# elun15/Graph-Convolutional-Network-for-Multi-Camera-Vehicle-Tracking

Hardware: NVIDIA B200
Metric: mpn_inference_directed_edges_per_sec (higher is better)
Workload: dtype f32

## Files before the change

graph-convolutional-network-for-multi-camera-vehicle-tracking_b200/_lib.py:

```python
import ctypes as C
import os

_HERE = os.path.dirname(os.path.abspath(__file__))
LIB_PATH = os.path.join(_HERE, "libmpn_b200.so")

MPN_OK, MPN_ERR_INVALID, MPN_ERR_CUDA, MPN_ERR_UNSORTED, MPN_ERR_WORKSPACE, MPN_ERR_NO_DEVICE = range(6)
MPN_DE, MPN_DH, MPN_MAX_NODE_LAYERS = 4, 32, 8
MPN_SUMS_DOUBLES = 96
ABI_VERSION = 6
STAGE_ENC0, STAGE_ENC1, STAGE_EDGE, STAGE_NODE, STAGE_APPLY = range(5)
POST_CUT, POST_PRUNE, POST_SPLIT = 1, 2, 4

W_ENC1_W, W_ENC1_B, W_ENC1_G, W_ENC1_BETA = 0, 8, 12, 16
W_ENC2_W, W_ENC2_B, W_ENC2_G, W_ENC2_BETA = 20, 36, 40, 44
W_EDGE_W, W_EDGE_B, W_EDGE_G, W_EDGE_BETA = 48, 320, 324, 328
W_NODE_W, W_NODE_B, W_NODE_G, W_NODE_BETA = 332, 1484, 1516, 1548
W_CLS_W, W_CLS_B = 1580, 1588
W_EDGE_W0, W_NODE_W0, W_SMALL_FLOATS = 1592, 1864, 2888


class MpnGraph(C.Structure):
    _fields_ = [("n_nodes", C.c_int32), ("n_cols", C.c_int32), ("row_offset", C.c_int32), ("chunk", C.c_int32),
                ("n_edges", C.c_int64), ("max_tasks", C.c_int32), ("layout_hint", C.c_int32),
                ("rowptr", C.c_void_p), ("col", C.c_void_p), ("taskptr", C.c_void_p), ("task_row", C.c_void_p),
                ("n_tasks", C.c_void_p), ("n_graphs", C.c_int32), ("max_graph_nodes", C.c_int32),
                ("node_gid", C.c_void_p), ("graph_nptr", C.c_void_p)]


class MpnWeights(C.Structure):
    _fields_ = [("n_node_layers", C.c_int32), ("node_dims", C.c_int32 * (MPN_MAX_NODE_LAYERS + 1)),
                ("node_w", C.c_void_p * MPN_MAX_NODE_LAYERS), ("node_b", C.c_void_p * MPN_MAX_NODE_LAYERS),
                ("node_gamma", C.c_void_p * MPN_MAX_NODE_LAYERS), ("node_beta", C.c_void_p * MPN_MAX_NODE_LAYERS),
                ("small", C.c_void_p),
                ("node_w_hi", C.c_void_p * MPN_MAX_NODE_LAYERS), ("node_w_lo", C.c_void_p * MPN_MAX_NODE_LAYERS),
                ("node_w_hi16", C.c_void_p * MPN_MAX_NODE_LAYERS), ("node_w_lo16", C.c_void_p * MPN_MAX_NODE_LAYERS),
                ("node_w_scale16", C.c_float * MPN_MAX_NODE_LAYERS), ("node_bn_gmax", C.c_float * MPN_MAX_NODE_LAYERS),
                ("node_bn_bmax", C.c_float * MPN_MAX_NODE_LAYERS),
                ("node_agg", C.c_int32), ("reattach_nodes", C.c_int32), ("reattach_edges", C.c_int32), ("reserved", C.c_int32)]


AGG_SUM, AGG_MEAN, AGG_MAX = 0, 1, 2


MPN_MAX_PEERS = 16


class MpnPeerCtx(C.Structure):
    _fields_ = [("rank", C.c_int32), ("world", C.c_int32), ("sums", C.c_void_p * MPN_MAX_PEERS),
                ("flags", C.c_void_p * MPN_MAX_PEERS), ("h", C.c_void_p * MPN_MAX_PEERS),
                ("cstats", C.c_void_p * MPN_MAX_PEERS),
                ("seq_moments", C.c_uint64), ("seq_h", C.c_uint64), ("seq_c", C.c_uint64),
                ("shard_node_encoder", C.c_int32), ("reserved", C.c_int32),
                ("edge_attr", C.c_void_p * MPN_MAX_PEERS), ("node_tables", C.c_void_p * MPN_MAX_PEERS),
                ("block_start", C.c_int32 * (MPN_MAX_PEERS + 1)), ("reserved2", C.c_int32), ("seq_t", C.c_uint64)]
MPN_PEER_CSTAT_COLS = 1024


class MpnError(RuntimeError):
    def __init__(self, code, message):
        super().__init__("libmpn_b200 error %d: %s" % (code, message))
        self.code = code


class UnsortedEdgeIndex(MpnError):
    pass


_lib = None

_PROTOS = {
    "mpn_abi_version": (C.c_int, []),
    "mpn_last_error": (C.c_char_p, []),
    "mpn_kernel_launches": (C.c_uint64, []),
    "mpn_check_device": (C.c_int, [C.c_int]),
    "mpn_set_pdl": (C.c_int, [C.c_int]),
    "mpn_graph_build": (C.c_int, [C.POINTER(MpnGraph), C.c_void_p, C.c_void_p]),
    "mpn_graph_build_i32": (C.c_int, [C.POINTER(MpnGraph), C.c_void_p, C.c_void_p, C.c_void_p]),
    "mpn_graph_build_deferred": (C.c_int, [C.POINTER(MpnGraph), C.c_void_p, C.c_void_p, C.c_void_p, C.c_void_p]),
    "mpn_cross_camera_edges": (C.c_int64, [C.c_void_p, C.c_int32]),
    "mpn_cross_camera_block_edges": (C.c_int64, [C.c_void_p, C.c_int32, C.c_int32, C.c_int32]),
    "mpn_graph_build_cross_camera": (C.c_int, [C.POINTER(MpnGraph), C.c_void_p, C.c_int32, C.c_void_p, C.c_void_p]),
    "mpn_cross_camera_batched_layout": (C.c_int64, [C.c_void_p, C.c_int32, C.c_void_p, C.c_int32, C.c_void_p]),
    "mpn_graph_build_cross_camera_batched": (C.c_int, [C.POINTER(MpnGraph), C.c_void_p, C.c_int32, C.c_void_p, C.c_void_p,
                                                       C.c_void_p, C.c_void_p]),
    "mpn_profile_gram": (C.c_int, [C.c_int]),
    "mpn_profile_gram_ms": (C.c_float, []),
    "mpn_shared_gram_mode": (C.c_int, [C.c_void_p, C.c_int32, C.c_void_p, C.c_size_t, C.c_void_p]),
    "mpn_shared_gram_row_range": (C.c_int, [C.c_int32, C.c_int32, C.c_void_p, C.c_int32, C.c_void_p]),
    "mpn_pack_decisions": (C.c_int, [C.c_void_p, C.c_int64, C.c_void_p, C.c_void_p]),
    "mpn_profile_timeline": (C.c_int, [C.c_int]),
    "mpn_profile_timeline_read": (C.c_int, [C.c_void_p, C.c_char_p, C.c_int]),
    "mpn_edge_features_workspace_bytes": (C.c_size_t, [C.POINTER(MpnGraph), C.c_int32]),
    "mpn_edge_features": (C.c_int, [C.POINTER(MpnGraph), C.c_void_p, C.c_int32, C.c_void_p, C.c_int, C.c_void_p, C.c_size_t, C.c_void_p]),
    "mpn_forward_workspace_bytes": (C.c_size_t, [C.POINTER(MpnGraph), C.POINTER(MpnWeights), C.c_int32]),
    "mpn_forward": (C.c_int, [C.POINTER(MpnGraph), C.POINTER(MpnWeights), C.c_void_p, C.c_void_p, C.c_int32, C.c_int32,
                              C.c_void_p, C.c_void_p, C.c_void_p, C.c_void_p, C.c_int, C.c_void_p, C.c_size_t, C.c_void_p]),
    "mpn_forward_with_edge_features": (C.c_int, [C.POINTER(MpnGraph), C.POINTER(MpnWeights), C.c_void_p, C.c_void_p, C.c_int32, C.c_int32,
                                                 C.c_void_p, C.c_void_p, C.c_void_p, C.c_void_p, C.c_int, C.c_void_p, C.c_size_t,
                                                 C.c_void_p, C.c_size_t, C.c_void_p]),
    "mpn_plan_create": (C.c_int, [C.POINTER(C.c_void_p), C.POINTER(MpnGraph), C.POINTER(MpnWeights), C.c_int32, C.c_int32,
                                  C.c_int64, C.c_int, C.c_void_p, C.c_size_t]),
    "mpn_plan_destroy": (None, [C.c_void_p]),
    "mpn_plan_node_encoder": (C.c_int, [C.c_void_p, C.c_void_p, C.c_void_p]),
    "mpn_plan_node_tables": (C.c_int, [C.c_void_p, C.c_int32, C.c_void_p]),
    "mpn_plan_sweep": (C.c_int, [C.c_void_p, C.c_int32, C.c_int32, C.c_void_p, C.c_void_p, C.c_void_p, C.c_void_p, C.c_void_p]),
    "mpn_plan_sums": (C.c_void_p, [C.c_void_p]),
    "mpn_plan_reduce": (C.c_int, [C.c_void_p, C.c_int32, C.c_int, C.c_void_p]),
    "mpn_plan_finalize": (C.c_int, [C.c_void_p, C.c_int32, C.c_int32, C.c_void_p]),
    "mpn_plan_node_finalize": (C.c_int, [C.c_void_p, C.c_int32, C.c_void_p]),
    "mpn_plan_h_full": (C.c_void_p, [C.c_void_p]),
    "mpn_split_tf32": (C.c_int, [C.c_void_p, C.c_int64, C.c_void_p, C.c_void_p, C.c_void_p]),
    "mpn_split_f16": (C.c_int, [C.c_void_p, C.c_int64, C.c_float, C.c_void_p, C.c_void_p, C.POINTER(C.c_float), C.c_void_p]),
    "mpn_forward_sharded": (C.c_int, [C.POINTER(MpnGraph), C.POINTER(MpnWeights), C.c_void_p, C.c_void_p, C.c_int32, C.c_int32,
                                      C.c_int64, C.c_void_p, C.c_void_p, C.c_void_p, C.c_void_p, C.c_int, C.POINTER(MpnPeerCtx),
                                      C.c_void_p, C.c_size_t, C.c_void_p]),
    "mpn_forward_sharded_with_edge_features": (C.c_int, [C.POINTER(MpnGraph), C.POINTER(MpnWeights), C.c_void_p, C.c_void_p, C.c_int32,
                                                         C.c_int32, C.c_int64, C.c_void_p, C.c_void_p, C.c_void_p, C.c_void_p, C.c_int,
                                                         C.POINTER(MpnPeerCtx), C.c_void_p, C.c_size_t, C.c_void_p, C.c_size_t, C.c_void_p]),
    "mpn_decide": (C.c_int, [C.c_void_p, C.c_int64, C.c_void_p, C.c_void_p, C.c_void_p]),
    "mpn_post_workspace_bytes": (C.c_size_t, [C.POINTER(MpnGraph)]),
    "mpn_cut": (C.c_int, [C.POINTER(MpnGraph), C.c_void_p, C.c_void_p, C.c_size_t, C.c_void_p]),
    "mpn_prune": (C.c_int, [C.POINTER(MpnGraph), C.c_void_p, C.c_void_p, C.c_int32, C.c_int32, C.POINTER(C.c_int32),
                            C.POINTER(C.c_int32), C.c_void_p, C.c_size_t, C.c_void_p]),
    "mpn_split": (C.c_int, [C.POINTER(MpnGraph), C.c_void_p, C.c_void_p, C.c_int32, C.c_int32, C.POINTER(C.c_int32),
                            C.c_void_p, C.c_size_t, C.c_void_p]),
    "mpn_split_last_stats": (None, [C.c_void_p]),
    "mpn_scc_labels": (C.c_int, [C.POINTER(MpnGraph), C.c_void_p, C.c_void_p, C.POINTER(C.c_int32), C.c_void_p, C.c_size_t, C.c_void_p]),
    "mpn_post_processing": (C.c_int, [C.POINTER(MpnGraph), C.c_void_p, C.c_void_p, C.c_int32, C.c_int32, C.c_int32, C.c_void_p,
                                      C.POINTER(C.c_int32), C.POINTER(C.c_int32), C.c_void_p, C.c_size_t, C.c_void_p]),
    "mpn_post_processing_batched": (C.c_int, [C.POINTER(MpnGraph), C.c_void_p, C.c_void_p, C.c_int32, C.c_void_p, C.c_int32,
                                              C.c_void_p, C.c_void_p, C.c_void_p, C.c_size_t, C.c_void_p]),
    "mpn_active_edges": (C.c_int, [C.POINTER(MpnGraph), C.c_void_p, C.c_void_p, C.c_void_p, C.c_int64, C.POINTER(C.c_int64),
                                   C.c_void_p, C.c_size_t, C.c_void_p]),
    "mpn_compact_workspace_bytes": (C.c_size_t, [C.POINTER(MpnGraph)]),
    "mpn_count_active": (C.c_int, [C.POINTER(MpnGraph), C.c_void_p, C.POINTER(C.c_int64), C.c_void_p, C.c_size_t, C.c_void_p]),
    "mpn_compact_active": (C.c_int, [C.POINTER(MpnGraph), C.c_void_p, C.c_void_p, C.c_int32, C.c_void_p, C.c_void_p, C.c_void_p,
                                     C.c_void_p, C.c_void_p, C.c_size_t, C.c_void_p]),
    "mpn_clear_inactive": (C.c_int, [C.c_void_p, C.c_void_p, C.c_void_p, C.c_int64, C.c_void_p]),
    "mpn_labels_reference": (C.c_int, [C.POINTER(MpnGraph), C.c_void_p, C.c_void_p, C.POINTER(C.c_int32), C.c_void_p, C.c_size_t,
                                      C.c_void_p]),
    "mpn_labels_reference_batched": (C.c_int, [C.POINTER(MpnGraph), C.c_void_p, C.c_void_p, C.c_void_p, C.c_void_p, C.c_size_t,
                                              C.c_void_p]),
    "mpn_labels_reference_host": (C.c_int, [C.c_void_p, C.c_void_p, C.c_int64, C.c_int32, C.c_void_p, C.POINTER(C.c_int32)]),
    "mpn_split_exact_host": (C.c_int, [C.c_void_p, C.c_void_p, C.c_void_p, C.c_int64, C.c_int32, C.c_int32, C.c_void_p,
                                      C.c_void_p]),
    "mpn_edge_confusion": (C.c_int, [C.c_void_p, C.c_int, C.c_void_p, C.c_int, C.c_int64, C.c_void_p, C.c_void_p]),
    "mpn_contingency_workspace_bytes": (C.c_size_t, [C.c_int64]),
    "mpn_contingency": (C.c_int, [C.c_void_p, C.c_void_p, C.c_int64, C.c_int64, C.c_int64, C.c_void_p, C.c_void_p, C.c_void_p,
                                  C.POINTER(C.c_int64), C.c_void_p, C.c_void_p, C.c_void_p, C.c_size_t, C.c_void_p]),
    "mpn_expected_mutual_information_host": (C.c_double, [C.c_void_p, C.c_int64, C.c_void_p, C.c_int64, C.c_int64]),
    "mpn_relabel_workspace_bytes": (C.c_size_t, [C.c_int64]),
    "mpn_relabel_detections": (C.c_int, [C.c_void_p, C.c_void_p, C.c_int64, C.c_void_p, C.c_void_p, C.c_void_p, C.c_int64,
                                         C.c_void_p, C.c_void_p, C.c_size_t, C.c_void_p]),
    "mpn_write_mtmc_txt_host": (C.c_int, [C.c_char_p, C.c_void_p, C.c_int64, C.c_int32]),
    "mpn_edge_labels": (C.c_int, [C.POINTER(MpnGraph), C.c_void_p, C.c_void_p, C.c_void_p]),
    "mpn_normalize_columns_workspace_bytes": (C.c_size_t, [C.c_int32]),
    "mpn_normalize_columns": (C.c_int, [C.c_void_p, C.c_int32, C.c_int32, C.c_void_p, C.c_void_p, C.c_size_t, C.c_void_p]),
    "mpn_normalize_columns_batched": (C.c_int, [C.c_void_p, C.c_int32, C.c_int32, C.c_void_p, C.c_int32, C.c_void_p, C.c_void_p,
                                                C.c_size_t, C.c_void_p]),
    "mpn_gemm_nt_workspace_bytes": (C.c_size_t, [C.c_int32, C.c_int32, C.c_int32, C.c_int]),
    "mpn_gram_nt": (C.c_int, [C.c_void_p, C.c_int32, C.c_void_p, C.c_int32, C.c_int32, C.c_int32, C.c_void_p, C.c_void_p, C.c_size_t,
                              C.c_void_p]),
    "mpn_gemm_nt": (C.c_int, [C.c_void_p, C.c_void_p, C.c_void_p, C.c_void_p, C.c_int32, C.c_int32, C.c_int32, C.c_int,
                              C.c_void_p, C.c_size_t, C.c_void_p]),
}

EXPORTED_SYMBOLS = tuple(_PROTOS.keys())


def lib():
    global _lib
    if _lib is None:
        if not os.path.isfile(LIB_PATH):
            raise ImportError("libmpn_b200.so not built: run %s (or __graft_entry__.build()); "
                              "the MPN hot path has no CPU fallback" % os.path.join(_HERE, "csrc", "build.sh"))
        l = C.CDLL(LIB_PATH)
        for name, (res, args) in _PROTOS.items():
            fn = getattr(l, name)
            fn.restype, fn.argtypes = res, args
        if l.mpn_abi_version() != ABI_VERSION:
            raise ImportError("libmpn_b200.so ABI version mismatch")
        _lib = l
    return _lib


def check(code):
    if code != MPN_OK:
        msg = lib().mpn_last_error().decode("utf-8", "replace")
        if code == MPN_ERR_UNSORTED:
            raise UnsortedEdgeIndex(code, msg)
        raise MpnError(code, msg)


_DEVICE_OK = set()


def require_device(index: int):
    index = int(index)
    if index not in _DEVICE_OK:
        check(lib().mpn_check_device(index))
        _DEVICE_OK.add(index)
```

graph-convolutional-network-for-multi-camera-vehicle-tracking_b200/csrc/gemm_tc.cu:

```cuda
#include <cuda.h>
#include <cuda_fp16.h>
#include <stdlib.h>

#include <cmath>

#include "common.cuh"
#include "kernels.h"
#include "tcgen05.cuh"

namespace mpn {

constexpr int TC_BM = 128;
constexpr int TC_BK = 32;
constexpr int TC_UMMA_K = 8;
constexpr int TC_THREADS = 192;
constexpr int TC_BK_F16 = 64;

__device__ __forceinline__ uint64_t make_smem_desc(uint32_t saddr) {
  uint64_t d = 0;
  d |= (uint64_t)((saddr & 0x3FFFF) >> 4);
  d |= (uint64_t)1 << 16;
  d |= (uint64_t)(1024 >> 4) << 32;
  d |= (uint64_t)1 << 46;
  d |= (uint64_t)2 << 61;
  return d;
}

template <int BN>
struct TcCfg {
  static constexpr int STAGES = (BN == 256) ? 2 : 3;
  static constexpr int A_BYTES = TC_BM * TC_BK * 4;
  static constexpr int B_BYTES = BN * TC_BK * 4;
  static constexpr int STAGE_BYTES = 2 * A_BYTES + 2 * B_BYTES;
  static constexpr int SMEM_BYTES = STAGES * STAGE_BYTES + 1024  + 256 ;
  static constexpr int N_MAIN = (BN == 256) ? 1 : 2;
  static constexpr int TMEM_COLS = 512;
  static constexpr int CORR_COL = N_MAIN * BN;
  static constexpr uint32_t IDESC = (1u << 4) | (2u << 7) | (2u << 10) | ((uint32_t)(BN >> 3) << 17) | ((uint32_t)(TC_BM >> 4) << 24);
  static constexpr uint32_t IDESC_F16 = (1u << 4) | ((uint32_t)(BN >> 3) << 17) | ((uint32_t)(TC_BM >> 4) << 24);
};

template <int BN, bool SYM, bool F16>
__global__ void __launch_bounds__(TC_THREADS, 1)
gemm_nt_3xtf32_kernel(const __grid_constant__ CUtensorMap map_a_hi, const __grid_constant__ CUtensorMap map_a_lo,
                      const __grid_constant__ CUtensorMap map_b_hi, const __grid_constant__ CUtensorMap map_b_lo,
                      const float* __restrict__ bias, float* __restrict__ C, int M, int N, int K,
                      const int* __restrict__ graph_nptr, const long long* __restrict__ g_off,
                      const float* __restrict__ out_scale, const int* __restrict__ run_flag) {
  pdl_wait();
  if (run_flag != nullptr && *run_flag == 0) return;
  constexpr int BK = F16 ? TC_BK_F16 : TC_BK;
  using Cfg = TcCfg<BN>;
  extern __shared__ uint8_t smem_raw[];
  uint8_t* smem = (uint8_t*)(((uintptr_t)smem_raw + 1023) & ~(uintptr_t)1023);
  uint64_t* full_bar = (uint64_t*)(smem + Cfg::STAGES * Cfg::STAGE_BYTES);
  uint64_t* empty_bar = full_bar + Cfg::STAGES;
  uint64_t* tmem_full_bar = empty_bar + Cfg::STAGES;
  uint32_t* tmem_slot = (uint32_t*)(tmem_full_bar + 1);

  const int warp = threadIdx.x >> 5, lane = threadIdx.x & 31;
  int m0 = blockIdx.y * TC_BM, n0 = blockIdx.x * BN;
  int tm0 = m0, tn0 = n0;
  const int num_kb = (K + BK - 1) / BK;
  if (SYM && n0 + BN <= m0) return;
  if (graph_nptr != nullptr) {
    const int base = graph_nptr[blockIdx.z];
    const int ng = graph_nptr[blockIdx.z + 1] - base;
    if (m0 >= ng || n0 >= ng) return;
    tm0 = base + m0;
    tn0 = base + n0;
    M = N = ng;
    C += g_off[blockIdx.z];
  }
  if (threadIdx.x == 0) {
    for (int s = 0; s < Cfg::STAGES; ++s) { mbar_init(&full_bar[s], 1); mbar_init(&empty_bar[s], 1); }
    mbar_init(tmem_full_bar, 1);
    asm volatile("fence.mbarrier_init.release.cluster;" ::: "memory");
  }
  if (warp == 1) {
    asm volatile("tcgen05.alloc.cta_group::1.sync.aligned.shared::cta.b32 [%0], %1;" ::"r"(smem_u32(tmem_slot)), "n"(Cfg::TMEM_COLS));
    asm volatile("tcgen05.relinquish_alloc_permit.cta_group::1.sync.aligned;");
  }
  asm volatile("tcgen05.fence::before_thread_sync;" ::: "memory");
  __syncthreads();
  asm volatile("tcgen05.fence::after_thread_sync;" ::: "memory");
  const uint32_t tmem_base = *tmem_slot;

  if (warp == 0) {
    if (lane == 0) {
      asm volatile("prefetch.tensormap [%0];" ::"l"(&map_a_hi));
      asm volatile("prefetch.tensormap [%0];" ::"l"(&map_a_lo));
      asm volatile("prefetch.tensormap [%0];" ::"l"(&map_b_hi));
      asm volatile("prefetch.tensormap [%0];" ::"l"(&map_b_lo));
      int stage = 0;
      uint32_t phase = 0;
      for (int kb = 0; kb < num_kb; ++kb) {
        mbar_wait(&empty_bar[stage], phase ^ 1);
        uint8_t* st = smem + stage * Cfg::STAGE_BYTES;
        mbar_expect_tx(&full_bar[stage], Cfg::STAGE_BYTES);
        const int k0 = kb * BK;
        tma_load_2d(&map_a_hi, &full_bar[stage], st, k0, tm0);
        tma_load_2d(&map_a_lo, &full_bar[stage], st + Cfg::A_BYTES, k0, tm0);
        tma_load_2d(&map_b_hi, &full_bar[stage], st + 2 * Cfg::A_BYTES, k0, tn0);
        tma_load_2d(&map_b_lo, &full_bar[stage], st + 2 * Cfg::A_BYTES + Cfg::B_BYTES, k0, tn0);
        if (++stage == Cfg::STAGES) { stage = 0; phase ^= 1; }
      }
    }
  } else if (warp == 1) {
    if (lane == 0) {
      int stage = 0;
      uint32_t phase = 0;
      for (int kb = 0; kb < num_kb; ++kb) {
        mbar_wait(&full_bar[stage], phase);
        asm volatile("tcgen05.fence::after_thread_sync;" ::: "memory");
        const uint32_t sbase = smem_u32(smem + stage * Cfg::STAGE_BYTES);
        const uint64_t a_hi = make_smem_desc(sbase), a_lo = make_smem_desc(sbase + Cfg::A_BYTES);
        const uint64_t b_hi = make_smem_desc(sbase + 2 * Cfg::A_BYTES), b_lo = make_smem_desc(sbase + 2 * Cfg::A_BYTES + Cfg::B_BYTES);
#pragma unroll
        for (int kk = 0; kk < TC_BK / TC_UMMA_K; ++kk) {
          const uint64_t adv = (uint64_t)((kk * TC_UMMA_K * 4) >> 4);
          const int slice = kb * (TC_BK / TC_UMMA_K) + kk;
          const int which = (Cfg::N_MAIN == 2) ? (slice & 1) : 0;
          if (F16) {
            umma_f16(tmem_base + which * BN, a_hi + adv, b_hi + adv, Cfg::IDESC_F16, slice >= Cfg::N_MAIN);
            umma_f16(tmem_base + Cfg::CORR_COL, a_lo + adv, b_hi + adv, Cfg::IDESC_F16, slice != 0);
            umma_f16(tmem_base + Cfg::CORR_COL, a_hi + adv, b_lo + adv, Cfg::IDESC_F16, 1);
          } else {
            umma_tf32(tmem_base + which * BN, a_hi + adv, b_hi + adv, Cfg::IDESC, slice >= Cfg::N_MAIN);
            umma_tf32(tmem_base + Cfg::CORR_COL, a_lo + adv, b_hi + adv, Cfg::IDESC, slice != 0);
            umma_tf32(tmem_base + Cfg::CORR_COL, a_hi + adv, b_lo + adv, Cfg::IDESC, 1);
          }
        }
        umma_commit(&empty_bar[stage]);
        if (++stage == Cfg::STAGES) { stage = 0; phase ^= 1; }
      }
      umma_commit(tmem_full_bar);
    }
  } else {
    mbar_wait(tmem_full_bar, 0);
    asm volatile("tcgen05.fence::after_thread_sync;" ::: "memory");
    const int q = warp & 3;
    const int row = m0 + q * 32 + lane;
    const bool vec_ok = ((N & 3) == 0) && ((((uintptr_t)C) & 15) == 0);
    const float oscale = (F16 && out_scale) ? *out_scale : 1.f;
#pragma unroll 1
    for (int c0 = 0; c0 < BN; c0 += 32) {
      if (n0 + c0 >= N) break;
      float v[32], w[32];
      const uint32_t tq = tmem_base + ((uint32_t)(q * 32) << 16) + (uint32_t)c0;
      tmem_ld32(tq, v);
      if (Cfg::N_MAIN == 2) {
        tmem_ld32(tq + BN, w);
#pragma unroll
        for (int j = 0; j < 32; ++j) v[j] += w[j];
      }
      tmem_ld32(tq + Cfg::CORR_COL, w);
#pragma unroll
      for (int j = 0; j < 32; ++j) v[j] = F16 ? (v[j] + w[j]) * oscale : v[j] + w[j];
      if (row < M) {
        float* out = C + (size_t)row * N + n0 + c0;
        if (vec_ok && n0 + c0 + 32 <= N) {
#pragma unroll
          for (int j = 0; j < 32; j += 4) {
            float4 o = make_float4(v[j], v[j + 1], v[j + 2], v[j + 3]);
            if (bias) {
              const float4 b = *reinterpret_cast<const float4*>(bias + n0 + c0 + j);
              o.x += b.x; o.y += b.y; o.z += b.z; o.w += b.w;
            }
            *reinterpret_cast<float4*>(out + j) = o;
          }
        } else {
#pragma unroll
          for (int j = 0; j < 32; ++j)
            if (n0 + c0 + j < N) out[j] = v[j] + (bias ? bias[n0 + c0 + j] : 0.f);
        }
      }
      if (SYM && row < M) {
#pragma unroll
        for (int j = 0; j < 32; ++j) {
          const int col = n0 + c0 + j;
          if (col < N && col >= m0 + TC_BM) C[(size_t)col * N + row] = v[j];
        }
      }
    }
    asm volatile("tcgen05.fence::before_thread_sync;" ::: "memory");
  }
  __syncthreads();
  if (warp == 1) {
    asm volatile("tcgen05.fence::after_thread_sync;" ::: "memory");
    asm volatile("tcgen05.dealloc.cta_group::1.sync.aligned.b32 %0, %1;" ::"r"(tmem_base), "n"(Cfg::TMEM_COLS));
  }
}

__global__ void __launch_bounds__(256) split_tf32_kernel(const float4* __restrict__ x, long long n4, int K, const float* __restrict__ scale,
                                                         const float* __restrict__ shift, const int* __restrict__ row_gid,
                                                         float4* __restrict__ hi, float4* __restrict__ lo) {
  pdl_wait();
  const long long stride = (long long)gridDim.x * blockDim.x;
  for (long long i = (long long)blockIdx.x * blockDim.x + threadIdx.x; i < n4; i += stride) {
    const float4 v = x[i];
    float in[4] = {v.x, v.y, v.z, v.w};
    if (scale != nullptr) {
      const int k = (int)((i * 4) % K);
      const size_t o = (row_gid ? (size_t)row_gid[(i * 4) / K] * K : 0) + k;
      const float4 sc = *reinterpret_cast<const float4*>(scale + o), sh = *reinterpret_cast<const float4*>(shift + o);
      in[0] = fmaxf(fmaf(in[0], sc.x, sh.x), 0.f);
      in[1] = fmaxf(fmaf(in[1], sc.y, sh.y), 0.f);
      in[2] = fmaxf(fmaf(in[2], sc.z, sh.z), 0.f);
      in[3] = fmaxf(fmaf(in[3], sc.w, sh.w), 0.f);
    }
    float h[4], l[4];
#pragma unroll
    for (int j = 0; j < 4; ++j) {
      uint32_t hb, lb;
      asm("cvt.rna.tf32.f32 %0, %1;" : "=r"(hb) : "f"(in[j]));
      h[j] = __uint_as_float(hb);
      const float r = in[j] - h[j];
      asm("cvt.rna.tf32.f32 %0, %1;" : "=r"(lb) : "f"(r));
      l[j] = __uint_as_float(lb);
    }
    hi[i] = make_float4(h[0], h[1], h[2], h[3]);
    lo[i] = make_float4(l[0], l[1], l[2], l[3]);
  }
}

__device__ __forceinline__ float f16_scale_of(float amax) {
  if (!(amax > 0.f) || !isfinite(amax)) return 1.f;
  int e;
  frexpf(amax, &e);
  return ldexpf(1.f, 14 - e);
}
__global__ void __launch_bounds__(256) split_f16_kernel(const float4* __restrict__ x, long long n4, const float* __restrict__ amax,
                                                        uint2* __restrict__ hi, uint2* __restrict__ lo, float* __restrict__ out_scale,
                                                        const int* __restrict__ run_flag) {
  pdl_wait();
  if (run_flag != nullptr && *run_flag == 0) return;
  const float s = f16_scale_of(*amax);
  if (out_scale && blockIdx.x == 0 && threadIdx.x == 0) *out_scale = (1.f / s) * (1.f / s);
  const long long stride = (long long)gridDim.x * blockDim.x;
  for (long long i = (long long)blockIdx.x * blockDim.x + threadIdx.x; i < n4; i += stride) {
    const float4 v = x[i];
    const float in[4] = {v.x * s, v.y * s, v.z * s, v.w * s};
    __half h[4], l[4];
#pragma unroll
    for (int j = 0; j < 4; ++j) {
      h[j] = __float2half_rn(in[j]);
      l[j] = __float2half_rn(in[j] - __half2float(h[j]));
    }
    uint2 ph, pl;
    ph.x = (uint32_t)__half_as_ushort(h[0]) | ((uint32_t)__half_as_ushort(h[1]) << 16);
    ph.y = (uint32_t)__half_as_ushort(h[2]) | ((uint32_t)__half_as_ushort(h[3]) << 16);
    pl.x = (uint32_t)__half_as_ushort(l[0]) | ((uint32_t)__half_as_ushort(l[1]) << 16);
    pl.y = (uint32_t)__half_as_ushort(l[2]) | ((uint32_t)__half_as_ushort(l[3]) << 16);
    hi[i] = ph;
    lo[i] = pl;
  }
}

typedef CUresult (*EncodeTiledFn)(CUtensorMap*, CUtensorMapDataType, cuuint32_t, void*, const cuuint64_t*, const cuuint64_t*,
                                  const cuuint32_t*, const cuuint32_t*, CUtensorMapInterleave, CUtensorMapSwizzle,
                                  CUtensorMapL2promotion, CUtensorMapFloatOOBfill);

static EncodeTiledFn get_encode_fn() {
  static EncodeTiledFn fn = nullptr;
  if (!fn) {
    void* p = nullptr;
    cudaDriverEntryPointQueryResult q;
    if (cudaGetDriverEntryPoint("cuTensorMapEncodeTiled", &p, cudaEnableDefault, &q) == cudaSuccess && q == cudaDriverEntryPointSuccess)
      fn = (EncodeTiledFn)p;
  }
  return fn;
}

int make_tma_map_2d(CUtensorMap* map, const void* base, int rows, int K, int box_rows, bool f16) {
  EncodeTiledFn enc = get_encode_fn();
  MPN_REQUIRE(enc != nullptr, "cuTensorMapEncodeTiled is not available from the driver");
  cuuint64_t dims[2] = {(cuuint64_t)K, (cuuint64_t)rows};
  cuuint64_t strides[1] = {(cuuint64_t)K * (f16 ? sizeof(__half) : sizeof(float))};
  cuuint32_t box[2] = {(cuuint32_t)(f16 ? TC_BK_F16 : TC_BK), (cuuint32_t)box_rows};
  cuuint32_t estr[2] = {1, 1};
  CUresult r = enc(map, f16 ? CU_TENSOR_MAP_DATA_TYPE_FLOAT16 : CU_TENSOR_MAP_DATA_TYPE_FLOAT32, 2, (void*)base, dims, strides, box, estr, CU_TENSOR_MAP_INTERLEAVE_NONE,
                   CU_TENSOR_MAP_SWIZZLE_128B, CU_TENSOR_MAP_L2_PROMOTION_L2_256B, CU_TENSOR_MAP_FLOAT_OOB_FILL_NONE);
  MPN_REQUIRE(r == CUDA_SUCCESS, "cuTensorMapEncodeTiled failed with CUresult %d (rows=%d K=%d)", (int)r, rows, K);
  return MPN_OK;
}

int split_tf32(const float* x, long long n, float* hi, float* lo, cudaStream_t st) {
  MPN_REQUIRE(x && hi && lo && n > 0 && (n % 4) == 0, "split_tf32: bad arguments (n must be a positive multiple of 4)");
  MPN_REQUIRE((((uintptr_t)x | (uintptr_t)hi | (uintptr_t)lo) & 15) == 0, "split_tf32: pointers must be 16-byte aligned");
  mpn::launch(split_tf32_kernel, (int)min((long long)kNumSMs * 8, (n / 4 + 255) / 256), 256, 0, st, (const float4*)x, n / 4, 4, nullptr, nullptr, nullptr, (float4*)hi, (float4*)lo);
  MPN_LAUNCH_OK();
  return MPN_OK;
}

bool gemm_tc_supported(int M, int N, int K) { return M >= 1 && N >= 64 && K >= 64 && (K % 4) == 0; }

size_t gemm_tc_workspace_bytes(int M, int N, int K) {
  if (!gemm_tc_supported(M, N, K)) return 0;
  const size_t plane_a = (((size_t)M * K * sizeof(float)) + 255) & ~(size_t)255;
  const size_t plane_b = (((size_t)N * K * sizeof(float)) + 255) & ~(size_t)255;
  return 2 * plane_a + 2 * plane_b + 1024;
}

template <int BN, bool SYM, bool F16 = false>
static int launch_tc(const CUtensorMap& ah, const CUtensorMap& al, const CUtensorMap& bh, const CUtensorMap& bl, const float* bias,
                     float* C, int M, int N, int K, cudaStream_t st, const int* graph_nptr = nullptr, const long long* g_off = nullptr,
                     int n_graphs = 1, int max_ng = 0, const float* out_scale = nullptr, const int* run_flag = nullptr) {
  static bool configured = false;
  if (!configured) {
    MPN_CUDA_OK(cudaFuncSetAttribute(gemm_nt_3xtf32_kernel<BN, SYM, F16>, cudaFuncAttributeMaxDynamicSharedMemorySize, TcCfg<BN>::SMEM_BYTES));
    configured = true;
  }
  dim3 grid(div_up(N, BN), div_up(M, TC_BM));
  if (graph_nptr) grid = dim3(div_up(max_ng, BN), div_up(max_ng, TC_BM), n_graphs);
  mpn::launch(gemm_nt_3xtf32_kernel<BN, SYM, F16>, grid, TC_THREADS, TcCfg<BN>::SMEM_BYTES, st, ah, al, bh, bl, bias, C, M, N, K, graph_nptr, g_off, out_scale, run_flag);
  MPN_LAUNCH_OK();
  return MPN_OK;
}

int gemm_nt_tc(const float* A, const float* B, const float* bias, float* C, int M, int N, int K, void* ws, size_t ws_bytes,
               cudaStream_t st, const float* a_scale, const float* a_shift, const float* b_hi_cached, const float* b_lo_cached,
               const int* row_gid) {
  MPN_REQUIRE(gemm_tc_supported(M, N, K), "tcgen05 GEMM: unsupported shape %d x %d x %d", M, N, K);
  MPN_REQUIRE(ws && ws_bytes >= gemm_tc_workspace_bytes(M, N, K), "tcgen05 GEMM: workspace too small");
  MPN_REQUIRE((((uintptr_t)A | (uintptr_t)B) & 15) == 0, "tcgen05 GEMM: operands must be 16-byte aligned");
  char* w = (char*)(((uintptr_t)ws + 255) & ~(uintptr_t)255);
  const size_t plane_b = (((size_t)N * K * sizeof(float)) + 255) & ~(size_t)255;
  const size_t plane_a = (((size_t)M * K * sizeof(float)) + 255) & ~(size_t)255;
  float* b_hi = (float*)w;
  float* b_lo = (float*)(w + plane_b);
  float *a_hi, *a_lo;
  const int split_grid = kNumSMs * 8;
  if (b_hi_cached && b_lo_cached) {
    b_hi = (float*)b_hi_cached;
    b_lo = (float*)b_lo_cached;
  } else {
    mpn::launch(split_tf32_kernel, split_grid, 256, 0, st, (const float4*)B, (long long)N * K / 4, K, nullptr, nullptr, nullptr, (float4*)b_hi, (float4*)b_lo);
    MPN_LAUNCH_OK();
  }
  if (a_scale == nullptr && A >= B && A + (size_t)M * K <= B + (size_t)N * K) {
    a_hi = b_hi + (A - B);
    a_lo = b_lo + (A - B);
  } else {
    a_hi = (float*)(w + 2 * plane_b);
    a_lo = (float*)(w + 2 * plane_b + plane_a);
    mpn::launch(split_tf32_kernel, split_grid, 256, 0, st, (const float4*)A, (long long)M * K / 4, K, a_scale, a_shift, row_gid, (float4*)a_hi, (float4*)a_lo);
    MPN_LAUNCH_OK();
  }
  CUtensorMap ah, al, bh, bl;
  static int forced_bn = -1;
  if (forced_bn < 0) {
    const char* e = getenv("MPN_TC_BN");
    forced_bn = e ? atoi(e) : 0;
  }
  const int BN = (forced_bn == 128 || forced_bn == 256) ? forced_bn : 128;
  MPN_TRY(make_tma_map_2d(&ah, a_hi, M, K, TC_BM, false));
  MPN_TRY(make_tma_map_2d(&al, a_lo, M, K, TC_BM, false));
  MPN_TRY(make_tma_map_2d(&bh, b_hi, N, K, BN, false));
  MPN_TRY(make_tma_map_2d(&bl, b_lo, N, K, BN, false));
  const bool sym = (A == B) && (M == N) && bias == nullptr;
  if (BN == 256) return launch_tc<256, false>(ah, al, bh, bl, bias, C, M, N, K, st);
  if (sym) return launch_tc<128, true>(ah, al, bh, bl, bias, C, M, N, K, st);
  return launch_tc<128, false>(ah, al, bh, bl, bias, C, M, N, K, st);
}

__global__ void __launch_bounds__(256) split_f16_bn_kernel(const float4* __restrict__ x, long long n4, int K, const float* __restrict__ scale,
                                                           const float* __restrict__ shift, const int* __restrict__ row_gid,
                                                           const float* __restrict__ amax_dev, float amax_host, float b_scale,
                                                           uint2* __restrict__ hi, uint2* __restrict__ lo, float* __restrict__ out_scale) {
  pdl_wait();
  const float s = f16_scale_of(amax_dev ? *amax_dev : amax_host);
  if (out_scale && blockIdx.x == 0 && threadIdx.x == 0) *out_scale = (1.f / s) * (1.f / b_scale);
  const long long stride = (long long)gridDim.x * blockDim.x;
  for (long long i = (long long)blockIdx.x * blockDim.x + threadIdx.x; i < n4; i += stride) {
    const float4 v = x[i];
    float in[4] = {v.x, v.y, v.z, v.w};
    if (scale != nullptr) {
      const int k = (int)((i * 4) % K);
      const size_t o = (row_gid ? (size_t)row_gid[(i * 4) / K] * K : 0) + k;
      const float4 sc = *reinterpret_cast<const float4*>(scale + o), sh = *reinterpret_cast<const float4*>(shift + o);
      in[0] = fmaxf(fmaf(in[0], sc.x, sh.x), 0.f);
      in[1] = fmaxf(fmaf(in[1], sc.y, sh.y), 0.f);
      in[2] = fmaxf(fmaf(in[2], sc.z, sh.z), 0.f);
      in[3] = fmaxf(fmaf(in[3], sc.w, sh.w), 0.f);
    }
    __half h[4], l[4];
#pragma unroll
    for (int j = 0; j < 4; ++j) {
      const float t = fminf(in[j] * s, 65000.f);
      h[j] = __float2half_rn(t);
      l[j] = __float2half_rn(t - __half2float(h[j]));
    }
    uint2 ph, pl;
    ph.x = (uint32_t)__half_as_ushort(h[0]) | ((uint32_t)__half_as_ushort(h[1]) << 16);
    ph.y = (uint32_t)__half_as_ushort(h[2]) | ((uint32_t)__half_as_ushort(h[3]) << 16);
    pl.x = (uint32_t)__half_as_ushort(l[0]) | ((uint32_t)__half_as_ushort(l[1]) << 16);
    pl.y = (uint32_t)__half_as_ushort(l[2]) | ((uint32_t)__half_as_ushort(l[3]) << 16);
    hi[i] = ph;
    lo[i] = pl;
  }
}
__global__ void __launch_bounds__(256) absmax_kernel(const float4* __restrict__ x, long long n4, unsigned int* __restrict__ amax_bits) {
  pdl_wait();
  float m = 0.f;
  const long long stride = (long long)gridDim.x * blockDim.x;
  for (long long i = (long long)blockIdx.x * blockDim.x + threadIdx.x; i < n4; i += stride) {
    const float4 v = x[i];
    m = fmaxf(m, fmaxf(fmaxf(fabsf(v.x), fabsf(v.y)), fmaxf(fabsf(v.z), fabsf(v.w))));
  }
#pragma unroll
  for (int o = 16; o > 0; o >>= 1) m = fmaxf(m, __shfl_xor_sync(0xffffffffu, m, o));
  if ((threadIdx.x & 31) == 0) atomicMax(amax_bits, __float_as_uint(m));
}

float f16_plane_scale_host(float amax) {
  if (!(amax > 0.f) || !std::isfinite(amax)) return 1.f;
  int e;
  frexpf(amax, &e);
  return ldexpf(1.f, 14 - e);
}

int split_f16_host_scale(const float* x, long long n, float amax, void* hi, void* lo, float* scale_out, cudaStream_t st) {
  MPN_REQUIRE(x && hi && lo && n > 0 && (n % 4) == 0, "split_f16: bad arguments (n must be a positive multiple of 4)");
  MPN_REQUIRE((((uintptr_t)x | (uintptr_t)hi | (uintptr_t)lo) & 15) == 0, "split_f16: pointers must be 16-byte aligned");
  mpn::launch(split_f16_bn_kernel, (int)min((long long)kNumSMs * 8, (n / 4 + 255) / 256), 256, 0, st, (const float4*)x, n / 4, 4, nullptr, nullptr, nullptr,
                                                                                           nullptr, amax, 1.f, (uint2*)hi, (uint2*)lo, nullptr);
  MPN_LAUNCH_OK();
  if (scale_out) *scale_out = f16_plane_scale_host(amax);
  return MPN_OK;
}

int gemm_nt_tc_f16(const float* A, const float* bias, float* C, int M, int N, int K, void* ws, size_t ws_bytes, cudaStream_t st,
                   const float* a_scale, const float* a_shift, const int* row_gid, float a_amax_host, const void* b_hi16,
                   const void* b_lo16, float b_scale) {
  MPN_REQUIRE(gemm_tc_supported(M, N, K) && (K % 8) == 0, "tcgen05 fp16-plane GEMM: unsupported shape %d x %d x %d", M, N, K);
  MPN_REQUIRE(ws && ws_bytes >= gemm_tc_workspace_bytes(M, N, K), "tcgen05 GEMM: workspace too small");
  MPN_REQUIRE(b_hi16 && b_lo16 && b_scale > 0.f, "tcgen05 fp16-plane GEMM: missing weight planes");
  char* w = (char*)(((uintptr_t)ws + 255) & ~(uintptr_t)255);
  const size_t plane = (((size_t)M * K * sizeof(__half)) + 255) & ~(size_t)255;
  __half* a_hi = (__half*)w;
  __half* a_lo = (__half*)(w + plane);
  float* out_scale = (float*)(w + 2 * plane);
  unsigned int* amax_bits = (unsigned int*)(w + 2 * plane + 256);
  const float* amax_dev = nullptr;
  if (!(a_amax_host > 0.f)) {
    MPN_CUDA_OK(cudaMemsetAsync(amax_bits, 0, sizeof(unsigned int), st));
    mpn::launch(absmax_kernel, kNumSMs * 8, 256, 0, st, (const float4*)A, (long long)M * K / 4, amax_bits);
    MPN_LAUNCH_OK();
    amax_dev = (const float*)amax_bits;
  }
  mpn::launch(split_f16_bn_kernel, kNumSMs * 8, 256, 0, st, (const float4*)A, (long long)M * K / 4, K, a_scale, a_shift, row_gid, amax_dev, a_amax_host,
                                                   b_scale, (uint2*)a_hi, (uint2*)a_lo, out_scale);
  MPN_LAUNCH_OK();
  CUtensorMap ah, al, bh, bl;
  MPN_TRY(make_tma_map_2d(&ah, a_hi, M, K, TC_BM, true));
  MPN_TRY(make_tma_map_2d(&al, a_lo, M, K, TC_BM, true));
  MPN_TRY(make_tma_map_2d(&bh, b_hi16, N, K, 128, true));
  MPN_TRY(make_tma_map_2d(&bl, b_lo16, N, K, 128, true));
  return launch_tc<128, false, true>(ah, al, bh, bl, bias, C, M, N, K, st, nullptr, nullptr, 1, 0, out_scale);
}

static bool gram_f16_enabled() {
  static int opt = -1;
  if (opt < 0) { const char* e = getenv("MPN_GRAM_F16"); opt = e ? atoi(e) : 1; }
  return opt != 0;
}

int gram_nt_tc(const float* X, int a_row0, float* C, int M, int N, int K, const float* amax_dev, void* ws, size_t ws_bytes, cudaStream_t st,
               const int* run_flag) {
  const float* A = X + (size_t)a_row0 * K;
  if (!gram_f16_enabled() || amax_dev == nullptr || (K % 8) != 0) {
    MPN_REQUIRE(run_flag == nullptr, "tcgen05 Gram: the TF32 planes have no conditional launch");
    return gemm_nt_tc(A, X, nullptr, C, M, N, K, ws, ws_bytes, st);
  }
  MPN_REQUIRE(gemm_tc_supported(M, N, K), "tcgen05 Gram: unsupported shape %d x %d x %d", M, N, K);
  MPN_REQUIRE(ws && ws_bytes >= gemm_tc_workspace_bytes(M, N, K), "tcgen05 Gram: workspace too small");
  char* w = (char*)(((uintptr_t)ws + 255) & ~(uintptr_t)255);
  const size_t plane = (((size_t)N * K * sizeof(__half)) + 255) & ~(size_t)255;
  __half* hi = (__half*)w;
  __half* lo = (__half*)(w + plane);
  float* out_scale = (float*)(w + 2 * plane);
  mpn::launch(split_f16_kernel, kNumSMs * 8, 256, 0, st, (const float4*)X, (long long)N * K / 4, amax_dev, (uint2*)hi, (uint2*)lo, out_scale, run_flag);
  MPN_LAUNCH_OK();
  CUtensorMap ah, al, bh, bl;
  MPN_TRY(make_tma_map_2d(&ah, hi + (size_t)a_row0 * K, M, K, TC_BM, true));
  MPN_TRY(make_tma_map_2d(&al, lo + (size_t)a_row0 * K, M, K, TC_BM, true));
  MPN_TRY(make_tma_map_2d(&bh, hi, N, K, 128, true));
  MPN_TRY(make_tma_map_2d(&bl, lo, N, K, 128, true));
  if (a_row0 == 0 && M == N) return launch_tc<128, true, true>(ah, al, bh, bl, nullptr, C, M, N, K, st, nullptr, nullptr, 1, 0, out_scale, run_flag);
  return launch_tc<128, false, true>(ah, al, bh, bl, nullptr, C, M, N, K, st, nullptr, nullptr, 1, 0, out_scale, run_flag);
}

int gram_blockdiag_tc(const float* X, int N, int K, const int* graph_nptr, const long long* g_off, int n_graphs, int max_ng,
                      float* Gbuf, void* ws, size_t ws_bytes, cudaStream_t st, const float* amax_dev) {
  MPN_REQUIRE(gemm_tc_supported(N, 64, K), "block-diagonal tcgen05 Gram: unsupported K=%d", K);
  MPN_REQUIRE(n_graphs >= 1 && n_graphs <= 65535, "block-diagonal Gram: at most 65535 graphs per launch");
  const size_t plane = (((size_t)N * K * sizeof(float)) + 255) & ~(size_t)255;
  MPN_REQUIRE(ws && ws_bytes >= 2 * plane + 256, "block-diagonal Gram: workspace too small");
  char* w = (char*)(((uintptr_t)ws + 255) & ~(uintptr_t)255);
  if (gram_f16_enabled() && amax_dev != nullptr && (K % 8) == 0) {
    const size_t plane16 = (((size_t)N * K * sizeof(__half)) + 255) & ~(size_t)255;
    __half *hi16 = (__half*)w, *lo16 = (__half*)(w + plane16);
    float* out_scale = (float*)(w + 2 * plane16);
    mpn::launch(split_f16_kernel, kNumSMs * 8, 256, 0, st, (const float4*)X, (long long)N * K / 4, amax_dev, (uint2*)hi16, (uint2*)lo16, out_scale, (const int*)nullptr);
    MPN_LAUNCH_OK();
    CUtensorMap mh16, ml16;
    MPN_TRY(make_tma_map_2d(&mh16, hi16, N, K, TC_BM, true));
    MPN_TRY(make_tma_map_2d(&ml16, lo16, N, K, TC_BM, true));
    return launch_tc<128, true, true>(mh16, ml16, mh16, ml16, nullptr, Gbuf, N, N, K, st, graph_nptr, g_off, n_graphs, max_ng, out_scale);
  }
  float *hi = (float*)w, *lo = (float*)(w + plane);
  mpn::launch(split_tf32_kernel, kNumSMs * 8, 256, 0, st, (const float4*)X, (long long)N * K / 4, K, nullptr, nullptr, nullptr, (float4*)hi, (float4*)lo);
  MPN_LAUNCH_OK();
  CUtensorMap mh, ml;
  MPN_TRY(make_tma_map_2d(&mh, hi, N, K, TC_BM, false));
  MPN_TRY(make_tma_map_2d(&ml, lo, N, K, TC_BM, false));
  return launch_tc<128, true>(mh, ml, mh, ml, nullptr, Gbuf, N, N, K, st, graph_nptr, g_off, n_graphs, max_ng);
}

}
```

graph-convolutional-network-for-multi-camera-vehicle-tracking_b200/csrc/gram_ef.cu:

```cuda
#include <cuda.h>
#include <cuda_fp16.h>

#include <stdlib.h>
#include <string.h>

#include "common.cuh"
#include "kernels.h"
#include "tcgen05.cuh"

namespace mpn {

constexpr int GE_BM = 128, GE_BN = 128, GE_BK = 64;
constexpr int GE_STAGES = 3;
constexpr int GE_PLANE_BYTES = GE_BM * GE_BK * 2;
constexpr int GE_STAGE_BYTES = 4 * GE_PLANE_BYTES;
constexpr int GE_EPI_WARPS = 8;
constexpr int GE_THREADS = 64 + 32 * GE_EPI_WARPS;
constexpr int GE_TMEM_COLS = 512;
constexpr int GE_SUB = 8;
constexpr int GE_TPITCH = GE_SUB + 1;
constexpr uint32_t GE_IDESC_N256 = (1u << 4) | ((uint32_t)(256 >> 3) << 17) | ((uint32_t)(GE_BM >> 4) << 24);
constexpr uint32_t GE_IDESC_N128 = (1u << 4) | ((uint32_t)(128 >> 3) << 17) | ((uint32_t)(GE_BM >> 4) << 24);

struct GeSmem {
// ... 524 lines not shown
            tb[lane][jj] = make_float2(cross ? dd : -1.f, cosv);
          }
          __syncwarp();
          {
            const int cj = lane & (GE_SUB - 1), rsel = lane >> 3;
            const int col = cbase + sub * GE_SUB + cj;
#pragma unroll
            for (int k = 0; k < 32; k += 4) {
              const int rr = k + rsel;
              const float2 o = tb[rr][cj];
              const int4 ri = S.rowinfo[q * 32 + rr];
              if (o.x >= 0.f) A.edge_attr[col + (col >= ri.z ? ri.y : ri.x)] = o;
            }
          }
          __syncwarp();
        }
        if (__any_sync(0xffffffffu, flagged != 0u)) {
          while (flagged) {
            const int j = __ffs(flagged) - 1;
            flagged &= flagged - 1;
            const int col = cbase + j;
            const int4 cb = S.cs_b[c0 + j];
            const bool mir = !SHARED && mirror && cb.y >= 0;
            const int slot = atomicAdd(A.refine_count, mir ? 2 : 1);
            A.refine_list[slot] = col + (col >= gap1 ? rp_row - (gap1 - gap0) : rp_row);
            if (mir) A.refine_list[slot + 1] = grow + (grow >= cb.w ? cb.z : cb.y);
          }
        }
        acc[0] += (double)s_a; acc[1] += (double)s_b; acc[2] += (double)s_aa; acc[3] += (double)s_ab; acc[4] += (double)s_bb;
      }
      tc_fence_before();
      mbar_arrive(&S.tmem_empty_bar[as]);
      asm volatile("bar.sync 1, 256;" ::: "memory");
    }
    if (A.partials != nullptr) {
      double* red = reinterpret_cast<double*>(&S.tbuf[0][0][0]);
#pragma unroll
      for (int k = 0; k < 5; ++k) {
        const double s = warp_sum(acc[k]);
        if (lane == 0) red[ew * 5 + k] = s;
      }
      asm volatile("bar.sync 1, 256;" ::: "memory");
      if (et < 5) {
        double s = 0.0;
        for (int wv = 0; wv < GE_EPI_WARPS; ++wv) s += red[wv * 5 + et];
        A.partials[(size_t)blockIdx.x * MPN_SUMS_DOUBLES + et] = s;
      }
    }
  }
  tc_fence_before();
  __syncthreads();
  if (warp == 1) {
    tc_fence_after();
    tmem_dealloc(tmem_base, GE_TMEM_COLS);
  }
}

int ge_workspace_layout(int n_cols, int M, int D, GeWorkspace* L, void* ws, size_t ws_bytes) {
  Arena a(ws, ws_bytes);
  const size_t plane = (size_t)n_cols * D;
  L->hi = a.take<uint16_t>(plane);
  L->lo = a.take<uint16_t>(plane);
  L->rec = a.take<float4>((size_t)n_cols);
  L->scale_inv = a.take<float>((size_t)n_cols);
  const int tm = (M + GE_BM - 1) / GE_BM, tn = (n_cols + GE_BN - 1) / GE_BN;
  L->tiles = a.take<int>((size_t)tm * tn);
  L->n_tiles = a.take<int>(1);
  L->total = a.off;
  return a.ok() ? MPN_OK : MPN_ERR_WORKSPACE;
}

int ge_col_mean_splits() { return GE_CM_SPLITS; }
bool gram_ef_shape_ok(int M, int N, int D) { return M >= 1 && N >= 2 && D >= GE_BK && (D % GE_BK) == 0 && N < 65536 * GE_BN && M < 65536 * GE_BM; }

static int g_profile_gram = 0;
static cudaEvent_t g_prof_ev[2] = {nullptr, nullptr};

int ge_col_mean(const float* x, int n, int D, double* part, unsigned int* ticket, float* mu, cudaStream_t st) {
  MPN_REQUIRE((D % 4) == 0 && (((uintptr_t)x) & 15) == 0, "column means: D must be a multiple of 4 and x 16-byte aligned");
  const int splits = min(GE_CM_SPLITS, max(1, n / 8));
  mpn::launch(ge_col_mean_kernel, dim3(div_up(D, 128), splits), 256, 0, st, x, n, D, div_up(n, splits), part, ticket, mu);
  MPN_LAUNCH_OK();
  return MPN_OK;
}

int gram_ef_run(const float* x, const float* mu, const mpn_graph* g, int D, int2* gap, int* not_one_gap, float2* edge_attr,
                int* refine_list, int* refine_count, double* partials, int* n_partial_rows, const GeWorkspace& L, cudaStream_t st,
                const GeShare* share) {
  const int N = g->n_cols, M = g->n_nodes;
  MPN_REQUIRE(gram_ef_shape_ok(M, N, D), "fused edge features: unsupported shape M=%d N=%d D=%d", M, N, D);
  const int cs_grid = min(kNumSMs * 16, div_up((long long)N, GE_CS_WARPS));
  const size_t cs_smem = (size_t)GE_CS_WARPS * D * sizeof(float);
  if (cs_smem <= 48 * 1024) {
    mpn::launch(ge_center_split_kernel<true>, cs_grid, 32 * GE_CS_WARPS, cs_smem, st, x, mu, N, D, (uint2*)L.hi, (uint2*)L.lo, L.rec, L.scale_inv, *g,
                gap, not_one_gap);
  } else {
    mpn::launch(ge_center_split_kernel<false>, cs_grid, 32 * GE_CS_WARPS, 0, st, x, mu, N, D, (uint2*)L.hi, (uint2*)L.lo, L.rec, L.scale_inv, *g,
                gap, not_one_gap);
  }
  MPN_LAUNCH_OK();
  GeShare sh;
  memset(&sh, 0, sizeof(sh));
  if (share != nullptr) {
    sh = *share;
    MPN_REQUIRE(sh.world >= 2 && sh.world <= MPN_MAX_PEERS && sh.rank >= 0 && sh.rank < sh.world && sh.mode != nullptr, "shared Gram: bad rank/world");
    MPN_REQUIRE(sh.blk[sh.rank] == g->row_offset && sh.blk[sh.rank + 1] == g->row_offset + M && sh.blk[0] == 0 && sh.blk[sh.world] == N,
                "shared Gram: the row blocks do not match the graph (block [%d,%d), graph rows [%d,%d) of %d)", sh.blk[sh.rank],
                sh.blk[sh.rank + 1], g->row_offset, g->row_offset + M, N);
    MPN_REQUIRE((float2*)sh.ea[sh.rank] == edge_attr, "shared Gram: edge_attr must be this rank's peer-visible buffer");
    mpn::launch(ge_share_exchange_kernel, 1, 1024, 0, st, sh, g->rowptr, (const int2*)gap, M, (const int*)not_one_gap);
    MPN_LAUNCH_OK();
  }
  const int sym = (g->row_offset == 0 && M == N) ? 1 : 0;
  mpn::launch(ge_tile_list_kernel, 1, 1024, 0, st, gap, M, N, g->row_offset, sym, L.tiles, L.n_tiles, not_one_gap, sh);
  MPN_LAUNCH_OK();
  CUtensorMap ah, al, bh, bl;
  MPN_TRY(make_tma_map_2d(&ah, L.hi + (size_t)g->row_offset * D, M, D, GE_BM, true));
  MPN_TRY(make_tma_map_2d(&al, L.lo + (size_t)g->row_offset * D, M, D, GE_BM, true));
  MPN_TRY(make_tma_map_2d(&bh, L.hi, N, D, GE_BN, true));
  MPN_TRY(make_tma_map_2d(&bl, L.lo, N, D, GE_BN, true));
  static bool configured = false;
  if (!configured) {
    MPN_CUDA_OK(cudaFuncSetAttribute(gram_ef_kernel<false>, cudaFuncAttributeMaxDynamicSharedMemorySize, GE_SMEM_BYTES));
    MPN_CUDA_OK(cudaFuncSetAttribute(gram_ef_kernel<true>, cudaFuncAttributeMaxDynamicSharedMemorySize, GE_SMEM_BYTES));
    configured = true;
  }
  GeArgs A;
  A.rec = L.rec; A.scale_inv = L.scale_inv; A.rowptr = g->rowptr; A.gap = gap; A.tiles = L.tiles; A.n_tiles = L.n_tiles;
  A.not_one_gap = not_one_gap; A.edge_attr = edge_attr; A.refine_list = refine_list; A.refine_count = refine_count;
  A.partials = partials; A.M = M; A.N = N; A.K = D; A.row_global0 = g->row_offset; A.sym = sym;
  A.d_eps2 = (float)((double)D * (double)PAIRWISE_EPS * (double)PAIRWISE_EPS);
  A.sh = sh;
  A.node_tab = share ? sh.tab[sh.rank] : nullptr;
  static int balance = -1;
  if (balance < 0) { const char* e = getenv("MPN_GRAM_BALANCE"); balance = e ? atoi(e) : 1; }
  A.balance = balance;
  const int tm = (M + GE_BM - 1) / GE_BM, tn = (N + GE_BN - 1) / GE_BN;
  const int grid = (int)min((long long)kNumSMs, (long long)tm * tn);
  if (n_partial_rows) *n_partial_rows = grid;
  if (g_profile_gram) {
    if (!g_prof_ev[0]) { MPN_CUDA_OK(cudaEventCreate(&g_prof_ev[0])); MPN_CUDA_OK(cudaEventCreate(&g_prof_ev[1])); }
    MPN_CUDA_OK(cudaEventRecord(g_prof_ev[0], st));
  }
  mpn::launch(gram_ef_kernel<false>, grid, GE_THREADS, GE_SMEM_BYTES, st, ah, al, bh, bl, A);
  MPN_LAUNCH_OK();
  if (share != nullptr) {
    mpn::launch(gram_ef_kernel<true>, grid, GE_THREADS, GE_SMEM_BYTES, st, ah, al, bh, bl, A);
    MPN_LAUNCH_OK();
  }
  if (g_profile_gram) MPN_CUDA_OK(cudaEventRecord(g_prof_ev[1], st));
  return MPN_OK;
}

}

extern "C" int mpn_shared_gram_row_range(int32_t rank, int32_t world, const int32_t* block_start, int32_t c, int32_t* out) {
  if (world < 1 || world > MPN_MAX_PEERS || rank < 0 || rank >= world || block_start == nullptr || out == nullptr) return -1;
  mpn::GeShare sh;
  memset(&sh, 0, sizeof(sh));
  sh.rank = rank; sh.world = world;
  for (int r = 0; r <= world; ++r) sh.blk[r] = block_start[r];
  if (c < sh.blk[0] || c >= sh.blk[world]) return -1;
  const int owner = mpn::ge_owner(sh, c);
  const int2 range = mpn::ge_row_range(sh, owner, c);
  out[0] = range.x; out[1] = range.y;
  return owner;
}

extern "C" int mpn_profile_gram(int enable) {
  mpn::g_profile_gram = enable != 0;
  return mpn::g_profile_gram;
}
extern "C" float mpn_profile_gram_ms(void) {
  float ms = -1.f;
  if (mpn::g_prof_ev[0] && cudaEventSynchronize(mpn::g_prof_ev[1]) == cudaSuccess) cudaEventElapsedTime(&ms, mpn::g_prof_ev[0], mpn::g_prof_ev[1]);
  return ms;
}
```

graph-convolutional-network-for-multi-camera-vehicle-tracking_b200/csrc/kernels.h:

```cpp
#pragma once
#include <cuda.h>
#include <cuda_runtime.h>
#include <stddef.h>
#include <stdint.h>

namespace mpn {

constexpr float PAIRWISE_EPS = 1e-6f;
constexpr float COSINE_EPS = 1e-8f;
constexpr float REFINE_FRACTION = 0.25f;

int make_tma_map_2d(CUtensorMap* map, const void* base, int rows, int K, int box_rows, bool f16);

struct GeWorkspace {
  uint16_t *hi, *lo;
  float4* rec;
  float* scale_inv;
  int *tiles, *n_tiles;
  size_t total;
};
struct GeShare {
  int rank, world;
  int blk[MPN_MAX_PEERS + 1];
  float2* ea[MPN_MAX_PEERS];
  int4* tab[MPN_MAX_PEERS];
  unsigned long long* flags[MPN_MAX_PEERS];
  unsigned long long seq;
  int* mode;
};
int ge_workspace_layout(int n_cols, int M, int D, GeWorkspace* L, void* ws, size_t ws_bytes);
bool gram_ef_shape_ok(int M, int N, int D);
int ge_col_mean_splits();
int ge_col_mean(const float* x, int n, int D, double* part, unsigned int* ticket, float* mu, cudaStream_t st);
int gram_ef_run(const float* x, const float* mu, const mpn_graph* g, int D, int2* gap, int* not_one_gap, float2* edge_attr,
                int* refine_list, int* refine_count, double* partials, int* n_partial_rows, const GeWorkspace& L, cudaStream_t st,
                const GeShare* share = nullptr);

struct EfMoments {
  double* partials;
  unsigned long long* fixed_sums;
  const int* handled_flag;
  int known_fused;
};
int edge_features_impl(const mpn_graph* g, const float* x, int32_t D, float* edge_attr, int use_tc, void* ws, size_t ws_bytes,
                       cudaStream_t st, EfMoments* moments, const GeShare* share = nullptr);

int gemm_nt_simt(const float* A, const float* B, const float* bias, const float* a_scale, const float* a_shift,
                 float* C, int M, int N, int K, cudaStream_t st, const int* row_gid = nullptr);

size_t gemm_tc_workspace_bytes(int M, int N, int K);
int gemm_nt_tc(const float* A, const float* B, const float* bias, float* C, int M, int N, int K,
               void* workspace, size_t workspace_bytes, cudaStream_t st, const float* a_scale = nullptr,
               const float* a_shift = nullptr, const float* b_hi_cached = nullptr, const float* b_lo_cached = nullptr,
               const int* row_gid = nullptr);
int split_tf32(const float* x, long long n, float* hi, float* lo, cudaStream_t st);
int gram_nt_tc(const float* X, int a_row0, float* C, int M, int N, int K, const float* amax_dev, void* workspace, size_t workspace_bytes,
               cudaStream_t st, const int* run_flag = nullptr);
bool gemm_tc_supported(int M, int N, int K);
int gemm_nt_tc_f16(const float* A, const float* bias, float* C, int M, int N, int K, void* workspace, size_t workspace_bytes,
                   cudaStream_t st, const float* a_scale, const float* a_shift, const int* row_gid, float a_amax_host,
                   const void* b_hi16, const void* b_lo16, float b_scale);
int split_f16_host_scale(const float* x, long long n, float amax, void* hi, void* lo, float* scale_out, cudaStream_t st);
int gram_blockdiag_tc(const float* X, int N, int K, const int* graph_nptr, const long long* g_off, int n_graphs, int max_ng,
                      float* Gbuf, void* ws, size_t ws_bytes, cudaStream_t st, const float* amax_dev = nullptr);

}
```

graph-convolutional-network-for-multi-camera-vehicle-tracking_b200/csrc/mpn_forward.cu:

```cuda
#include <mutex>
#include <new>
#include <stdlib.h>
#include <string.h>

#include "common.cuh"
#include "kernels.h"
#include "tcgen05.cuh"

namespace mpn {

enum {
  FC_ENC1_W = 0,
  FC_ENC1_C = 8,
  FC_ENC2_W = 12,
  FC_ENC2_C = 28,
  FC_EDGE_WE = 32,
  FC_BN3_S = 48,
  FC_BN3_T = 52,
  FC_NODE_WE = 64,
  FC_BN4_S = 192,
  FC_BN4_T = 224,
  FC_CLS_W = 256,
  FC_CLS_B = 264,
  FC_EDGE_WE0 = 272,
  FC_TOTAL = 288
};

constexpr int SUMS = MPN_SUMS_DOUBLES;
constexpr int SWEEP_THREADS = 256;
constexpr int SWEEP_BLOCKS_PER_SM = 4;
constexpr int SWEEP_GRID = kNumSMs * SWEEP_BLOCKS_PER_SM;
constexpr int SWEEP_RESIDENT_BLOCKS = 3;
constexpr int SWEEP_RESIDENT_GRID = kNumSMs * SWEEP_RESIDENT_BLOCKS;
constexpr float BN_EPS = 1e-5f;

struct EdgeConsts {
  float v[FC_TOTAL];
};

__device__ __forceinline__ void load_consts(EdgeConsts& sc, const float* __restrict__ consts) {
  for (int i = threadIdx.x; i < FC_TOTAL; i += blockDim.x) sc.v[i] = consts[i];
  __syncthreads();
}

constexpr int TASK_PART = 16;
__device__ __forceinline__ void warp_load_consts(EdgeConsts& sc, const float* __restrict__ consts_g, int lane) {
  __syncwarp();
  for (int i = lane; i < FC_TOTAL; i += 32) sc.v[i] = consts_g[i];
  __syncwarp();
}

__device__ __forceinline__ void enc_layer1(const EdgeConsts& sc, float2 ea, float (&a1)[4]) {
#pragma unroll
  for (int j = 0; j < 4; ++j)
    a1[j] = fmaxf(fmaf(sc.v[FC_ENC1_W + 2 * j], ea.x, fmaf(sc.v[FC_ENC1_W + 2 * j + 1], ea.y, sc.v[FC_ENC1_C + j])), 0.f);
}
__device__ __forceinline__ void enc_layer2_pre(const float* __restrict__ w2 , const float* __restrict__ c2,
                                               const float (&a1)[4], float (&u)[4]) {
#pragma unroll
  for (int j = 0; j < 4; ++j) {
    float s = c2[j];
#pragma unroll
    for (int k = 0; k < 4; ++k) s = fmaf(w2[4 * j + k], a1[k], s);
    u[j] = s;
  }
}
__device__ __forceinline__ void enc_full(const EdgeConsts& sc, float2 ea, float (&e0)[4]) {
  float a1[4];
  enc_layer1(sc, ea, a1);
  enc_layer2_pre(&sc.v[FC_ENC2_W], &sc.v[FC_ENC2_C], a1, e0);
#pragma unroll
  for (int j = 0; j < 4; ++j) e0[j] = fmaxf(e0[j], 0.f);
}
__device__ __forceinline__ void edge_pre(const EdgeConsts& sc, const float4 ps, const float4 pd, const float (&ein)[4], float (&y)[4]) {
  const float p[4] = {ps.x + pd.x, ps.y + pd.y, ps.z + pd.z, ps.w + pd.w};
#pragma unroll
  for (int j = 0; j < 4; ++j) {
    float s = p[j];
#pragma unroll
    for (int k = 0; k < 4; ++k) s = fmaf(sc.v[FC_EDGE_WE + 4 * j + k], ein[k], s);
    y[j] = s;
  }
}
__device__ __forceinline__ void bn3_relu(const EdgeConsts& sc, const float (&y)[4], float (&e)[4]) {
#pragma unroll
  for (int j = 0; j < 4; ++j) e[j] = fmaxf(fmaf(sc.v[FC_BN3_S + j], y[j], sc.v[FC_BN3_T + j]), 0.f);
}

struct TaskRange {
  int row, beg, end;
};
__device__ __forceinline__ TaskRange task_range(const mpn_graph& g, int t) {
  TaskRange r;
  r.row = g.task_row[t];
  const int rb = g.rowptr[r.row];
  r.beg = rb + (t - g.taskptr[r.row]) * g.chunk;
  r.end = min(r.beg + g.chunk, g.rowptr[r.row + 1]);
  return r;
}

__device__ __forceinline__ bool task_in(int t, int n_tasks) { return (unsigned)t < (unsigned)n_tasks; }
struct TaskPrefetch {
  TaskRange cur, nxt;
  int row_n;
  __device__ __forceinline__ void start(const mpn_graph& g, int t, int stride, int n_tasks) {
    if (task_in(t, n_tasks)) cur = task_range(g, t);
    row_n = task_in(t + stride, n_tasks) ? g.task_row[t + stride] : 0;
  }
  __device__ __forceinline__ int issue(const mpn_graph& g, int t, int stride, int n_tasks) {
    if (task_in(t + stride, n_tasks)) {
      const int tn = t + stride;
      nxt.row = row_n;
      const int rb = g.rowptr[row_n];
      nxt.beg = rb + (tn - g.taskptr[row_n]) * g.chunk;
      nxt.end = min(nxt.beg + g.chunk, g.rowptr[row_n + 1]);
    }
    return task_in(t + 2 * stride, n_tasks) ? g.task_row[t + 2 * stride] : 0;
  }
  __device__ __forceinline__ void rotate(int row_nn) { cur = nxt; row_n = row_nn; }
};

struct PeerArgs;
struct FinArgs {
  int stage;
  const double* partials;
  int n_partials;
  int row_stride;
  const double* partials2;
  int n_partials2;
  double* sums;
  float* consts;
  const float* small;
  double n_total;
  unsigned int* counter;
  double* n_total_dev;
  double local_edges;
  const unsigned long long* fixed;
  const struct PeerArgs* peers;
  unsigned long long seq;
  int re_e;
};

__device__ __forceinline__ int fin_ncols(int stage) { return (stage == MPN_STAGE_NODE) ? 74 : 8; }

__device__ __forceinline__ double fold_rows(const double* rows, int n_rows, int row_stride, int ncols) {
  __shared__ double red[2048];
  const int k = threadIdx.x;
  const size_t rs = (size_t)row_stride * SUMS;
  const int pairs = ncols >> 1;
  int groups = (int)blockDim.x / pairs;
  if (groups * ncols > 2048) groups = 2048 / ncols;
  if (k < groups * pairs) {
    const int cp = k % pairs, gi = k / pairs;
    const double* base = rows + 2 * cp;
    double2 a0 = make_double2(0.0, 0.0), a1 = a0, a2 = a0, a3 = a0;
    int p = gi;
    for (; p + 3 * groups < n_rows; p += 4 * groups) {
      const double2 v0 = __ldcg(reinterpret_cast<const double2*>(base + (size_t)p * rs));
      const double2 v1 = __ldcg(reinterpret_cast<const double2*>(base + (size_t)(p + groups) * rs));
      const double2 v2 = __ldcg(reinterpret_cast<const double2*>(base + (size_t)(p + 2 * groups) * rs));
// ... 980 lines not shown
      } else {
        float a1[4], u[4];
        enc_layer1(sc, ea, a1);
        enc_layer2_pre(w2raw, w2raw + 16, a1, u);
#pragma unroll
        for (int k = 0; k < 4; ++k) { const double d = u[k]; acc[k] += d; acc[4 + k] += d * d; }
      }
    }
#pragma unroll
    for (int k = 0; k < 8; ++k) {
      const double v = warp_sum(acc[k]);
      if (lane == 0) task_part[(size_t)t * TASK_PART + k] = v;
    }
  }
}

__global__ void __launch_bounds__(128) graph_finalize_kernel(int stage, const mpn_graph g, const double* __restrict__ task_part,
                                                             const float* __restrict__ A, const float4* __restrict__ s1_task,
                                                             const float* __restrict__ small, double* __restrict__ sums_all,
                                                             float* __restrict__ consts_all, int re_e) {
  pdl_wait();
  __shared__ double red[4][64];
  const int gi = blockIdx.x;
  const int n0 = g.graph_nptr[gi], n1 = g.graph_nptr[gi + 1];
  const int t0 = g.taskptr[n0], t1 = g.taskptr[n1];
  const int lane = threadIdx.x & 31, warp = threadIdx.x >> 5;
  double* sums = sums_all + (size_t)gi * SUMS;
  const int ncols = (stage == MPN_STAGE_NODE) ? 10 : 8;
  const int cbase = (stage == MPN_STAGE_NODE) ? 64 : 0;
  for (int col = warp; col < ncols; col += 4) {
    double v = 0.0;
    for (int t = t0 + lane; t < t1; t += 32) v += task_part[(size_t)t * TASK_PART + col];
    v = warp_sum(v);
    if (lane == 0) sums[cbase + col] = v;
  }
  if (stage == MPN_STAGE_NODE) {
    float w[4];
#pragma unroll
    for (int k = 0; k < 4; ++k) w[k] = small[MPN_W_NODE_W + lane * 36 + 32 + k];
    double m1 = 0.0, m2 = 0.0;
    for (int n = n0 + warp; n < n1; n += 4) {
      const int deg = g.rowptr[n + 1] - g.rowptr[n];
      if (deg == 0) continue;
      double sv[4] = {0, 0, 0, 0};
      for (int t = g.taskptr[n]; t < g.taskptr[n + 1]; ++t) {
        const float4 v = s1_task[t];
        sv[0] += v.x; sv[1] += v.y; sv[2] += v.z; sv[3] += v.w;
      }
      const double a = A[(size_t)n * MPN_DH + lane];
      const double qd = w[0] * sv[0] + w[1] * sv[1] + w[2] * sv[2] + w[3] * sv[3];
      m1 += deg * a + qd;
      m2 += deg * a * a + 2.0 * a * qd;
    }
    red[warp][lane] = m1;
    red[warp][32 + lane] = m2;
    __syncthreads();
    if (threadIdx.x < 64) sums[threadIdx.x] = red[0][threadIdx.x] + red[1][threadIdx.x] + red[2][threadIdx.x] + red[3][threadIdx.x];
  }
  __syncthreads();
  FinArgs f;
  f.stage = stage;
  f.partials = nullptr; f.n_partials = 0; f.row_stride = 1; f.partials2 = nullptr; f.n_partials2 = 0;
  f.sums = sums;
  f.consts = consts_all + (size_t)gi * FC_TOTAL;
  f.small = small;
  f.n_total = (double)(g.rowptr[n1] - g.rowptr[n0]);
  f.counter = nullptr;
  f.n_total_dev = nullptr;
  f.local_edges = 0.0;
  f.fixed = nullptr;
  f.peers = nullptr;
  f.seq = 0;
  f.re_e = re_e;
  finalize_body(f, 0, 1);
}

__global__ void __launch_bounds__(256) colstats_graph_kernel(const float* __restrict__ Y, int Nc, const int* __restrict__ graph_nptr,
                                                             const float* __restrict__ gamma, const float* __restrict__ beta,
                                                             float* __restrict__ scale, float* __restrict__ shift) {
  pdl_wait();
  __shared__ double ssum[8][33], ssq[8][33];
  const int cx = threadIdx.x & 31, ry = threadIdx.x >> 5;
  const int col = blockIdx.x * 32 + cx;
  const int gi = blockIdx.y;
  const int r0 = graph_nptr[gi], r1 = graph_nptr[gi + 1];
  double s = 0.0, q = 0.0;
  if (col < Nc)
    for (int r = r0 + ry; r < r1; r += 8) {
      const double v = Y[(size_t)r * Nc + col];
      s += v;
      q += v * v;
    }
  ssum[ry][cx] = s;
  ssq[ry][cx] = q;
  __syncthreads();
  if (ry == 0 && col < Nc) {
    for (int i = 1; i < 8; ++i) { s += ssum[i][cx]; q += ssq[i][cx]; }
    const int M = r1 - r0;
    const double mean = s / M;
    double var = q / M - mean * mean;
    if (var < 0.0) var = 0.0;
    const double sc = (double)gamma[col] / sqrt(var + (double)BN_EPS);
    scale[(size_t)gi * Nc + col] = (float)sc;
    shift[(size_t)gi * Nc + col] = (float)((double)beta[col] - sc * mean);
  }
}

__global__ void __launch_bounds__(SWEEP_THREADS) classify_encoded_kernel(const float2* __restrict__ edge_attr, long long E,
                                                                         const float* __restrict__ consts,
                                                                         float2* __restrict__ logits, uint8_t* __restrict__ pred,
                                                                         float* __restrict__ prob1) {
  pdl_wait();
  __shared__ EdgeConsts sc;
  load_consts(sc, consts);
  const long long stride = (long long)gridDim.x * blockDim.x;
  for (long long e = (long long)blockIdx.x * blockDim.x + threadIdx.x; e < E; e += stride) {
    float ep[4];
    enc_full(sc, ldg_stream2(edge_attr + e), ep);
    float l0 = sc.v[FC_CLS_B + 0], l1 = sc.v[FC_CLS_B + 1];
#pragma unroll
    for (int k = 0; k < 4; ++k) {
      l0 = fmaf(sc.v[FC_CLS_W + k], ep[k], l0);
      l1 = fmaf(sc.v[FC_CLS_W + 4 + k], ep[k], l1);
    }
    logits[e] = make_float2(l0, l1);
    if (pred) pred[e] = (l1 > l0) ? 1 : 0;
    if (prob1) prob1[e] = softmax1(l0, l1);
  }
}

__global__ void __launch_bounds__(256) pack_decisions_kernel(const uint8_t* __restrict__ pred, long long E, uint32_t* __restrict__ words) {
  pdl_wait();
  const long long n_words = (E + 31) >> 5;
  const int lane = threadIdx.x & 31;
  const long long warp0 = ((long long)blockIdx.x * blockDim.x + threadIdx.x) >> 5, nwarps = ((long long)gridDim.x * blockDim.x) >> 5;
  for (long long w = warp0; w < n_words; w += nwarps) {
    const long long e = (w << 5) + lane;
    const unsigned int bits = __ballot_sync(0xffffffffu, e < E && pred[e] != 0);
    if (lane == 0) words[w] = bits;
  }
}

__global__ void decide_kernel(const float2* __restrict__ logits, long long E, uint8_t* __restrict__ pred, float* __restrict__ prob1) {
  pdl_wait();
  const long long stride = (long long)gridDim.x * blockDim.x;
  for (long long e = (long long)blockIdx.x * blockDim.x + threadIdx.x; e < E; e += stride) {
    const float2 l = logits[e];
    if (pred) pred[e] = (l.y > l.x) ? 1 : 0;
    if (prob1) prob1[e] = softmax1(l.x, l.y);
  }
}

constexpr int CS_ROWSPLIT_MAX = 64;
__global__ void __launch_bounds__(256) colstats_kernel(const float* __restrict__ Y, int M, int Nc, int rows_per_split,
                                                       double* __restrict__ part , unsigned int* __restrict__ tile_counter,
                                                       const float* __restrict__ gamma, const float* __restrict__ beta,
                                                       float* __restrict__ scale, float* __restrict__ shift) {
  pdl_wait();
  __shared__ double ssum[8][33], ssq[8][33];
  __shared__ unsigned int s_ticket;
  const int cx = threadIdx.x & 31, ry = threadIdx.x >> 5;
  const int col = blockIdx.x * 32 + cx;
  const int r0 = blockIdx.y * rows_per_split, r1 = min(r0 + rows_per_split, M);
  double s = 0.0, q = 0.0;
  if (col < Nc)
    for (int r = r0 + ry; r < r1; r += 8) {
      const double v = Y[(size_t)r * Nc + col];
      s += v;
      q += v * v;
    }
  ssum[ry][cx] = s;
  ssq[ry][cx] = q;
  __syncthreads();
  if (ry == 0 && col < Nc) {
    for (int i = 1; i < 8; ++i) { s += ssum[i][cx]; q += ssq[i][cx]; }
    part[((size_t)blockIdx.y * Nc + col) * 2 + 0] = s;
    part[((size_t)blockIdx.y * Nc + col) * 2 + 1] = q;
  }
  if (tile_counter == nullptr) return;
  __threadfence();
  __syncthreads();
  if (threadIdx.x == 0) s_ticket = atomicAdd(&tile_counter[blockIdx.x], 1u);
  __syncthreads();
  if (s_ticket != gridDim.y - 1) return;
  __threadfence();
  if (ry == 0 && col < Nc) {
    double ts = 0.0, tq = 0.0;
    for (int i = 0; i < (int)gridDim.y; ++i) {
      ts += __ldcg(&part[((size_t)i * Nc + col) * 2 + 0]);
      tq += __ldcg(&part[((size_t)i * Nc + col) * 2 + 1]);
    }
    const double mean = ts / M;
    double var = tq / M - mean * mean;
    if (var < 0.0) var = 0.0;
    const double sc = (double)gamma[col] / sqrt(var + (double)BN_EPS);
    scale[col] = (float)sc;
    shift[col] = (float)((double)beta[col] - sc * mean);
  }
  if (threadIdx.x == 0) tile_counter[blockIdx.x] = 0u;
}

__global__ void __launch_bounds__(1024) colstats_peer_kernel(const double* __restrict__ part, int splits, int Nc, int M_total,
                                                             const float* __restrict__ gamma, const float* __restrict__ beta,
                                                             float* __restrict__ scale, float* __restrict__ shift,
                                                             const PeerArgs P, unsigned long long seq) {
  pdl_wait();
  const int col = threadIdx.x;
  const int slot = (int)(seq & 1ull);
  double* mine = P.cstats[P.rank] + (size_t)slot * MPN_PEER_CSTAT_COLS * 2;
  if (col < Nc) {
    double s = 0.0, q = 0.0;
    for (int i = 0; i < splits; ++i) {
      s += part[((size_t)i * Nc + col) * 2 + 0];
      q += part[((size_t)i * Nc + col) * 2 + 1];
    }
    mine[2 * col] = s;
    mine[2 * col + 1] = q;
  }
  __threadfence_system();
  __syncthreads();
  if (col == 0) st_release_sys(P.flags[P.rank] + 2 * KPEERS, seq);
  if (col < P.world) wait_flag(P.flags[col] + 2 * KPEERS, seq);
  __syncthreads();
  if (col < Nc) {
    double s = 0.0, q = 0.0;
    for (int r = 0; r < P.world; ++r) {
      const double* src = P.cstats[r] + (size_t)slot * MPN_PEER_CSTAT_COLS * 2 + 2 * col;
      double a, b;
      asm volatile("ld.volatile.global.f64 %0, [%1];" : "=d"(a) : "l"(src));
      asm volatile("ld.volatile.global.f64 %0, [%1];" : "=d"(b) : "l"(src + 1));
      s += a;
      q += b;
    }
    const double mean = s / M_total;
    double var = q / M_total - mean * mean;
    if (var < 0.0) var = 0.0;
    const double sc = (double)gamma[col] / sqrt(var + (double)BN_EPS);
    scale[col] = (float)sc;
    shift[col] = (float)((double)beta[col] - sc * mean);
  }
}

__global__ void bn_relu_apply_peer_kernel(const float* __restrict__ Y, int rows, int row_offset, const float* __restrict__ scale,
                                          const float* __restrict__ shift, const PeerArgs P) {
  pdl_wait();
  const long long total = (long long)rows * MPN_DH;
  const long long stride = (long long)gridDim.x * blockDim.x;
  for (long long i = (long long)blockIdx.x * blockDim.x + threadIdx.x; i < total; i += stride) {
    const int c = (int)(i % MPN_DH);
    const float v = fmaxf(fmaf(Y[i], scale[c], shift[c]), 0.f);
    const size_t o = (size_t)row_offset * MPN_DH + (size_t)i;
    for (int r = 0; r < P.world; ++r) P.h[r][o] = v;
  }
}

__global__ void bn_relu_apply_kernel(const float* __restrict__ Y, long long total, int Nc, const float* __restrict__ scale,
                                     const float* __restrict__ shift, const int* __restrict__ row_gid, float* __restrict__ out) {
  pdl_wait();
  const long long stride = (long long)gridDim.x * blockDim.x;
  for (long long i = (long long)blockIdx.x * blockDim.x + threadIdx.x; i < total; i += stride) {
    const int c = (int)(i % Nc);
    const size_t o = row_gid ? (size_t)row_gid[i / Nc] * Nc + c : (size_t)c;
    out[i] = fmaxf(fmaf(Y[i], scale[o], shift[o]), 0.f);
  }
}

constexpr int NT_NODES = 64, NT_THREADS = 256, NT_OUT = 40;
template <bool RE_N>
__global__ void __launch_bounds__(NT_THREADS) node_tables_kernel(const float* __restrict__ h_full, float* __restrict__ h0_full,
                                                                 int first_step, int n_cols, int row_offset,
                                                                 int n_rows, const float* __restrict__ small,
                                                                 float* __restrict__ Ps, float* __restrict__ Pd,
                                                                 float* __restrict__ A) {
  pdl_wait();
  __shared__ float hs[NT_NODES][33];
  __shared__ float ws[NT_OUT][33];
  __shared__ float hs0[RE_N ? NT_NODES : 1][33];
  __shared__ float ws0[RE_N ? NT_OUT : 1][33];
  __shared__ float bs[NT_OUT];
  const int n0 = blockIdx.x * NT_NODES;
  for (int i = threadIdx.x; i < NT_NODES * 32; i += NT_THREADS) {
    const int n = n0 + (i >> 5);
    const float v = (n < n_cols) ? h_full[(size_t)n * 32 + (i & 31)] : 0.f;
    hs[i >> 5][i & 31] = v;
    if (RE_N) {
      float v0 = v;
      if (n < n_cols) {
        if (first_step) h0_full[(size_t)n * 32 + (i & 31)] = v;
        else v0 = h0_full[(size_t)n * 32 + (i & 31)];
      }
      hs0[i >> 5][i & 31] = v0;
    }
  }
  for (int i = threadIdx.x; i < NT_OUT * 32; i += NT_THREADS) {
    const int o = i >> 5, c = i & 31;
    float v, v0 = 0.f;
    if (o < 4) v = small[MPN_W_EDGE_W + o * 68 + c];
    else if (o < 8) v = small[MPN_W_EDGE_W + (o - 4) * 68 + 32 + c];
    else v = small[MPN_W_NODE_W + (o - 8) * 36 + c];
    ws[o][c] = v;
    if (RE_N) {
      if (o < 4) v0 = small[MPN_W_EDGE_W0 + o * 68 + c];
      else if (o < 8) v0 = small[MPN_W_EDGE_W0 + (o - 4) * 68 + 32 + c];
      else v0 = small[MPN_W_NODE_W0 + (o - 8) * 32 + c];
      ws0[o][c] = v0;
    }
  }
  if (threadIdx.x < NT_OUT) {
    const int o = threadIdx.x;
    bs[o] = (o < 4) ? small[MPN_W_EDGE_B + o] : (o < 8 ? 0.f : small[MPN_W_NODE_B + o - 8]);
  }
  __syncthreads();
  for (int i = threadIdx.x; i < NT_NODES * NT_OUT; i += NT_THREADS) {
    const int ln = i / NT_OUT, o = i % NT_OUT;
    const int n = n0 + ln;
    if (n >= n_cols) continue;
    float s = bs[o];
    if (RE_N) {
#pragma unroll
      for (int c = 0; c < 32; ++c) s = fmaf(ws0[o][c], hs0[ln][c], s);
    }
#pragma unroll
    for (int c = 0; c < 32; ++c) s = fmaf(ws[o][c], hs[ln][c], s);
    const int lr = n - row_offset;
    if (o >= 4 && o < 8) Pd[(size_t)n * 4 + (o - 4)] = s;
    else if (lr >= 0 && lr < n_rows) {
      if (o < 4) Ps[(size_t)lr * 4 + o] = s;
      else A[(size_t)lr * 32 + (o - 8)] = s;
    }
  }
}

struct AbsFix {
  int on;
  int agg;
  const float* A;
  const float4* s1_task;
  const float* consts;
};
template <bool PEERS>
__global__ void __launch_bounds__(256) node_finalize_kernel(const mpn_graph g, const float* __restrict__ msg_task,
                                                            float* __restrict__ h_full, const PeerArgs P, const AbsFix fix) {
  pdl_wait();
  const int lane = threadIdx.x & 31;
  const int gwarp = (blockIdx.x * blockDim.x + threadIdx.x) >> 5;
  const int nwarps = (gridDim.x * blockDim.x) >> 5;
  for (int n = gwarp; n < g.n_nodes; n += nwarps) {
    float s = 0.f;
    const int tb = g.taskptr[n], te = g.taskptr[n + 1];
    if (fix.agg == MPN_AGG_MAX) {
      for (int t = tb; t < te; ++t) s = fmaxf(s, msg_task[(size_t)t * MPN_DH + lane]);
    } else {
      for (int t = tb; t < te; ++t) s += msg_task[(size_t)t * MPN_DH + lane];
    }
    if (fix.on && te > tb) {
      float4 s1 = make_float4(0.f, 0.f, 0.f, 0.f);
      for (int t = tb; t < te; ++t) {
        const float4 v = fix.s1_task[t];
        s1.x += v.x; s1.y += v.y; s1.z += v.z; s1.w += v.w;
      }
      const float deg = (float)(g.rowptr[n + 1] - g.rowptr[n]);
      const float ap = fmaf(fix.consts[FC_BN4_S + lane], fix.A[(size_t)n * MPN_DH + lane], fix.consts[FC_BN4_T + lane]);
      const float* w = fix.consts + FC_NODE_WE + 4 * lane;
      const float lin = fmaf(deg, ap, fmaf(w[0], s1.x, fmaf(w[1], s1.y, fmaf(w[2], s1.z, w[3] * s1.w))));
      s = 0.5f * (s + lin);
    }
    if (fix.agg == MPN_AGG_MEAN) s /= fmaxf((float)(g.rowptr[n + 1] - g.rowptr[n]), 1.f);
    const size_t o = (size_t)(g.row_offset + n) * MPN_DH + lane;
    h_full[o] = s;
    if (PEERS)
      for (int r = 0; r < P.world; ++r)
        if (r != P.rank) P.h[r][o] = s;
  }
}

}

using namespace mpn;

struct mpn_fwd_plan {
  mpn_graph g;
  mpn_weights w;
  int L, n_cls, use_tc, max_dim;
  int msg_abs;
  long long total_edges;
  float *act0, *act1, *colscale, *colshift;
  double* colpart;
  float *h_full, *h0_full, *Ps, *Pd, *A, *consts, *s1_task, *msg_task, *ybuf;
  double *partials, *partials2, *sums;
  unsigned int* fin_counter;
  unsigned long long* fix_sums;
  int seq_m_active;
  PeerArgs* peers_dev;
  unsigned long long seq_m;
  unsigned int* col_counter;
  int fuse_fin;
  int n_graphs;
  double* n_total_dev;
  int n_total_on_device;
  double* task_part;
  void* gemm_ws;
  size_t gemm_ws_bytes;
};

static bool stores_y(const mpn_fwd_plan& p) {
  static int opt = -1;
  if (opt < 0) { const char* e = getenv("MPN_STORE_Y"); opt = e ? atoi(e) : 1; }
  return p.L > 1 || (p.L == 1 && opt != 0 && p.n_graphs <= 1);
}

static mpn::AbsFix abs_fix(const mpn_fwd_plan* p) {
  mpn::AbsFix f;
  f.on = p->msg_abs;
  f.agg = p->w.node_agg;
  f.A = p->A;
  f.s1_task = (const float4*)p->s1_task;
  f.consts = p->consts;
  return f;
}

static int plan_layout(mpn_fwd_plan& p, void* ws, size_t ws_bytes, size_t* need) {
  Arena a(ws, ws_bytes);
  const mpn_graph& g = p.g;
  int max_dim = 0;
  for (int i = 1; i <= p.w.n_node_layers; ++i) max_dim = p.w.node_dims[i] > max_dim ? p.w.node_dims[i] : max_dim;
  p.max_dim = max_dim;
  p.act0 = a.take<float>((size_t)g.n_cols * max_dim);
  p.act1 = a.take<float>((size_t)g.n_cols * max_dim);
  const size_t G = (g.n_graphs > 1 && g.node_gid && g.graph_nptr) ? (size_t)g.n_graphs : 1;
  p.n_graphs = (int)G;
  p.colscale = a.take<float>(G * (max_dim > 0 ? max_dim : 1));
  p.colshift = a.take<float>(G * (max_dim > 0 ? max_dim : 1));
  p.colpart = a.take<double>((size_t)CS_ROWSPLIT_MAX * (max_dim > 0 ? max_dim : 1) * 2);
  p.h_full = a.take<float>((size_t)g.n_cols * MPN_DH);
  p.h0_full = p.w.reattach_nodes ? a.take<float>((size_t)g.n_cols * MPN_DH) : nullptr;
  p.Ps = a.take<float>((size_t)g.n_nodes * 4);
  p.Pd = a.take<float>((size_t)g.n_cols * 4);
  p.A = a.take<float>((size_t)g.n_nodes * MPN_DH);
  p.consts = a.take<float>(G * FC_TOTAL);
  p.task_part = (G > 1) ? a.take<double>((size_t)g.max_tasks * TASK_PART) : nullptr;
  p.s1_task = a.take<float>((size_t)g.max_tasks * 4);
  p.msg_task = a.take<float>((size_t)g.max_tasks * MPN_DH);
  p.sums = a.take<double>(G * SUMS);
  p.partials = a.take<double>((size_t)SWEEP_GRID * SUMS);
  p.partials2 = nullptr;
  p.fin_counter = a.take<unsigned int>(FIN_COUNTERS);
  p.fix_sums = a.take<unsigned long long>(8);
  p.peers_dev = a.take<PeerArgs>(1);
  p.n_total_dev = a.take<double>(1);
  p.col_counter = a.take<unsigned int>((size_t)(max_dim > 0 ? max_dim : 1) / 32 + 1);
  p.ybuf = stores_y(p) ? a.take<float>((size_t)g.n_edges * 4) : nullptr;
  size_t gw = 0;
  if (p.use_tc) {
    int prev = p.w.node_dims[0];
    for (int i = 0; i < p.w.n_node_layers; ++i) {
      size_t b = gemm_tc_workspace_bytes(g.n_cols, p.w.node_dims[i + 1], prev);
      gw = b > gw ? b : gw;
      prev = p.w.node_dims[i + 1];
    }
  }
  p.gemm_ws_bytes = gw;
  p.gemm_ws = gw ? (void*)a.take<char>(gw) : nullptr;
  if (need) *need = a.off;
  if (!a.ok()) {
    set_error("forward workspace too small: need %zu bytes, have %zu", a.off, ws_bytes);
    return MPN_ERR_WORKSPACE;
  }
  return MPN_OK;
}

static int check_weights(const mpn_weights* w) {
  MPN_REQUIRE(w != nullptr, "weights is NULL");
  MPN_REQUIRE(w->n_node_layers >= 1 && w->n_node_layers <= MPN_MAX_NODE_LAYERS, "n_node_layers must be in [1,%d]", MPN_MAX_NODE_LAYERS);
  MPN_REQUIRE(w->node_dims[w->n_node_layers] == MPN_DH, "node_out_dim must be %d (got %d)", MPN_DH, w->node_dims[w->n_node_layers]);
  for (int i = 0; i < w->n_node_layers; ++i)
    MPN_REQUIRE(w->node_w[i] && w->node_b[i] && w->node_gamma[i] && w->node_beta[i] && w->node_dims[i] > 0, "node layer %d has NULL tensors", i);
  MPN_REQUIRE(w->small != nullptr, "small weight block is NULL");
  MPN_REQUIRE(w->node_agg >= MPN_AGG_SUM && w->node_agg <= MPN_AGG_MAX, "node_agg must be MPN_AGG_SUM, _MEAN or _MAX (got %d)", w->node_agg);
  return MPN_OK;
}

extern "C" {

size_t mpn_forward_workspace_bytes(const mpn_graph* g, const mpn_weights* w, int32_t num_enc_steps) {
  if (!g || !w) return 0;
  mpn_fwd_plan p;
  memset(&p, 0, sizeof(p));
  p.g = *g; p.w = *w; p.L = num_enc_steps; p.use_tc = 1;
  size_t need = 0;
  plan_layout(p, nullptr, 0, &need);
  return need + 256;
}

int mpn_plan_create(mpn_fwd_plan** plan_out, const mpn_graph* g, const mpn_weights* w, int32_t L, int32_t n_cls,
                    int64_t total_edges, int use_tc, void* ws, size_t ws_bytes) {
  MPN_REQUIRE(plan_out && g && ws, "plan_create: NULL argument");
  MPN_TRY(check_weights(w));
  MPN_REQUIRE(L >= 0 && n_cls >= 0 && n_cls <= (L > 0 ? L : 1), "need 0 <= num_class_steps <= max(num_enc_steps,1)");
  MPN_REQUIRE(total_edges >= g->n_edges, "total_edges smaller than this shard's edges");
  MPN_REQUIRE(total_edges > 1, "BatchNorm over edges needs more than 1 edge (reference raises ValueError)");
  MPN_REQUIRE(g->n_cols > 1, "BatchNorm over nodes needs more than 1 node (reference raises ValueError)");
  MPN_REQUIRE(((uintptr_t)ws & 255) == 0, "workspace must be 256-byte aligned");
  mpn_fwd_plan* p = new (std::nothrow) mpn_fwd_plan;
  MPN_REQUIRE(p != nullptr, "out of host memory");
  memset(p, 0, sizeof(*p));
  p->g = *g; p->w = *w; p->L = L; p->n_cls = n_cls; p->use_tc = use_tc; p->total_edges = total_edges;
  int rc = plan_layout(*p, ws, ws_bytes, nullptr);
  if (rc != MPN_OK) { delete p; return rc; }
  *plan_out = p;
  return MPN_OK;
}

void mpn_plan_destroy(mpn_fwd_plan* plan) { delete plan; }
double* mpn_plan_sums(mpn_fwd_plan* plan) { return plan ? plan->sums : nullptr; }
float* mpn_plan_h_full(mpn_fwd_plan* plan) { return plan ? plan->h_full : nullptr; }

static cudaError_t clear_moment_state(const mpn_fwd_plan* p, cudaStream_t st) {
  return cudaMemsetAsync(p->partials, 0, (size_t)((const char*)(p->fix_sums + 8) - (const char*)p->partials), st);
}

static FinArgs make_fin(const mpn_fwd_plan* p, int stage, bool fused) {
  FinArgs f;
  f.stage = stage;
  f.partials = p->partials;
  f.n_partials = SWEEP_GRID;
  f.row_stride = 1;
  f.partials2 = p->partials;
  f.n_partials2 = SWEEP_GRID;
  f.sums = p->sums;
  f.consts = p->consts;
  f.small = p->w.small;
  f.n_total = (double)p->total_edges;
  f.counter = fused ? p->fin_counter : nullptr;
  f.n_total_dev = p->n_total_on_device ? p->n_total_dev : nullptr;
  f.local_edges = (double)p->g.n_edges;
  f.fixed = nullptr;
  f.peers = nullptr;
  f.seq = 0;
  if (fused && p->seq_m_active) { f.peers = p->peers_dev; f.seq = ++const_cast<mpn_fwd_plan*>(p)->seq_m; }
  f.re_e = p->w.reattach_edges ? (stores_y(*p) ? 2 : 1) : 0;
  return f;
}

static int sweep_fin(const mpn_fwd_plan* p, int stage, bool fused, int grid, cudaStream_t st, FinArgs& f) {
  f = make_fin(p, stage, fused);
  f.n_partials = f.n_partials2 = grid;
  if (!fused && grid < SWEEP_GRID)
    MPN_CUDA_OK(cudaMemsetAsync(p->partials + (size_t)grid * SUMS, 0, sizeof(double) * (size_t)(SWEEP_GRID - grid) * SUMS, st));
  return MPN_OK;
}

static bool encoder_f16(const mpn_fwd_plan* p, int l, int K) {
  static int opt = -1;
  if (opt < 0) { const char* e = getenv("MPN_ENC_F16"); opt = e ? atoi(e) : 1; }
  return opt != 0 && (K % 8) == 0 && p->w.node_w_hi16[l] && p->w.node_w_lo16[l] && p->w.node_w_scale16[l] > 0.f;
}
static float encoder_input_bound(const mpn_fwd_plan* p, int l, int M_total) {
  if (l == 0) return -1.f;
  const float b = p->w.node_bn_bmax[l - 1] + p->w.node_bn_gmax[l - 1] * sqrtf((float)(M_total > 1 ? M_total - 1 : 1));
  return b > 0.f ? b * 1.0001f : 1.f;
}

static int node_encoder_layers(mpn_fwd_plan* p, const float* x, int l_begin, int l_end, cudaStream_t st) {
  MPN_REQUIRE(p && x, "node_encoder: NULL argument");
  const int M = p->g.n_cols;
  const bool batched = p->n_graphs > 1;
  if (l_begin == 0) MPN_CUDA_OK(cudaMemsetAsync(p->col_counter, 0, sizeof(unsigned int) * ((size_t)p->max_dim / 32 + 1), st));
  float* bufs[2] = {p->act0, p->act1};
  const float* in = l_begin == 0 ? x : bufs[(l_begin - 1) & 1];
  const float *sc = l_begin == 0 ? nullptr : p->colscale, *sh = l_begin == 0 ? nullptr : p->colshift;
  for (int l = l_begin; l < l_end; ++l) {
    const int K = p->w.node_dims[l], Nc = p->w.node_dims[l + 1];
    float* out = bufs[l & 1];
    bool done = false;
    const int* gid = batched ? p->g.node_gid : nullptr;
    if (p->use_tc && gemm_tc_supported(M, Nc, K)) {
      if (encoder_f16(p, l, K))
        MPN_TRY(gemm_nt_tc_f16(in, p->w.node_b[l], out, M, Nc, K, p->gemm_ws, p->gemm_ws_bytes, st, sc, sh, gid,
                               encoder_input_bound(p, l, M), p->w.node_w_hi16[l], p->w.node_w_lo16[l], p->w.node_w_scale16[l]));
      else
        MPN_TRY(gemm_nt_tc(in, p->w.node_w[l], p->w.node_b[l], out, M, Nc, K, p->gemm_ws, p->gemm_ws_bytes, st, sc, sh,
                           p->w.node_w_hi[l], p->w.node_w_lo[l], gid));
      done = true;
    }
    if (!done) MPN_TRY(gemm_nt_simt(in, p->w.node_w[l], p->w.node_b[l], sc, sh, out, M, Nc, K, st, gid));
    if (batched) {
      mpn::launch(colstats_graph_kernel, dim3(div_up(Nc, 32), p->n_graphs), 256, 0, st, out, Nc, p->g.graph_nptr, p->w.node_gamma[l],
                                                                              p->w.node_beta[l], p->colscale, p->colshift);
    } else {
      int splits = div_up(M, 256);
      splits = splits > CS_ROWSPLIT_MAX ? CS_ROWSPLIT_MAX : splits;
      const int rps = div_up(M, splits);
      mpn::launch(colstats_kernel, dim3(div_up(Nc, 32), splits), 256, 0, st, out, M, Nc, rps, p->colpart, p->col_counter, p->w.node_gamma[l],
                                                                    p->w.node_beta[l], p->colscale, p->colshift);
    }
    MPN_LAUNCH_OK();
    in = out;
    sc = p->colscale;
    sh = p->colshift;
  }
  if (l_end < p->w.n_node_layers) return MPN_OK;
  mpn::launch(bn_relu_apply_kernel, min(kNumSMs * 4, div_up((long long)M * MPN_DH, 256)), 256, 0, st, in, (long long)M * MPN_DH, MPN_DH, sc, sh, batched ? p->g.node_gid : nullptr, p->h_full);
  MPN_LAUNCH_OK();
  return MPN_OK;
}

int mpn_plan_node_encoder(mpn_fwd_plan* p, const float* x, void* stream) {
  MPN_REQUIRE(p && x, "node_encoder: NULL argument");
  return node_encoder_layers(p, x, 0, p->w.n_node_layers, (cudaStream_t)stream);
}

static int node_encoder_sharded(mpn_fwd_plan* p, const float* x, const PeerArgs& P, unsigned long long& seq_c, cudaStream_t st,
                                int l_begin, int l_end) {
  const int M = p->g.n_nodes, off = p->g.row_offset;
  float* bufs[2] = {p->act0, p->act1};
  const float* in = l_begin == 0 ? x + (size_t)off * p->w.node_dims[0] : bufs[(l_begin - 1) & 1];
  const float *sc = l_begin == 0 ? nullptr : p->colscale, *sh = l_begin == 0 ? nullptr : p->colshift;
  for (int l = l_begin; l < l_end; ++l) {
    const int K = p->w.node_dims[l], Nc = p->w.node_dims[l + 1];
    MPN_REQUIRE(Nc <= MPN_PEER_CSTAT_COLS, "sharded node encoder: layer width %d > %d", Nc, MPN_PEER_CSTAT_COLS);
    float* out = bufs[l & 1];
    if (p->use_tc && gemm_tc_supported(M, Nc, K) && encoder_f16(p, l, K))
      MPN_TRY(gemm_nt_tc_f16(in, p->w.node_b[l], out, M, Nc, K, p->gemm_ws, p->gemm_ws_bytes, st, sc, sh, nullptr,
                             encoder_input_bound(p, l, p->g.n_cols), p->w.node_w_hi16[l], p->w.node_w_lo16[l], p->w.node_w_scale16[l]));
    else if (p->use_tc && gemm_tc_supported(M, Nc, K))
      MPN_TRY(gemm_nt_tc(in, p->w.node_w[l], p->w.node_b[l], out, M, Nc, K, p->gemm_ws, p->gemm_ws_bytes, st, sc, sh,
                         p->w.node_w_hi[l], p->w.node_w_lo[l], nullptr));
    else
      MPN_TRY(gemm_nt_simt(in, p->w.node_w[l], p->w.node_b[l], sc, sh, out, M, Nc, K, st, nullptr));
    int splits = div_up(M, 256);
    splits = splits > CS_ROWSPLIT_MAX ? CS_ROWSPLIT_MAX : splits;
    const int rps = div_up(M, splits);
    mpn::launch(colstats_kernel, dim3(div_up(Nc, 32), splits), 256, 0, st, out, M, Nc, rps, p->colpart, nullptr, p->w.node_gamma[l],
                                                                  p->w.node_beta[l], p->colscale, p->colshift);
    MPN_LAUNCH_OK();
    mpn::launch(colstats_peer_kernel, 1, 1024, 0, st, p->colpart, splits, Nc, p->g.n_cols, p->w.node_gamma[l], p->w.node_beta[l], p->colscale,
                                            p->colshift, P, ++seq_c);
    MPN_LAUNCH_OK();
    in = out;
    sc = p->colscale;
    sh = p->colshift;
  }
  if (l_end < p->w.n_node_layers) return MPN_OK;
  mpn::launch(bn_relu_apply_peer_kernel, min(kNumSMs * 4, div_up((long long)M * MPN_DH, 256)), 256, 0, st, in, M, off, sc, sh, P);
  MPN_LAUNCH_OK();
  return MPN_OK;
}

int mpn_plan_node_tables(mpn_fwd_plan* p, int32_t step, void* stream) {
  MPN_REQUIRE(p, "node_tables: NULL plan");
  if (p->w.reattach_nodes)
    mpn::launch(node_tables_kernel<true>, div_up(p->g.n_cols, NT_NODES), NT_THREADS, 0, (cudaStream_t)stream, 
        p->h_full, p->h0_full, step <= 1, p->g.n_cols, p->g.row_offset, p->g.n_nodes, p->w.small, p->Ps, p->Pd, p->A);
  else
    mpn::launch(node_tables_kernel<false>, div_up(p->g.n_cols, NT_NODES), NT_THREADS, 0, (cudaStream_t)stream, 
        p->h_full, nullptr, step <= 1, p->g.n_cols, p->g.row_offset, p->g.n_nodes, p->w.small, p->Ps, p->Pd, p->A);
  MPN_LAUNCH_OK();
  return MPN_OK;
}

int mpn_plan_sweep(mpn_fwd_plan* p, int32_t step, int32_t stage, const float* edge_attr, float* logits_out,
                   uint8_t* pred_out, float* prob1_out, void* stream) {
  MPN_REQUIRE(p && edge_attr, "sweep: NULL argument");
  cudaStream_t st = (cudaStream_t)stream;
  const mpn_graph& g = p->g;
  const float2* ea = (const float2*)edge_attr;
  const bool stored = stores_y(*p);
  const bool fused = p->fuse_fin != 0;
  const int flat_grid = (int)min((long long)SWEEP_GRID, (long long)div_up(g.n_edges > 0 ? g.n_edges : 1, SWEEP_THREADS));
  const bool batched = p->n_graphs > 1;
  const float4 *Ps4 = (const float4*)p->Ps, *Pd4 = (const float4*)p->Pd;
  float4* yb = (float4*)p->ybuf;
  if (batched) {
    double* tp = p->task_part;
    switch (stage) {
      case MPN_STAGE_ENC0:
        mpn::launch(enc_moments_task_kernel<0>, SWEEP_GRID, SWEEP_THREADS, 0, st, g, ea, p->consts, p->w.small, tp);
        break;
      case MPN_STAGE_ENC1:
        mpn::launch(enc_moments_task_kernel<1>, SWEEP_GRID, SWEEP_THREADS, 0, st, g, ea, p->consts, p->w.small, tp);
        break;
      case MPN_STAGE_EDGE:
        if (step == 1) {
          if (stored) mpn::launch(edge_moments_kernel<0, true, true>, SWEEP_GRID, SWEEP_THREADS, 0, st, g, ea, Ps4, Pd4, yb, p->consts, tp, make_fin(p, stage, false));
          else mpn::launch(edge_moments_kernel<0, false, true>, SWEEP_GRID, SWEEP_THREADS, 0, st, g, ea, Ps4, Pd4, nullptr, p->consts, tp, make_fin(p, stage, false));
        } else {
          if (p->w.reattach_edges) mpn::launch(edge_moments_kernel<1, true, true, true>, SWEEP_GRID, SWEEP_THREADS, 0, st, g, ea, Ps4, Pd4, yb, p->consts, tp, make_fin(p, stage, false));
          else mpn::launch(edge_moments_kernel<1, true, true>, SWEEP_GRID, SWEEP_THREADS, 0, st, g, ea, Ps4, Pd4, yb, p->consts, tp, make_fin(p, stage, false));
        }
        break;
      case MPN_STAGE_NODE:
        if (stored) mpn::launch(node_moments_sweep_kernel<1, true>, SWEEP_RESIDENT_GRID, SWEEP_THREADS, 0, st, g, ea, Ps4, Pd4, yb, p->consts, (float4*)p->s1_task, tp, p->A, p->w.small, make_fin(p, stage, false));
        else mpn::launch(node_moments_sweep_kernel<0, true>, SWEEP_GRID, SWEEP_THREADS, 0, st, g, ea, Ps4, Pd4, nullptr, p->consts, (float4*)p->s1_task, tp, p->A, p->w.small, make_fin(p, stage, false));
        break;
      case MPN_STAGE_APPLY: {
        const bool classify = logits_out != nullptr;
        float2* lg = (float2*)logits_out;
        MPN_REQUIRE(p->L > 0, "batched graphs need num_enc_steps >= 1");
#define MPN_APPLY_B2(YS, CL, MX) mpn::launch(apply_kernel<YS, CL, true, MX>, SWEEP_GRID, SWEEP_THREADS, 0, st, g, ea, Ps4, Pd4, yb, p->A, p->consts, p->msg_task, lg, pred_out, prob1_out)
#define MPN_APPLY_B(YS, CL) do { if (p->w.node_agg == MPN_AGG_MAX) MPN_APPLY_B2(YS, CL, true); else MPN_APPLY_B2(YS, CL, false); } while (0)
        if (stored) { if (classify) MPN_APPLY_B(1, true); else MPN_APPLY_B(1, false); }
        else        { if (classify) MPN_APPLY_B(0, true); else MPN_APPLY_B(0, false); }
#undef MPN_APPLY_B
#undef MPN_APPLY_B2
        break;
      }
      default:
        MPN_REQUIRE(false, "unknown stage %d", stage);
    }
    MPN_LAUNCH_OK();
    if (stage != MPN_STAGE_APPLY) {
      mpn::launch(graph_finalize_kernel, p->n_graphs, 128, 0, st, stage, g, tp, p->A, (const float4*)p->s1_task, p->w.small, p->sums, p->consts,
                                                         p->w.reattach_edges ? (stored ? 2 : 1) : 0);
      MPN_LAUNCH_OK();
    }
    return MPN_OK;
  }
  switch (stage) {
    case MPN_STAGE_ENC0:
      MPN_CUDA_OK(clear_moment_state(p, st));
      mpn::launch(enc_moments_kernel<0>, flat_grid, SWEEP_THREADS, 0, st, ea, g.n_edges, p->consts, p->w.small, p->partials, make_fin(p, stage, fused),
                  (const int*)nullptr);
      break;
    case MPN_STAGE_ENC1:
      if ((((uintptr_t)ea) & 15) == 0 && g.n_edges >= 2) {
        const long long n_pairs = g.n_edges >> 1;
        const int pgrid = (int)min((long long)kNumSMs * 2, (long long)div_up(n_pairs, SWEEP_THREADS));
        FinArgs pf;
        MPN_TRY(sweep_fin(p, stage, fused, pgrid, st, pf));
        mpn::launch(enc_moments1_packed_kernel, pgrid, SWEEP_THREADS, 0, st, (const float4*)ea, n_pairs, ea, g.n_edges, p->consts, p->w.small,
                    p->partials, pf);
      } else {
        mpn::launch(enc_moments_kernel<1>, flat_grid, SWEEP_THREADS, 0, st, ea, g.n_edges, p->consts, p->w.small, p->partials, make_fin(p, stage, fused),
                    (const int*)nullptr);
      }
      break;
    case MPN_STAGE_EDGE:
      if (step == 1) {
        if (stored) mpn::launch(edge_moments_kernel<0, true, false>, SWEEP_GRID, SWEEP_THREADS, 0, st, g, ea, Ps4, Pd4, yb, p->consts, p->partials, make_fin(p, stage, fused));
        else mpn::launch(edge_moments_kernel<0, false, false>, SWEEP_GRID, SWEEP_THREADS, 0, st, g, ea, Ps4, Pd4, nullptr, p->consts, p->partials, make_fin(p, stage, fused));
      } else {
        if (p->w.reattach_edges) mpn::launch(edge_moments_kernel<1, true, false, true>, SWEEP_GRID, SWEEP_THREADS, 0, st, g, ea, Ps4, Pd4, yb, p->consts, p->partials, make_fin(p, stage, fused));
        else mpn::launch(edge_moments_kernel<1, true, false>, SWEEP_GRID, SWEEP_THREADS, 0, st, g, ea, Ps4, Pd4, yb, p->consts, p->partials, make_fin(p, stage, fused));
      }
      break;
    case MPN_STAGE_NODE: {
      FinArgs nf;
      MPN_TRY(sweep_fin(p, stage, fused, stored ? SWEEP_RESIDENT_GRID : SWEEP_GRID, st, nf));
      if (stored) mpn::launch(node_moments_sweep_kernel<1, false>, SWEEP_RESIDENT_GRID, SWEEP_THREADS, 0, st, g, ea, Ps4, Pd4, yb, p->consts, (float4*)p->s1_task, p->partials, p->A, p->w.small, nf);
      else mpn::launch(node_moments_sweep_kernel<0, false>, SWEEP_GRID, SWEEP_THREADS, 0, st, g, ea, Ps4, Pd4, nullptr, p->consts, (float4*)p->s1_task, p->partials, p->A, p->w.small, nf);
      break;
    }
    case MPN_STAGE_APPLY: {
      const bool classify = logits_out != nullptr;
      float2* lg = (float2*)logits_out;
      if (p->L == 0) {
        MPN_REQUIRE(classify, "L == 0 needs a logits buffer");
        mpn::launch(classify_encoded_kernel, flat_grid, SWEEP_THREADS, 0, st, ea, g.n_edges, p->consts, lg, pred_out, prob1_out);
        break;
      }
      static int apply_tc = -1;
      if (apply_tc < 0) { const char* e = getenv("MPN_APPLY_TC"); apply_tc = e ? atoi(e) : 1; }
      p->msg_abs = 0;
      if (p->use_tc && apply_tc && stored && g.chunk >= ATC_THREADS && (!classify || (pred_out != nullptr) == (prob1_out != nullptr))) {
        const bool agg_max = p->w.node_agg == MPN_AGG_MAX;
        p->msg_abs = agg_max ? 0 : 1;
#define MPN_ATC3(CL, DE, MX, NC) mpn::launch(apply_tc_kernel<CL, DE, MX, NC>, kNumSMs * NC, ATC_THREADS, 0, st, g, yb, p->A, p->consts, p->msg_task, lg, pred_out, prob1_out)
#define MPN_ATC2(CL, DE, MX) MPN_ATC3(CL, DE, MX, ATC_CTAS_PER_SM)
#define MPN_ATC(CL, DE) do { if (agg_max) MPN_ATC2(CL, DE, true); else MPN_ATC2(CL, DE, false); } while (0)
        if (!classify) MPN_ATC(false, false);
        else if (pred_out && prob1_out) MPN_ATC(true, true);
        else MPN_ATC(true, false);
#undef MPN_ATC
#undef MPN_ATC2
#undef MPN_ATC3
        break;
      }
#define MPN_APPLY2(YS, CL, MX) mpn::launch(apply_kernel<YS, CL, false, MX>, SWEEP_GRID, SWEEP_THREADS, 0, st, g, ea, Ps4, Pd4, yb, p->A, p->consts, p->msg_task, lg, pred_out, prob1_out)
#define MPN_APPLY(YS, CL) do { if (p->w.node_agg == MPN_AGG_MAX) MPN_APPLY2(YS, CL, true); else MPN_APPLY2(YS, CL, false); } while (0)
      if (stored) { if (classify) MPN_APPLY(1, true); else MPN_APPLY(1, false); }
      else        { if (classify) MPN_APPLY(0, true); else MPN_APPLY(0, false); }
#undef MPN_APPLY
#undef MPN_APPLY2
      break;
    }
    default:
      MPN_REQUIRE(false, "unknown stage %d", stage);
  }
  MPN_LAUNCH_OK();
  return MPN_OK;
}

int mpn_plan_finalize(mpn_fwd_plan* p, int32_t step, int32_t stage, void* stream) {
  MPN_REQUIRE(p, "finalize: NULL plan");
  (void)step;
  if (p->n_graphs > 1) return MPN_OK;
  mpn::launch(finalize_kernel, 1, FIN_THREADS, 0, (cudaStream_t)stream, make_fin(p, stage, false), 0, 1);
  MPN_LAUNCH_OK();
  return MPN_OK;
}

int mpn_plan_reduce(mpn_fwd_plan* p, int32_t stage, int with_consts, void* stream) {
  MPN_REQUIRE(p, "reduce: NULL plan");
  if (p->n_graphs > 1) return MPN_OK;
  mpn::launch(finalize_kernel, 1, FIN_THREADS, 0, (cudaStream_t)stream, make_fin(p, stage, false), 1, with_consts);
  MPN_LAUNCH_OK();
  return MPN_OK;
}

int mpn_plan_node_finalize(mpn_fwd_plan* p, int32_t step, void* stream) {
  MPN_REQUIRE(p, "node_finalize: NULL plan");
  (void)step;
  mpn::launch(node_finalize_kernel<false>, min(kNumSMs * 8, div_up((long long)p->g.n_nodes * 32, 256)), 256, 0, (cudaStream_t)stream, p->g, p->msg_task, p->h_full, PeerArgs(), abs_fix(p));
  MPN_LAUNCH_OK();
  return MPN_OK;
}

struct SideStream {
  cudaStream_t stream;
  cudaEvent_t fork, join;
};
static SideStream* side_stream() {
  static SideStream table[64];
  static int state[64];
  static std::mutex init_lock;
  int dev = 0;
  if (cudaGetDevice(&dev) != cudaSuccess || dev < 0 || dev >= 64) return nullptr;
  std::lock_guard<std::mutex> hold(init_lock);
  if (state[dev] == 0) {
    SideStream& s = table[dev];
    const bool ok = cudaStreamCreateWithFlags(&s.stream, cudaStreamNonBlocking) == cudaSuccess &&
                    cudaEventCreateWithFlags(&s.fork, cudaEventDisableTiming) == cudaSuccess &&
                    cudaEventCreateWithFlags(&s.join, cudaEventDisableTiming) == cudaSuccess;
    state[dev] = ok ? 1 : -1;
  }
  return state[dev] == 1 ? &table[dev] : nullptr;
}

constexpr int TL_MAX = 24;
static bool g_tl_on = false;
static cudaEvent_t g_tl_ev[TL_MAX];
static const char* g_tl_name[TL_MAX];
static int g_tl_n = 0;
static void tl_mark(const char* name, cudaStream_t st, bool first = false) {
  if (!g_tl_on) return;
  if (first) g_tl_n = 0;
  if (g_tl_n >= TL_MAX) return;
  if (!g_tl_ev[g_tl_n] && cudaEventCreate(&g_tl_ev[g_tl_n]) != cudaSuccess) return;
  if (cudaEventRecord(g_tl_ev[g_tl_n], st) != cudaSuccess) return;
  g_tl_name[g_tl_n++] = name;
}

static int forward_impl(const mpn_graph* g, const mpn_weights* w, const float* x, float* edge_attr_rw, int32_t L, int32_t n_cls,
                        float* logits_out, float* h_out, uint8_t* pred_out, float* prob1_out, int use_tc, void* ws, size_t ws_bytes,
                        void* ef_ws, size_t ef_ws_bytes, void* stream) {
  const float* edge_attr = edge_attr_rw;
  MPN_REQUIRE(g && x && edge_attr && logits_out, "forward: NULL argument");
  MPN_REQUIRE(g->row_offset == 0 && g->n_cols == g->n_nodes, "mpn_forward runs an unsharded graph; use the plan API for row blocks");
  cudaStream_t st = (cudaStream_t)stream;
  mpn_fwd_plan* p = nullptr;
  MPN_TRY(mpn_plan_create(&p, g, w, L, n_cls, g->n_edges, use_tc, ws, ws_bytes));
  int rc = MPN_OK;
  const size_t lstride = (size_t)g->n_edges * 2;
#define STEP_TRY(expr) do { rc = (expr); if (rc != MPN_OK) goto done; } while (0)
  p->fuse_fin = (p->n_graphs > 1) ? 0 : 1;
  {
    SideStream* ss = side_stream();
    tl_mark("start", st, true);
    const bool fork = ss != nullptr && cudaEventRecord(ss->fork, st) == cudaSuccess && cudaStreamWaitEvent(ss->stream, ss->fork, 0) == cudaSuccess;
    bool encoder_enqueued = false;
    int enc_done_layers = 0;
#define ENQUEUE_ENCODER() do { if (!encoder_enqueued) { encoder_enqueued = true; \
      STEP_TRY(node_encoder_layers(p, x, enc_done_layers, p->w.n_node_layers, fork ? ss->stream : st)); \
      tl_mark("node_encoder_end(side stream)", fork ? ss->stream : st); \
      if (fork && cudaEventRecord(ss->join, ss->stream) != cudaSuccess) { set_error("event record failed"); rc = MPN_ERR_CUDA; goto done; } } } while (0)
    if (!fork || ef_ws == nullptr) ENQUEUE_ENCODER();
    else if (p->w.n_node_layers > 1) {
      STEP_TRY(node_encoder_layers(p, x, 0, 1, ss->stream));
      enc_done_layers = 1;
    }
    bool enc0_done = false;
    if (ef_ws != nullptr && p->n_graphs <= 1) {
      if (clear_moment_state(p, st) != cudaSuccess) { set_error("memset failed"); rc = MPN_ERR_CUDA; goto done; }
      EfMoments mom;
      mom.partials = p->partials; mom.fixed_sums = p->fix_sums; mom.handled_flag = nullptr; mom.known_fused = 0;
      STEP_TRY(edge_features_impl(g, x, w->node_dims[0], edge_attr_rw, use_tc, ef_ws, ef_ws_bytes, st, &mom));
      ENQUEUE_ENCODER();
      if (mom.handled_flag != nullptr) {
        if (!mom.known_fused) {
          const int flat_grid = (int)min((long long)SWEEP_GRID, (long long)div_up(g->n_edges > 0 ? g->n_edges : 1, SWEEP_THREADS));
          mpn::launch(enc_moments_kernel<0>, flat_grid, SWEEP_THREADS, 0, st, (const float2*)edge_attr, g->n_edges, p->consts, p->w.small,
                      p->partials, make_fin(p, MPN_STAGE_ENC0, false), mom.handled_flag);
          ++mpn::g_kernel_launches;
        }
        FinArgs f = make_fin(p, MPN_STAGE_ENC0, false);
        f.fixed = p->fix_sums;
        mpn::launch(finalize_kernel, 1, FIN_THREADS, 0, st, f, 1, 1);
        ++mpn::g_kernel_launches;
        if (cudaGetLastError() != cudaSuccess) { set_error("ENC0 finalize launch failed"); rc = MPN_ERR_CUDA; goto done; }
        if ((long long)kNumSMs > (long long)div_up(g->n_edges > 0 ? g->n_edges : 1, SWEEP_THREADS) &&
            cudaMemsetAsync(p->partials, 0, sizeof(double) * SWEEP_GRID * SUMS, st) != cudaSuccess) { set_error("memset failed"); rc = MPN_ERR_CUDA; goto done; }
        enc0_done = true;
      }
    } else if (ef_ws != nullptr) {
      STEP_TRY(mpn_edge_features(g, x, w->node_dims[0], edge_attr_rw, use_tc, ef_ws, ef_ws_bytes, st));
    }
    ENQUEUE_ENCODER();
#undef ENQUEUE_ENCODER
    if (!enc0_done) STEP_TRY(mpn_plan_sweep(p, 0, MPN_STAGE_ENC0, edge_attr, nullptr, nullptr, nullptr, st));
    tl_mark("edge_features+enc0_end", st);
    STEP_TRY(mpn_plan_sweep(p, 0, MPN_STAGE_ENC1, edge_attr, nullptr, nullptr, nullptr, st));
    tl_mark("enc1_end", st);
    if (fork && cudaStreamWaitEvent(st, ss->join, 0) != cudaSuccess) { set_error("stream wait failed"); rc = MPN_ERR_CUDA; goto done; }
    tl_mark("joined", st);
  }
  if (L == 0) {
    STEP_TRY(mpn_plan_sweep(p, 0, MPN_STAGE_APPLY, edge_attr, logits_out, pred_out, prob1_out, st));
  }
  {
    const int first_class_step = L - n_cls + 1;
    int k = 0;
    for (int step = 1; step <= L; ++step) {
      STEP_TRY(mpn_plan_node_tables(p, step, st));
      tl_mark("node_tables_end", st);
      STEP_TRY(mpn_plan_sweep(p, step, MPN_STAGE_EDGE, edge_attr, nullptr, nullptr, nullptr, st));
      tl_mark("edge_update_end", st);
      STEP_TRY(mpn_plan_sweep(p, step, MPN_STAGE_NODE, edge_attr, nullptr, nullptr, nullptr, st));
      tl_mark("node_moments_end", st);
      const bool cls = step >= first_class_step;
      const bool last = step == L;
      STEP_TRY(mpn_plan_sweep(p, step, MPN_STAGE_APPLY, edge_attr, cls ? logits_out + lstride * k : nullptr,
                              (cls && last) ? pred_out : nullptr, (cls && last) ? prob1_out : nullptr, st));
      if (cls) ++k;
      tl_mark("node_apply_end", st);
      STEP_TRY(mpn_plan_node_finalize(p, step, st));
      tl_mark("node_finalize_end", st);
    }
  }
  if (h_out) {
    cudaError_t e = cudaMemcpyAsync(h_out, p->h_full, sizeof(float) * (size_t)g->n_nodes * MPN_DH, cudaMemcpyDeviceToDevice, st);
    if (e != cudaSuccess) { set_error("h copy failed: %s", cudaGetErrorString(e)); rc = MPN_ERR_CUDA; }
  }
#undef STEP_TRY
done:
  mpn_plan_destroy(p);
  return rc;
}

int mpn_forward(const mpn_graph* g, const mpn_weights* w, const float* x, const float* edge_attr, int32_t L, int32_t n_cls,
                float* logits_out, float* h_out, uint8_t* pred_out, float* prob1_out, int use_tc, void* ws, size_t ws_bytes,
                void* stream) {
  return forward_impl(g, w, x, const_cast<float*>(edge_attr), L, n_cls, logits_out, h_out, pred_out, prob1_out, use_tc, ws, ws_bytes,
                      nullptr, 0, stream);
}

int mpn_forward_with_edge_features(const mpn_graph* g, const mpn_weights* w, const float* x, float* edge_attr_out, int32_t L,
                                   int32_t n_cls, float* logits_out, float* h_out, uint8_t* pred_out, float* prob1_out, int use_tc,
                                   void* ws, size_t ws_bytes, void* ef_ws, size_t ef_ws_bytes, void* stream) {
  MPN_REQUIRE(ef_ws != nullptr && edge_attr_out != nullptr, "forward_with_edge_features: NULL edge-feature buffer / workspace");
  return forward_impl(g, w, x, edge_attr_out, L, n_cls, logits_out, h_out, pred_out, prob1_out, use_tc, ws, ws_bytes, ef_ws,
                      ef_ws_bytes, stream);
}

static int forward_sharded_impl(const mpn_graph* g, const mpn_weights* w, const float* x, float* edge_attr_rw, int32_t L, int32_t n_cls,
                                int64_t total_edges, float* logits_out, float* h_out, uint8_t* pred_out, float* prob1_out, int use_tc,
                                const mpn_peer_ctx* peers, void* ws, size_t ws_bytes, void* ef_ws, size_t ef_ws_bytes, void* stream) {
  const float* edge_attr = edge_attr_rw;
  MPN_REQUIRE(g && x && edge_attr && logits_out && peers, "forward_sharded: NULL argument");
  MPN_REQUIRE(peers->world >= 1 && peers->world <= MPN_MAX_PEERS && peers->rank >= 0 && peers->rank < peers->world, "forward_sharded: bad rank/world");
  MPN_REQUIRE(g->n_graphs <= 1, "forward_sharded: batched graphs cannot be row-sharded");
  MPN_REQUIRE(L >= 1, "forward_sharded needs num_enc_steps >= 1");
  PeerArgs P;
  P.rank = peers->rank;
  P.world = peers->world;
  for (int r = 0; r < peers->world; ++r) {
    MPN_REQUIRE(peers->sums[r] && peers->flags[r] && (L <= 1 || peers->h[r]), "forward_sharded: NULL peer buffer for rank %d", r);
    MPN_REQUIRE(!peers->shard_node_encoder || (peers->h[r] && peers->cstats[r]), "forward_sharded: sharded encoder needs h and cstats buffers");
    P.sums[r] = peers->sums[r];
    P.flags[r] = (unsigned long long*)peers->flags[r];
    P.h[r] = peers->h[r];
    P.cstats[r] = peers->cstats[r];
  }
  const bool shard_enc = peers->shard_node_encoder != 0;
  cudaStream_t st = (cudaStream_t)stream;
  mpn_fwd_plan* p = nullptr;
  MPN_TRY(mpn_plan_create(&p, g, w, L, n_cls, total_edges > 0 ? total_edges : (int64_t)1 << 40, use_tc, ws, ws_bytes));
  p->n_total_on_device = total_edges > 0 ? 0 : 1;
  if (L > 1 || shard_enc) p->h_full = peers->h[peers->rank];
  p->fuse_fin = 1;
  p->seq_m_active = 1;
  p->seq_m = peers->seq_moments;
  int rc = MPN_OK;
  unsigned long long& seq_m = p->seq_m;
  unsigned long long seq_h = peers->seq_h, seq_c = peers->seq_c;
  if (cudaMemcpyAsync(p->peers_dev, &P, sizeof(PeerArgs), cudaMemcpyHostToDevice, st) != cudaSuccess ||
      cudaMemsetAsync(p->fin_counter, 0, sizeof(unsigned int) * FIN_COUNTERS, st) != cudaSuccess) {
    set_error("peer table upload failed");
    mpn_plan_destroy(p);
    return MPN_ERR_CUDA;
  }
  bool h_pending = false;
  const size_t lstride = (size_t)g->n_edges * 2;
  GeShare share;
  const GeShare* share_ptr = nullptr;
  if (ef_ws != nullptr && peers->world >= 2 && peers->edge_attr[0] != nullptr) {
    memset(&share, 0, sizeof(share));
    share.rank = peers->rank; share.world = peers->world; share.seq = peers->seq_t + 1;
    for (int r = 0; r < peers->world; ++r) {
      if (!(peers->edge_attr[r] && peers->node_tables[r])) { set_error("forward_sharded: NULL shared-Gram buffer for rank %d", r); mpn_plan_destroy(p); return MPN_ERR_INVALID; }
      share.ea[r] = (float2*)peers->edge_attr[r];
      share.tab[r] = (int4*)peers->node_tables[r];
      share.flags[r] = (unsigned long long*)peers->flags[r];
      share.blk[r] = peers->block_start[r];
    }
    share.blk[peers->world] = peers->block_start[peers->world];
    share_ptr = &share;
  }
#define STEP_TRY(expr) do { rc = (expr); if (rc != MPN_OK) goto done; } while (0)
#define PEER_FINALIZE(stage) do { mpn::launch(finalize_peer_kernel, 1, FIN_THREADS, 0, st, make_fin(p, stage, false), P, ++seq_m); \
    ++mpn::g_kernel_launches; if (cudaGetLastError() != cudaSuccess) { set_error("finalize_peer launch failed"); rc = MPN_ERR_CUDA; goto done; } } while (0)
#define ENC0_STAGE() do { \
    bool enc0_done_ = false; \
    if (ef_ws != nullptr) { \
      if (clear_moment_state(p, st) != cudaSuccess) { set_error("memset failed"); rc = MPN_ERR_CUDA; goto done; } \
      EfMoments mom_; \
      mom_.partials = p->partials; mom_.fixed_sums = p->fix_sums; mom_.handled_flag = nullptr; mom_.known_fused = 0; \
      STEP_TRY(edge_features_impl(g, x, w->node_dims[0], edge_attr_rw, use_tc, ef_ws, ef_ws_bytes, st, &mom_, share_ptr)); \
      if (mom_.handled_flag != nullptr) { \
// ... 164 lines not shown
```

include/mpn_b200.h:

```cpp
#ifndef MPN_B200_H
#define MPN_B200_H

#include <stddef.h>
#include <stdint.h>

#ifdef __cplusplus
extern "C" {
#endif

#define MPN_B200_ABI_VERSION 6

enum {
  MPN_OK = 0,
  MPN_ERR_INVALID = 1,
  MPN_ERR_CUDA = 2,
  MPN_ERR_UNSORTED = 3,
  MPN_ERR_WORKSPACE = 4,
  MPN_ERR_NO_DEVICE = 5
};

#define MPN_DE 4
#define MPN_DH 32
#define MPN_MAX_NODE_LAYERS 8

int mpn_abi_version(void);
const char* mpn_last_error(void);
uint64_t mpn_kernel_launches(void);
int mpn_set_pdl(int enable);
int mpn_check_device(int dev);

typedef struct mpn_graph {
  int32_t n_nodes;
  int32_t n_cols;
  int32_t row_offset;
  int32_t chunk;
  int64_t n_edges;
  int32_t max_tasks;
  int32_t layout_hint;
  int32_t* rowptr;
  int32_t* col;
  int32_t* taskptr;
  int32_t* task_row;
  int32_t* n_tasks;
  int32_t n_graphs;
  int32_t max_graph_nodes;
  int32_t* node_gid;
  int32_t* graph_nptr;
} mpn_graph;

enum { MPN_LAYOUT_UNKNOWN = 0, MPN_LAYOUT_ONE_GAP = 1 };
int mpn_graph_build(mpn_graph* g, const int64_t* edge_index_dev, void* stream);
int mpn_graph_build_i32(mpn_graph* g, const int32_t* row_dev, const int32_t* col_dev, void* stream);
int mpn_graph_build_deferred(mpn_graph* g, const int64_t* edge_index_dev, int32_t* flags_dev, int32_t* flags_host_pinned,
                             void* stream);

#define MPN_MAX_CAMERAS 64
int64_t mpn_cross_camera_edges(const int32_t* cam_ptr_host, int32_t n_cams);
int64_t mpn_cross_camera_block_edges(const int32_t* cam_ptr_host, int32_t n_cams, int32_t row0, int32_t n_rows);
int mpn_graph_build_cross_camera(mpn_graph* g, const int32_t* cam_ptr_host, int32_t n_cams, int64_t* edge_index_out_dev,
                                 void* stream);
int64_t mpn_cross_camera_batched_layout(const int32_t* seg_ptr_host, int32_t n_segs, const int32_t* graph_seg_host, int32_t n_graphs,
                                        int64_t* seg_ebase_host);
int mpn_graph_build_cross_camera_batched(mpn_graph* g, const int32_t* seg_ptr_dev, int32_t n_segs, const int32_t* graph_seg_dev,
                                         const int64_t* seg_ebase_dev, int64_t* edge_index_out_dev, void* stream);

int mpn_profile_gram(int enable);
float mpn_profile_gram_ms(void);
int mpn_shared_gram_mode(const mpn_graph* g, int32_t feature_dim, const void* ef_workspace_dev, size_t ef_workspace_bytes, void* stream);
int mpn_shared_gram_row_range(int32_t rank, int32_t world, const int32_t* block_start, int32_t c, int32_t* out_host);
int mpn_profile_timeline(int enable);
int mpn_profile_timeline_read(float* ms_out, char* names_out, int names_bytes);
size_t mpn_edge_features_workspace_bytes(const mpn_graph* g, int32_t D);
int mpn_edge_features(const mpn_graph* g, const float* x_dev, int32_t D, float* edge_attr_dev,
                      int use_tensor_cores, void* workspace_dev, size_t workspace_bytes, void* stream);

enum {
  MPN_W_ENC1_W = 0,
  MPN_W_ENC1_B = 8,
  MPN_W_ENC1_G = 12,
  MPN_W_ENC1_BETA = 16,
  MPN_W_ENC2_W = 20,
  MPN_W_ENC2_B = 36,
  MPN_W_ENC2_G = 40,
  MPN_W_ENC2_BETA = 44,
  MPN_W_EDGE_W = 48,
  MPN_W_EDGE_B = 320,
  MPN_W_EDGE_G = 324,
  MPN_W_EDGE_BETA = 328,
  MPN_W_NODE_W = 332,
  MPN_W_NODE_B = 1484,
  MPN_W_NODE_G = 1516,
  MPN_W_NODE_BETA = 1548,
  MPN_W_CLS_W = 1580,
  MPN_W_CLS_B = 1588,
  MPN_W_EDGE_W0 = 1592,
  MPN_W_NODE_W0 = 1864,
  MPN_W_SMALL_FLOATS = 2888
};

typedef struct mpn_weights {
  int32_t n_node_layers;
  int32_t node_dims[MPN_MAX_NODE_LAYERS + 1];
  const float* node_w[MPN_MAX_NODE_LAYERS];
  const float* node_b[MPN_MAX_NODE_LAYERS];
  const float* node_gamma[MPN_MAX_NODE_LAYERS];
  const float* node_beta[MPN_MAX_NODE_LAYERS];
  const float* small;
  const float* node_w_hi[MPN_MAX_NODE_LAYERS];
  const float* node_w_lo[MPN_MAX_NODE_LAYERS];
  const void* node_w_hi16[MPN_MAX_NODE_LAYERS];
  const void* node_w_lo16[MPN_MAX_NODE_LAYERS];
  float node_w_scale16[MPN_MAX_NODE_LAYERS];
  float node_bn_gmax[MPN_MAX_NODE_LAYERS];
  float node_bn_bmax[MPN_MAX_NODE_LAYERS];
  int32_t node_agg;
  int32_t reattach_nodes;
  int32_t reattach_edges;
  int32_t reserved;
} mpn_weights;
enum { MPN_AGG_SUM = 0, MPN_AGG_MEAN = 1, MPN_AGG_MAX = 2 };

int mpn_split_tf32(const float* x_dev, int64_t n, float* hi_dev, float* lo_dev, void* stream);
int mpn_split_f16(const float* x_dev, int64_t n, float amax, void* hi_dev, void* lo_dev, float* scale_out_host, void* stream);

size_t mpn_forward_workspace_bytes(const mpn_graph* g, const mpn_weights* w, int32_t num_enc_steps);
int mpn_forward(const mpn_graph* g, const mpn_weights* w, const float* x_dev, const float* edge_attr_dev,
                int32_t num_enc_steps, int32_t num_class_steps, float* logits_out_dev, float* h_out_dev,
                uint8_t* pred_out_dev, float* prob1_out_dev, int use_tensor_cores,
                void* workspace_dev, size_t workspace_bytes, void* stream);

int mpn_forward_with_edge_features(const mpn_graph* g, const mpn_weights* w, const float* x_dev, float* edge_attr_out_dev,
                                   int32_t num_enc_steps, int32_t num_class_steps, float* logits_out_dev, float* h_out_dev,
                                   uint8_t* pred_out_dev, float* prob1_out_dev, int use_tensor_cores, void* workspace_dev,
                                   size_t workspace_bytes, void* ef_workspace_dev, size_t ef_workspace_bytes, void* stream);

typedef struct mpn_fwd_plan mpn_fwd_plan;
enum { MPN_SUMS_DOUBLES = 96 };
enum {
  MPN_STAGE_ENC0 = 0,
  MPN_STAGE_ENC1 = 1,
  MPN_STAGE_EDGE = 2,
  MPN_STAGE_NODE = 3,
  MPN_STAGE_APPLY = 4
};
int mpn_plan_create(mpn_fwd_plan** plan_out, const mpn_graph* g, const mpn_weights* w, int32_t num_enc_steps,
                    int32_t num_class_steps, int64_t total_edges, int use_tensor_cores,
                    void* workspace_dev, size_t workspace_bytes);
void mpn_plan_destroy(mpn_fwd_plan* plan);
int mpn_plan_node_encoder(mpn_fwd_plan* plan, const float* x_dev, void* stream);
int mpn_plan_node_tables(mpn_fwd_plan* plan, int32_t step, void* stream);
int mpn_plan_sweep(mpn_fwd_plan* plan, int32_t step, int32_t stage, const float* edge_attr_dev,
                   float* logits_out_dev, uint8_t* pred_out_dev, float* prob1_out_dev, void* stream);
double* mpn_plan_sums(mpn_fwd_plan* plan);
int mpn_plan_reduce(mpn_fwd_plan* plan, int32_t stage, int with_consts, void* stream);
int mpn_plan_finalize(mpn_fwd_plan* plan, int32_t step, int32_t stage, void* stream);
int mpn_plan_node_finalize(mpn_fwd_plan* plan, int32_t step, void* stream);
float* mpn_plan_h_full(mpn_fwd_plan* plan);

#define MPN_MAX_PEERS 16
typedef struct mpn_peer_ctx {
  int32_t rank, world;
  double* sums[MPN_MAX_PEERS];
  uint64_t* flags[MPN_MAX_PEERS];
  float* h[MPN_MAX_PEERS];
  double* cstats[MPN_MAX_PEERS];
  uint64_t seq_moments;
  uint64_t seq_h;
  uint64_t seq_c;
  int32_t shard_node_encoder;
  int32_t reserved;
  float* edge_attr[MPN_MAX_PEERS];
  int32_t* node_tables[MPN_MAX_PEERS];
  int32_t block_start[MPN_MAX_PEERS + 1];
  int32_t reserved2;
  uint64_t seq_t;
} mpn_peer_ctx;
#define MPN_PEER_CSTAT_COLS 1024
int mpn_forward_sharded(const mpn_graph* g, const mpn_weights* w, const float* x_dev, const float* edge_attr_dev,
                        int32_t num_enc_steps, int32_t num_class_steps, int64_t total_edges, float* logits_out_dev,
                        float* h_out_dev , uint8_t* pred_out_dev, float* prob1_out_dev,
                        int use_tensor_cores, const mpn_peer_ctx* peers, void* workspace_dev, size_t workspace_bytes, void* stream);
int mpn_forward_sharded_with_edge_features(const mpn_graph* g, const mpn_weights* w, const float* x_dev, float* edge_attr_out_dev,
                                           int32_t num_enc_steps, int32_t num_class_steps, int64_t total_edges, float* logits_out_dev,
                                           float* h_out_dev, uint8_t* pred_out_dev, float* prob1_out_dev, int use_tensor_cores,
                                           const mpn_peer_ctx* peers, void* workspace_dev, size_t workspace_bytes,
                                           void* ef_workspace_dev, size_t ef_workspace_bytes, void* stream);

int mpn_decide(const float* logits_dev, int64_t n_edges, uint8_t* pred_out_dev, float* prob1_out_dev, void* stream);
int mpn_pack_decisions(const uint8_t* pred_dev, int64_t n_edges, uint32_t* words_out_dev, void* stream);

enum { MPN_POST_CUT = 1, MPN_POST_PRUNE = 2, MPN_POST_SPLIT = 4 };
size_t mpn_post_workspace_bytes(const mpn_graph* g);
int mpn_cut(const mpn_graph* g, uint8_t* act_dev, void* workspace_dev, size_t workspace_bytes, void* stream);
int mpn_prune(const mpn_graph* g, uint8_t* act_dev, const float* prob1_dev, int32_t prob_stride, int32_t num_cameras,
              int32_t* changed_host, int32_t* rounds_host, void* workspace_dev, size_t workspace_bytes, void* stream);
int mpn_split(const mpn_graph* g, uint8_t* act_dev, const float* prob1_dev, int32_t prob_stride, int32_t num_cameras,
              int32_t* rounds_host, void* workspace_dev, size_t workspace_bytes, void* stream);
void mpn_split_last_stats(int64_t out_host[4]);
int mpn_scc_labels(const mpn_graph* g, const uint8_t* act_dev, int32_t* labels_dev, int32_t* n_components_host,
                   void* workspace_dev, size_t workspace_bytes, void* stream);
int mpn_post_processing(const mpn_graph* g, uint8_t* act_dev, const float* prob1_dev, int32_t prob_stride,
                        int32_t num_cameras, int32_t flags, int32_t* labels_dev, int32_t* n_components_host,
                        int32_t* prune_changed_host, void* workspace_dev, size_t workspace_bytes, void* stream);
int mpn_post_processing_batched(const mpn_graph* g, uint8_t* act_dev, const float* prob1_dev, int32_t prob_stride,
                                const int32_t* num_cameras_dev, int32_t flags, int32_t* labels_dev, int32_t* n_components_host,
                                void* workspace_dev, size_t workspace_bytes, void* stream);
int mpn_active_edges(const mpn_graph* g, const uint8_t* act_dev, int32_t* src_out_dev, int32_t* dst_out_dev,
                     int64_t capacity, int64_t* n_active_host, void* workspace_dev, size_t workspace_bytes, void* stream);
size_t mpn_compact_workspace_bytes(const mpn_graph* g);
int mpn_count_active(const mpn_graph* g, const uint8_t* act_dev, int64_t* n_active_host, void* workspace_dev,
                     size_t workspace_bytes, void* stream);
int mpn_compact_active(const mpn_graph* g, const uint8_t* act_dev, const float* prob1_dev, int32_t prob_stride,
                       int32_t* src_out_dev, int32_t* dst_out_dev, int32_t* eid_out_dev, float* prob_out_dev,
                       void* workspace_dev, size_t workspace_bytes, void* stream);
int mpn_clear_inactive(uint8_t* act_dev, const int32_t* eid_dev, const uint8_t* keep_dev, int64_t n, void* stream);
int mpn_labels_reference(const mpn_graph* g, const uint8_t* act_dev, int64_t* labels_out_host, int32_t* n_components_host,
                         void* workspace_dev, size_t workspace_bytes, void* stream);
int mpn_labels_reference_batched(const mpn_graph* g, const uint8_t* act_dev, int64_t* labels_out_host, int32_t* n_components_host,
                                 void* workspace_dev, size_t workspace_bytes, void* stream);
int mpn_labels_reference_host(const int32_t* src_host, const int32_t* dst_host, int64_t n_active, int32_t n_nodes,
                              int64_t* labels_out_host, int32_t* n_components_host);
int mpn_split_exact_host(const int32_t* src_host, const int32_t* dst_host, const float* prob_host, int64_t n_active,
                         int32_t n_nodes, int32_t num_cameras, uint8_t* keep_out_host, int64_t* stats_out);

size_t mpn_gemm_nt_workspace_bytes(int32_t M, int32_t N, int32_t K, int impl);
int mpn_gemm_nt(const float* A_dev, const float* B_dev, const float* bias_dev, float* C_dev,
                int32_t M, int32_t N, int32_t K, int impl, void* workspace_dev, size_t workspace_bytes, void* stream);
int mpn_gram_nt(const float* X_dev, int32_t row0, float* C_dev, int32_t M, int32_t N, int32_t K, const float* amax_dev,
                void* workspace_dev, size_t workspace_bytes, void* stream);

int mpn_edge_confusion(const void* pred_dev, int pred_kind, const void* labels_dev, int label_kind, int64_t n_edges,
                       int64_t* counts_dev , void* stream);
size_t mpn_contingency_workspace_bytes(int64_t n);
int mpn_contingency(const int64_t* a_dev, const int64_t* b_dev, int64_t n, int64_t Ka, int64_t Kb, int64_t* rows_out_dev,
                    int64_t* cols_out_dev, int64_t* counts_out_dev, int64_t* nnz_host, int64_t* row_sums_dev ,
                    int64_t* col_sums_dev , void* workspace_dev, size_t workspace_bytes, void* stream);
double mpn_expected_mutual_information_host(const int64_t* row_sums_host, int64_t R, const int64_t* col_sums_host, int64_t C,
                                            int64_t n_samples);
size_t mpn_relabel_workspace_bytes(int64_t n_tracklets);
int mpn_relabel_detections(const int64_t* det_cam_dev, const int64_t* det_id_dev, int64_t n_detections, const int64_t* node_cam_dev,
                           const int64_t* node_old_id_dev, const int64_t* node_new_id_dev, int64_t n_tracklets,
                           int64_t* out_id_dev, void* workspace_dev, size_t workspace_bytes, void* stream);
int mpn_write_mtmc_txt_host(const char* path, const int64_t* table_host, int64_t rows, int32_t cols);

int mpn_edge_labels(const mpn_graph* g, const int64_t* node_labels_dev, float* out_dev, void* stream);
size_t mpn_normalize_columns_workspace_bytes(int32_t D);
int mpn_normalize_columns(const float* x_dev, int32_t n, int32_t D, float* out_dev, void* workspace_dev, size_t workspace_bytes,
                          void* stream);
int mpn_normalize_columns_batched(const float* x_dev, int32_t n, int32_t D, const int32_t* graph_nptr_dev, int32_t n_graphs,
                                  float* out_dev, void* workspace_dev, size_t workspace_bytes, void* stream);

#ifdef __cplusplus
}
#endif
#endif
```

Measured before the change: 21.46 billion.

## Fuse node encoder tail layers into one persistent kernel with grid sync

Moves the tcgen05 GEMM tile pipeline into a reusable header and adds a persistent kernel that runs all remaining node-encoder layers after the first: f16 split, tensor-core GEMM or a small SIMT GEMM, column statistics and BN/ReLU, separated by software grid barriers. This replaces many small per-layer launches and their gaps. The grid is sized to the SMs left free by the concurrent edge-feature gram kernel, so the two can overlap on the side stream. It adds a grid-barrier dependency and a static one-time attribute configuration.

Measured after the change: 14.29 billion (median of 6 runs). 0.666x the previous value.

```diff
diff --git a/graph-convolutional-network-for-multi-camera-vehicle-tracking_b200/_lib.py b/graph-convolutional-network-for-multi-camera-vehicle-tracking_b200/_lib.py
--- a/graph-convolutional-network-for-multi-camera-vehicle-tracking_b200/_lib.py
+++ b/graph-convolutional-network-for-multi-camera-vehicle-tracking_b200/_lib.py
@@ -102,6 +102,7 @@
                                   C.c_int64, C.c_int, C.c_void_p, C.c_size_t]),
     "mpn_plan_destroy": (None, [C.c_void_p]),
     "mpn_plan_node_encoder": (C.c_int, [C.c_void_p, C.c_void_p, C.c_void_p]),
+    "mpn_plan_set_encoder_tail": (C.c_int, [C.c_void_p, C.c_int32]),
     "mpn_plan_node_tables": (C.c_int, [C.c_void_p, C.c_int32, C.c_void_p]),
     "mpn_plan_sweep": (C.c_int, [C.c_void_p, C.c_int32, C.c_int32, C.c_void_p, C.c_void_p, C.c_void_p, C.c_void_p, C.c_void_p]),
     "mpn_plan_sums": (C.c_void_p, [C.c_void_p]),
diff --git a/graph-convolutional-network-for-multi-camera-vehicle-tracking_b200/csrc/gemm_tc.cu b/graph-convolutional-network-for-multi-camera-vehicle-tracking_b200/csrc/gemm_tc.cu
--- a/graph-convolutional-network-for-multi-camera-vehicle-tracking_b200/csrc/gemm_tc.cu
+++ b/graph-convolutional-network-for-multi-camera-vehicle-tracking_b200/csrc/gemm_tc.cu
@@ -6,39 +6,9 @@
 
 #include "common.cuh"
 #include "kernels.h"
-#include "tcgen05.cuh"
+#include "gemm_tc_tile.cuh"
 
 namespace mpn {
-
-constexpr int TC_BM = 128;
-constexpr int TC_BK = 32;
-constexpr int TC_UMMA_K = 8;
-constexpr int TC_THREADS = 192;
-constexpr int TC_BK_F16 = 64;
-
-__device__ __forceinline__ uint64_t make_smem_desc(uint32_t saddr) {
-  uint64_t d = 0;
-  d |= (uint64_t)((saddr & 0x3FFFF) >> 4);
-  d |= (uint64_t)1 << 16;
-  d |= (uint64_t)(1024 >> 4) << 32;
-  d |= (uint64_t)1 << 46;
-  d |= (uint64_t)2 << 61;
-  return d;
-}
-
-template <int BN>
-struct TcCfg {
-  static constexpr int STAGES = (BN == 256) ? 2 : 3;
-  static constexpr int A_BYTES = TC_BM * TC_BK * 4;
-  static constexpr int B_BYTES = BN * TC_BK * 4;
-  static constexpr int STAGE_BYTES = 2 * A_BYTES + 2 * B_BYTES;
-  static constexpr int SMEM_BYTES = STAGES * STAGE_BYTES + 1024  + 256 ;
-  static constexpr int N_MAIN = (BN == 256) ? 1 : 2;
-  static constexpr int TMEM_COLS = 512;
-  static constexpr int CORR_COL = N_MAIN * BN;
-  static constexpr uint32_t IDESC = (1u << 4) | (2u << 7) | (2u << 10) | ((uint32_t)(BN >> 3) << 17) | ((uint32_t)(TC_BM >> 4) << 24);
-  static constexpr uint32_t IDESC_F16 = (1u << 4) | ((uint32_t)(BN >> 3) << 17) | ((uint32_t)(TC_BM >> 4) << 24);
-};
 
 template <int BN, bool SYM, bool F16>
 __global__ void __launch_bounds__(TC_THREADS, 1)
@@ -49,19 +19,9 @@
                       const float* __restrict__ out_scale, const int* __restrict__ run_flag) {
   pdl_wait();
   if (run_flag != nullptr && *run_flag == 0) return;
-  constexpr int BK = F16 ? TC_BK_F16 : TC_BK;
-  using Cfg = TcCfg<BN>;
   extern __shared__ uint8_t smem_raw[];
-  uint8_t* smem = (uint8_t*)(((uintptr_t)smem_raw + 1023) & ~(uintptr_t)1023);
-  uint64_t* full_bar = (uint64_t*)(smem + Cfg::STAGES * Cfg::STAGE_BYTES);
-  uint64_t* empty_bar = full_bar + Cfg::STAGES;
-  uint64_t* tmem_full_bar = empty_bar + Cfg::STAGES;
-  uint32_t* tmem_slot = (uint32_t*)(tmem_full_bar + 1);
-
-  const int warp = threadIdx.x >> 5, lane = threadIdx.x & 31;
   int m0 = blockIdx.y * TC_BM, n0 = blockIdx.x * BN;
   int tm0 = m0, tn0 = n0;
-  const int num_kb = (K + BK - 1) / BK;
   if (SYM && n0 + BN <= m0) return;
   if (graph_nptr != nullptr) {
     const int base = graph_nptr[blockIdx.z];
@@ -72,124 +32,16 @@
     M = N = ng;
     C += g_off[blockIdx.z];
   }
+  const float oscale = (F16 && out_scale) ? *out_scale : 1.f;
+  TcPipe<BN> P = tc_setup<BN>(smem_raw);
   if (threadIdx.x == 0) {
-    for (int s = 0; s < Cfg::STAGES; ++s) { mbar_init(&full_bar[s], 1); mbar_init(&empty_bar[s], 1); }
-    mbar_init(tmem_full_bar, 1);
-    asm volatile("fence.mbarrier_init.release.cluster;" ::: "memory");
-  }
-  if (warp == 1) {
-    asm volatile("tcgen05.alloc.cta_group::1.sync.aligned.shared::cta.b32 [%0], %1;" ::"r"(smem_u32(tmem_slot)), "n"(Cfg::TMEM_COLS));
-    asm volatile("tcgen05.relinquish_alloc_permit.cta_group::1.sync.aligned;");
-  }
-  asm volatile("tcgen05.fence::before_thread_sync;" ::: "memory");
-  __syncthreads();
-  asm volatile("tcgen05.fence::after_thread_sync;" ::: "memory");
-  const uint32_t tmem_base = *tmem_slot;
-
-  if (warp == 0) {
-    if (lane == 0) {
-      asm volatile("prefetch.tensormap [%0];" ::"l"(&map_a_hi));
-      asm volatile("prefetch.tensormap [%0];" ::"l"(&map_a_lo));
-      asm volatile("prefetch.tensormap [%0];" ::"l"(&map_b_hi));
-      asm volatile("prefetch.tensormap [%0];" ::"l"(&map_b_lo));
-      int stage = 0;
-      uint32_t phase = 0;
-      for (int kb = 0; kb < num_kb; ++kb) {
-        mbar_wait(&empty_bar[stage], phase ^ 1);
-        uint8_t* st = smem + stage * Cfg::STAGE_BYTES;
-        mbar_expect_tx(&full_bar[stage], Cfg::STAGE_BYTES);
-        const int k0 = kb * BK;
-        tma_load_2d(&map_a_hi, &full_bar[stage], st, k0, tm0);
-        tma_load_2d(&map_a_lo, &full_bar[stage], st + Cfg::A_BYTES, k0, tm0);
-        tma_load_2d(&map_b_hi, &full_bar[stage], st + 2 * Cfg::A_BYTES, k0, tn0);
-        tma_load_2d(&map_b_lo, &full_bar[stage], st + 2 * Cfg::A_BYTES + Cfg::B_BYTES, k0, tn0);
-        if (++stage == Cfg::STAGES) { stage = 0; phase ^= 1; }
-      }
-    }
-  } else if (warp == 1) {
-    if (lane == 0) {
-      int stage = 0;
-      uint32_t phase = 0;
-      for (int kb = 0; kb < num_kb; ++kb) {
-        mbar_wait(&full_bar[stage], phase);
-        asm volatile("tcgen05.fence::after_thread_sync;" ::: "memory");
-        const uint32_t sbase = smem_u32(smem + stage * Cfg::STAGE_BYTES);
-        const uint64_t a_hi = make_smem_desc(sbase), a_lo = make_smem_desc(sbase + Cfg::A_BYTES);
-        const uint64_t b_hi = make_smem_desc(sbase + 2 * Cfg::A_BYTES), b_lo = make_smem_desc(sbase + 2 * Cfg::A_BYTES + Cfg::B_BYTES);
-#pragma unroll
-        for (int kk = 0; kk < TC_BK / TC_UMMA_K; ++kk) {
-          const uint64_t adv = (uint64_t)((kk * TC_UMMA_K * 4) >> 4);
-          const int slice = kb * (TC_BK / TC_UMMA_K) + kk;
-          const int which = (Cfg::N_MAIN == 2) ? (slice & 1) : 0;
-          if (F16) {
-            umma_f16(tmem_base + which * BN, a_hi + adv, b_hi + adv, Cfg::IDESC_F16, slice >= Cfg::N_MAIN);
-            umma_f16(tmem_base + Cfg::CORR_COL, a_lo + adv, b_hi + adv, Cfg::IDESC_F16, slice != 0);
-            umma_f16(tmem_base + Cfg::CORR_COL, a_hi + adv, b_lo + adv, Cfg::IDESC_F16, 1);
-          } else {
-            umma_tf32(tmem_base + which * BN, a_hi + adv, b_hi + adv, Cfg::IDESC, slice >= Cfg::N_MAIN);
-            umma_tf32(tmem_base + Cfg::CORR_COL, a_lo + adv, b_hi + adv, Cfg::IDESC, slice != 0);
-            umma_tf32(tmem_base + Cfg::CORR_COL, a_hi + adv, b_lo + adv, Cfg::IDESC, 1);
-          }
-        }
-        umma_commit(&empty_bar[stage]);
-        if (++stage == Cfg::STAGES) { stage = 0; phase ^= 1; }
-      }
-      umma_commit(tmem_full_bar);
-    }
-  } else {
-    mbar_wait(tmem_full_bar, 0);
-    asm volatile("tcgen05.fence::after_thread_sync;" ::: "memory");
-    const int q = warp & 3;
-    const int row = m0 + q * 32 + lane;
-    const bool vec_ok = ((N & 3) == 0) && ((((uintptr_t)C) & 15) == 0);
-    const float oscale = (F16 && out_scale) ? *out_scale : 1.f;
-#pragma unroll 1
-    for (int c0 = 0; c0 < BN; c0 += 32) {
-      if (n0 + c0 >= N) break;
-      float v[32], w[32];
-      const uint32_t tq = tmem_base + ((uint32_t)(q * 32) << 16) + (uint32_t)c0;
-      tmem_ld32(tq, v);
-      if (Cfg::N_MAIN == 2) {
-        tmem_ld32(tq + BN, w);
-#pragma unroll
-        for (int j = 0; j < 32; ++j) v[j] += w[j];
-      }
-      tmem_ld32(tq + Cfg::CORR_COL, w);
-#pragma unroll
-      for (int j = 0; j < 32; ++j) v[j] = F16 ? (v[j] + w[j]) * oscale : v[j] + w[j];
-      if (row < M) {
-        float* out = C + (size_t)row * N + n0 + c0;
-        if (vec_ok && n0 + c0 + 32 <= N) {
-#pragma unroll
-          for (int j = 0; j < 32; j += 4) {
-            float4 o = make_float4(v[j], v[j + 1], v[j + 2], v[j + 3]);
-            if (bias) {
-              const float4 b = *reinterpret_cast<const float4*>(bias + n0 + c0 + j);
-              o.x += b.x; o.y += b.y; o.z += b.z; o.w += b.w;
-            }
-            *reinterpret_cast<float4*>(out + j) = o;
-          }
-        } else {
-#pragma unroll
-          for (int j = 0; j < 32; ++j)
-            if (n0 + c0 + j < N) out[j] = v[j] + (bias ? bias[n0 + c0 + j] : 0.f);
-        }
-      }
-      if (SYM && row < M) {
-#pragma unroll
-        for (int j = 0; j < 32; ++j) {
-          const int col = n0 + c0 + j;
-          if (col < N && col >= m0 + TC_BM) C[(size_t)col * N + row] = v[j];
-        }
-      }
-    }
-    asm volatile("tcgen05.fence::before_thread_sync;" ::: "memory");
-  }
-  __syncthreads();
-  if (warp == 1) {
-    asm volatile("tcgen05.fence::after_thread_sync;" ::: "memory");
-    asm volatile("tcgen05.dealloc.cta_group::1.sync.aligned.b32 %0, %1;" ::"r"(tmem_base), "n"(Cfg::TMEM_COLS));
-  }
+    asm volatile("prefetch.tensormap [%0];" ::"l"(&map_a_hi));
+    asm volatile("prefetch.tensormap [%0];" ::"l"(&map_a_lo));
+    asm volatile("prefetch.tensormap [%0];" ::"l"(&map_b_hi));
+    asm volatile("prefetch.tensormap [%0];" ::"l"(&map_b_lo));
+  }
+  tc_tile<BN, SYM, F16>(P, &map_a_hi, &map_a_lo, &map_b_hi, &map_b_lo, bias, C, M, N, K, m0, n0, tm0, tn0, oscale);
+  tc_teardown<BN>(P);
 }
 
 __global__ void __launch_bounds__(256) split_tf32_kernel(const float4* __restrict__ x, long long n4, int K, const float* __restrict__ scale,
@@ -224,12 +76,6 @@
   }
 }
 
-__device__ __forceinline__ float f16_scale_of(float amax) {
-  if (!(amax > 0.f) || !isfinite(amax)) return 1.f;
-  int e;
-  frexpf(amax, &e);
-  return ldexpf(1.f, 14 - e);
-}
 __global__ void __launch_bounds__(256) split_f16_kernel(const float4* __restrict__ x, long long n4, const float* __restrict__ amax,
                                                         uint2* __restrict__ hi, uint2* __restrict__ lo, float* __restrict__ out_scale,
                                                         const int* __restrict__ run_flag) {
@@ -372,33 +218,8 @@
   const float s = f16_scale_of(amax_dev ? *amax_dev : amax_host);
   if (out_scale && blockIdx.x == 0 && threadIdx.x == 0) *out_scale = (1.f / s) * (1.f / b_scale);
   const long long stride = (long long)gridDim.x * blockDim.x;
-  for (long long i = (long long)blockIdx.x * blockDim.x + threadIdx.x; i < n4; i += stride) {
-    const float4 v = x[i];
-    float in[4] = {v.x, v.y, v.z, v.w};
-    if (scale != nullptr) {
-      const int k = (int)((i * 4) % K);
-      const size_t o = (row_gid ? (size_t)row_gid[(i * 4) / K] * K : 0) + k;
-      const float4 sc = *reinterpret_cast<const float4*>(scale + o), sh = *reinterpret_cast<const float4*>(shift + o);
-      in[0] = fmaxf(fmaf(in[0], sc.x, sh.x), 0.f);
-      in[1] = fmaxf(fmaf(in[1], sc.y, sh.y), 0.f);
-      in[2] = fmaxf(fmaf(in[2], sc.z, sh.z), 0.f);
-      in[3] = fmaxf(fmaf(in[3], sc.w, sh.w), 0.f);
-    }
-    __half h[4], l[4];
-#pragma unroll
-    for (int j = 0; j < 4; ++j) {
-      const float t = fminf(in[j] * s, 65000.f);
-      h[j] = __float2half_rn(t);
-      l[j] = __float2half_rn(t - __half2float(h[j]));
-    }
-    uint2 ph, pl;
-    ph.x = (uint32_t)__half_as_ushort(h[0]) | ((uint32_t)__half_as_ushort(h[1]) << 16);
-    ph.y = (uint32_t)__half_as_ushort(h[2]) | ((uint32_t)__half_as_ushort(h[3]) << 16);
-    pl.x = (uint32_t)__half_as_ushort(l[0]) | ((uint32_t)__half_as_ushort(l[1]) << 16);
-    pl.y = (uint32_t)__half_as_ushort(l[2]) | ((uint32_t)__half_as_ushort(l[3]) << 16);
-    hi[i] = ph;
-    lo[i] = pl;
-  }
+  for (long long i = (long long)blockIdx.x * blockDim.x + threadIdx.x; i < n4; i += stride)
+    split_f16_bn4(x[i], i, K, scale, shift, row_gid, s, hi, lo);
 }
 __global__ void __launch_bounds__(256) absmax_kernel(const float4* __restrict__ x, long long n4, unsigned int* __restrict__ amax_bits) {
   pdl_wait();
diff --git a/graph-convolutional-network-for-multi-camera-vehicle-tracking_b200/csrc/gemm_tc_tile.cuh b/graph-convolutional-network-for-multi-camera-vehicle-tracking_b200/csrc/gemm_tc_tile.cuh
--- /dev/null
+++ b/graph-convolutional-network-for-multi-camera-vehicle-tracking_b200/csrc/gemm_tc_tile.cuh
@@ -0,0 +1,225 @@
+#pragma once
+#include <cuda.h>
+#include <cuda_fp16.h>
+
+#include "common.cuh"
+#include "tcgen05.cuh"
+
+namespace mpn {
+
+constexpr int TC_BM = 128;
+constexpr int TC_BK = 32;
+constexpr int TC_UMMA_K = 8;
+constexpr int TC_THREADS = 192;
+constexpr int TC_BK_F16 = 64;
+
+__device__ __forceinline__ uint64_t make_smem_desc(uint32_t saddr) {
+  uint64_t d = 0;
+  d |= (uint64_t)((saddr & 0x3FFFF) >> 4);
+  d |= (uint64_t)1 << 16;
+  d |= (uint64_t)(1024 >> 4) << 32;
+  d |= (uint64_t)1 << 46;
+  d |= (uint64_t)2 << 61;
+  return d;
+}
+
+template <int BN>
+struct TcCfg {
+  static constexpr int STAGES = (BN == 256) ? 2 : 3;
+  static constexpr int A_BYTES = TC_BM * TC_BK * 4;
+  static constexpr int B_BYTES = BN * TC_BK * 4;
+  static constexpr int STAGE_BYTES = 2 * A_BYTES + 2 * B_BYTES;
+  static constexpr int SMEM_BYTES = STAGES * STAGE_BYTES + 1024  + 256 ;
+  static constexpr int N_MAIN = (BN == 256) ? 1 : 2;
+  static constexpr int TMEM_COLS = 512;
+  static constexpr int CORR_COL = N_MAIN * BN;
+  static constexpr uint32_t IDESC = (1u << 4) | (2u << 7) | (2u << 10) | ((uint32_t)(BN >> 3) << 17) | ((uint32_t)(TC_BM >> 4) << 24);
+  static constexpr uint32_t IDESC_F16 = (1u << 4) | ((uint32_t)(BN >> 3) << 17) | ((uint32_t)(TC_BM >> 4) << 24);
+};
+
+template <int BN>
+struct TcPipe {
+  uint8_t* smem;
+  uint64_t *full_bar, *empty_bar, *tmem_full_bar;
+  uint32_t tmem_base;
+  int stage;
+  uint32_t phase, acc_phase;
+};
+
+template <int BN>
+__device__ __forceinline__ TcPipe<BN> tc_setup(uint8_t* smem_raw) {
+  using Cfg = TcCfg<BN>;
+  TcPipe<BN> p;
+  p.smem = (uint8_t*)(((uintptr_t)smem_raw + 1023) & ~(uintptr_t)1023);
+  p.full_bar = (uint64_t*)(p.smem + Cfg::STAGES * Cfg::STAGE_BYTES);
+  p.empty_bar = p.full_bar + Cfg::STAGES;
+  p.tmem_full_bar = p.empty_bar + Cfg::STAGES;
+  uint32_t* tmem_slot = (uint32_t*)(p.tmem_full_bar + 1);
+  if (threadIdx.x == 0) {
+    for (int s = 0; s < Cfg::STAGES; ++s) { mbar_init(&p.full_bar[s], 1); mbar_init(&p.empty_bar[s], 1); }
+    mbar_init(p.tmem_full_bar, 1);
+    asm volatile("fence.mbarrier_init.release.cluster;" ::: "memory");
+  }
+  if ((threadIdx.x >> 5) == 1) {
+    asm volatile("tcgen05.alloc.cta_group::1.sync.aligned.shared::cta.b32 [%0], %1;" ::"r"(smem_u32(tmem_slot)), "n"(Cfg::TMEM_COLS));
+    asm volatile("tcgen05.relinquish_alloc_permit.cta_group::1.sync.aligned;");
+  }
+  asm volatile("tcgen05.fence::before_thread_sync;" ::: "memory");
+  __syncthreads();
+  asm volatile("tcgen05.fence::after_thread_sync;" ::: "memory");
+  p.tmem_base = *tmem_slot;
+  p.stage = 0;
+  p.phase = 0;
+  p.acc_phase = 0;
+  return p;
+}
+
+template <int BN>
+__device__ __forceinline__ void tc_teardown(const TcPipe<BN>& p) {
+  if ((threadIdx.x >> 5) == 1) {
+    asm volatile("tcgen05.fence::after_thread_sync;" ::: "memory");
+    asm volatile("tcgen05.dealloc.cta_group::1.sync.aligned.b32 %0, %1;" ::"r"(p.tmem_base), "n"(TcCfg<BN>::TMEM_COLS));
+  }
+}
+
+template <int BN, bool SYM, bool F16>
+__device__ __forceinline__ void tc_tile(TcPipe<BN>& P, const CUtensorMap* map_a_hi, const CUtensorMap* map_a_lo,
+                                        const CUtensorMap* map_b_hi, const CUtensorMap* map_b_lo, const float* __restrict__ bias,
+                                        float* __restrict__ C, int M, int N, int K, int m0, int n0, int tm0, int tn0, float oscale) {
+  constexpr int BK = F16 ? TC_BK_F16 : TC_BK;
+  using Cfg = TcCfg<BN>;
+  const int warp = threadIdx.x >> 5, lane = threadIdx.x & 31;
+  const int num_kb = (K + BK - 1) / BK;
+  if (warp == 0) {
+    if (lane == 0) {
+      for (int kb = 0; kb < num_kb; ++kb) {
+        mbar_wait(&P.empty_bar[P.stage], P.phase ^ 1);
+        uint8_t* st = P.smem + P.stage * Cfg::STAGE_BYTES;
+        mbar_expect_tx(&P.full_bar[P.stage], Cfg::STAGE_BYTES);
+        const int k0 = kb * BK;
+        tma_load_2d(map_a_hi, &P.full_bar[P.stage], st, k0, tm0);
+        tma_load_2d(map_a_lo, &P.full_bar[P.stage], st + Cfg::A_BYTES, k0, tm0);
+        tma_load_2d(map_b_hi, &P.full_bar[P.stage], st + 2 * Cfg::A_BYTES, k0, tn0);
+        tma_load_2d(map_b_lo, &P.full_bar[P.stage], st + 2 * Cfg::A_BYTES + Cfg::B_BYTES, k0, tn0);
+        if (++P.stage == Cfg::STAGES) { P.stage = 0; P.phase ^= 1; }
+      }
+    }
+  } else if (warp == 1) {
+    if (lane == 0) {
+      const uint32_t tmem_base = P.tmem_base;
+      for (int kb = 0; kb < num_kb; ++kb) {
+        mbar_wait(&P.full_bar[P.stage], P.phase);
+        asm volatile("tcgen05.fence::after_thread_sync;" ::: "memory");
+        const uint32_t sbase = smem_u32(P.smem + P.stage * Cfg::STAGE_BYTES);
+        const uint64_t a_hi = make_smem_desc(sbase), a_lo = make_smem_desc(sbase + Cfg::A_BYTES);
+        const uint64_t b_hi = make_smem_desc(sbase + 2 * Cfg::A_BYTES), b_lo = make_smem_desc(sbase + 2 * Cfg::A_BYTES + Cfg::B_BYTES);
+#pragma unroll
+        for (int kk = 0; kk < TC_BK / TC_UMMA_K; ++kk) {
+          const uint64_t adv = (uint64_t)((kk * TC_UMMA_K * 4) >> 4);
+          const int slice = kb * (TC_BK / TC_UMMA_K) + kk;
+          const int which = (Cfg::N_MAIN == 2) ? (slice & 1) : 0;
+          if (F16) {
+            umma_f16(tmem_base + which * BN, a_hi + adv, b_hi + adv, Cfg::IDESC_F16, slice >= Cfg::N_MAIN);
+            umma_f16(tmem_base + Cfg::CORR_COL, a_lo + adv, b_hi + adv, Cfg::IDESC_F16, slice != 0);
+            umma_f16(tmem_base + Cfg::CORR_COL, a_hi + adv, b_lo + adv, Cfg::IDESC_F16, 1);
+          } else {
+            umma_tf32(tmem_base + which * BN, a_hi + adv, b_hi + adv, Cfg::IDESC, slice >= Cfg::N_MAIN);
+            umma_tf32(tmem_base + Cfg::CORR_COL, a_lo + adv, b_hi + adv, Cfg::IDESC, slice != 0);
+            umma_tf32(tmem_base + Cfg::CORR_COL, a_hi + adv, b_lo + adv, Cfg::IDESC, 1);
+          }
+        }
+        umma_commit(&P.empty_bar[P.stage]);
+        if (++P.stage == Cfg::STAGES) { P.stage = 0; P.phase ^= 1; }
+      }
+      umma_commit(P.tmem_full_bar);
+    }
+  } else if (warp < 6) {
+    mbar_wait(P.tmem_full_bar, P.acc_phase);
+    asm volatile("tcgen05.fence::after_thread_sync;" ::: "memory");
+    const int q = warp & 3;
+    const int row = m0 + q * 32 + lane;
+    const bool vec_ok = ((N & 3) == 0) && ((((uintptr_t)C) & 15) == 0);
+#pragma unroll 1
+    for (int c0 = 0; c0 < BN; c0 += 32) {
+      if (n0 + c0 >= N) break;
+      float v[32], w[32];
+      const uint32_t tq = P.tmem_base + ((uint32_t)(q * 32) << 16) + (uint32_t)c0;
+      tmem_ld32(tq, v);
+      if (Cfg::N_MAIN == 2) {
+        tmem_ld32(tq + BN, w);
+#pragma unroll
+        for (int j = 0; j < 32; ++j) v[j] += w[j];
+      }
+      tmem_ld32(tq + Cfg::CORR_COL, w);
+#pragma unroll
+      for (int j = 0; j < 32; ++j) v[j] = F16 ? (v[j] + w[j]) * oscale : v[j] + w[j];
+      if (row < M) {
+        float* out = C + (size_t)row * N + n0 + c0;
+        if (vec_ok && n0 + c0 + 32 <= N) {
+#pragma unroll
+          for (int j = 0; j < 32; j += 4) {
+            float4 o = make_float4(v[j], v[j + 1], v[j + 2], v[j + 3]);
+            if (bias) {
+              const float4 b = *reinterpret_cast<const float4*>(bias + n0 + c0 + j);
+              o.x += b.x; o.y += b.y; o.z += b.z; o.w += b.w;
+            }
+            *reinterpret_cast<float4*>(out + j) = o;
+          }
+        } else {
+#pragma unroll
+          for (int j = 0; j < 32; ++j)
+            if (n0 + c0 + j < N) out[j] = v[j] + (bias ? bias[n0 + c0 + j] : 0.f);
+        }
+      }
+      if (SYM && row < M) {
+#pragma unroll
+        for (int j = 0; j < 32; ++j) {
+          const int col = n0 + c0 + j;
+          if (col < N && col >= m0 + TC_BM) C[(size_t)col * N + row] = v[j];
+        }
+      }
+    }
+    asm volatile("tcgen05.fence::before_thread_sync;" ::: "memory");
+  }
+  P.acc_phase ^= 1;
+  __syncthreads();
+  asm volatile("tcgen05.fence::after_thread_sync;" ::: "memory");
+}
+
+__device__ __forceinline__ float f16_scale_of(float amax) {
+  if (!(amax > 0.f) || !isfinite(amax)) return 1.f;
+  int e;
+  frexpf(amax, &e);
+  return ldexpf(1.f, 14 - e);
+}
+
+__device__ __forceinline__ void split_f16_bn4(const float4 v, long long i, int K, const float* __restrict__ scale,
+                                              const float* __restrict__ shift, const int* __restrict__ row_gid, float s,
+                                              uint2* __restrict__ hi, uint2* __restrict__ lo) {
+  float in[4] = {v.x, v.y, v.z, v.w};
+  if (scale != nullptr) {
+    const int k = (int)((i * 4) % K);
+    const size_t o = (row_gid ? (size_t)row_gid[(i * 4) / K] * K : 0) + k;
+    const float4 sc = *reinterpret_cast<const float4*>(scale + o), sh = *reinterpret_cast<const float4*>(shift + o);
+    in[0] = fmaxf(fmaf(in[0], sc.x, sh.x), 0.f);
+    in[1] = fmaxf(fmaf(in[1], sc.y, sh.y), 0.f);
+    in[2] = fmaxf(fmaf(in[2], sc.z, sh.z), 0.f);
+    in[3] = fmaxf(fmaf(in[3], sc.w, sh.w), 0.f);
+  }
+  __half h[4], l[4];
+#pragma unroll
+  for (int j = 0; j < 4; ++j) {
+    const float t = fminf(in[j] * s, 65000.f);
+    h[j] = __float2half_rn(t);
+    l[j] = __float2half_rn(t - __half2float(h[j]));
+  }
+  uint2 ph, pl;
+  ph.x = (uint32_t)__half_as_ushort(h[0]) | ((uint32_t)__half_as_ushort(h[1]) << 16);
+  ph.y = (uint32_t)__half_as_ushort(h[2]) | ((uint32_t)__half_as_ushort(h[3]) << 16);
+  pl.x = (uint32_t)__half_as_ushort(l[0]) | ((uint32_t)__half_as_ushort(l[1]) << 16);
+  pl.y = (uint32_t)__half_as_ushort(l[2]) | ((uint32_t)__half_as_ushort(l[3]) << 16);
+  hi[i] = ph;
+  lo[i] = pl;
+}
+
+}
diff --git a/graph-convolutional-network-for-multi-camera-vehicle-tracking_b200/csrc/gram_ef.cu b/graph-convolutional-network-for-multi-camera-vehicle-tracking_b200/csrc/gram_ef.cu
--- a/graph-convolutional-network-for-multi-camera-vehicle-tracking_b200/csrc/gram_ef.cu
+++ b/graph-convolutional-network-for-multi-camera-vehicle-tracking_b200/csrc/gram_ef.cu
@@ -700,6 +700,15 @@
   return MPN_OK;
 }
 
+int gram_ef_busy_blocks(int M, int N, int sym) {
+  const long long tm = (M + GE_BM - 1) / GE_BM, tn = (N + GE_BN - 1) / GE_BN;
+  const long long tiles = sym ? tm * (tm + 1) / 2 : tm * tn;
+  const long long grid = tm * tn < kNumSMs ? tm * tn : kNumSMs;
+  if (tiles <= 0 || grid <= 0) return 0;
+  const long long rounds = (tiles + grid - 1) / grid;
+  return (int)((tiles + rounds - 1) / rounds);
+}
+
 }
 
 extern "C" int mpn_shared_gram_row_range(int32_t rank, int32_t world, const int32_t* block_start, int32_t c, int32_t* out) {
diff --git a/graph-convolutional-network-for-multi-camera-vehicle-tracking_b200/csrc/kernels.h b/graph-convolutional-network-for-multi-camera-vehicle-tracking_b200/csrc/kernels.h
--- a/graph-convolutional-network-for-multi-camera-vehicle-tracking_b200/csrc/kernels.h
+++ b/graph-convolutional-network-for-multi-camera-vehicle-tracking_b200/csrc/kernels.h
@@ -30,6 +30,7 @@
 };
 int ge_workspace_layout(int n_cols, int M, int D, GeWorkspace* L, void* ws, size_t ws_bytes);
 bool gram_ef_shape_ok(int M, int N, int D);
+int gram_ef_busy_blocks(int M, int N, int sym);
 int ge_col_mean_splits();
 int ge_col_mean(const float* x, int n, int D, double* part, unsigned int* ticket, float* mu, cudaStream_t st);
 int gram_ef_run(const float* x, const float* mu, const mpn_graph* g, int D, int2* gap, int* not_one_gap, float2* edge_attr,
diff --git a/graph-convolutional-network-for-multi-camera-vehicle-tracking_b200/csrc/mpn_forward.cu b/graph-convolutional-network-for-multi-camera-vehicle-tracking_b200/csrc/mpn_forward.cu
--- a/graph-convolutional-network-for-multi-camera-vehicle-tracking_b200/csrc/mpn_forward.cu
+++ b/graph-convolutional-network-for-multi-camera-vehicle-tracking_b200/csrc/mpn_forward.cu
@@ -5,7 +5,7 @@
 
 #include "common.cuh"
 #include "kernels.h"
-#include "tcgen05.cuh"
+#include "gemm_tc_tile.cuh"
 
 namespace mpn {
 
@@ -1292,18 +1292,18 @@
 }
 
 constexpr int CS_ROWSPLIT_MAX = 64;
-__global__ void __launch_bounds__(256) colstats_kernel(const float* __restrict__ Y, int M, int Nc, int rows_per_split,
-                                                       double* __restrict__ part , unsigned int* __restrict__ tile_counter,
-                                                       const float* __restrict__ gamma, const float* __restrict__ beta,
-                                                       float* __restrict__ scale, float* __restrict__ shift) {
-  pdl_wait();
+__device__ __forceinline__ void colstats_item(const float* __restrict__ Y, int M, int Nc, int rows_per_split, int tx, int ty,
+                                              int n_splits, double* __restrict__ part ,
+                                              unsigned int* __restrict__ tile_counter, const float* __restrict__ gamma,
+                                              const float* __restrict__ beta, float* __restrict__ scale, float* __restrict__ shift) {
   __shared__ double ssum[8][33], ssq[8][33];
   __shared__ unsigned int s_ticket;
   const int cx = threadIdx.x & 31, ry = threadIdx.x >> 5;
-  const int col = blockIdx.x * 32 + cx;
-  const int r0 = blockIdx.y * rows_per_split, r1 = min(r0 + rows_per_split, M);
+  const int col = tx * 32 + cx;
+  const int r0 = ty * rows_per_split, r1 = min(r0 + rows_per_split, M);
   double s = 0.0, q = 0.0;
   if (col < Nc)
+#pragma unroll 8
     for (int r = r0 + ry; r < r1; r += 8) {
       const double v = Y[(size_t)r * Nc + col];
       s += v;
@@ -1314,19 +1314,19 @@
   __syncthreads();
   if (ry == 0 && col < Nc) {
     for (int i = 1; i < 8; ++i) { s += ssum[i][cx]; q += ssq[i][cx]; }
-    part[((size_t)blockIdx.y * Nc + col) * 2 + 0] = s;
-    part[((size_t)blockIdx.y * Nc + col) * 2 + 1] = q;
+    part[((size_t)ty * Nc + col) * 2 + 0] = s;
+    part[((size_t)ty * Nc + col) * 2 + 1] = q;
   }
   if (tile_counter == nullptr) return;
   __threadfence();
   __syncthreads();
-  if (threadIdx.x == 0) s_ticket = atomicAdd(&tile_counter[blockIdx.x], 1u);
+  if (threadIdx.x == 0) s_ticket = atomicAdd(&tile_counter[tx], 1u);
   __syncthreads();
-  if (s_ticket != gridDim.y - 1) return;
+  if (s_ticket != (unsigned int)n_splits - 1) return;
   __threadfence();
   if (ry == 0 && col < Nc) {
     double ts = 0.0, tq = 0.0;
-    for (int i = 0; i < (int)gridDim.y; ++i) {
+    for (int i = 0; i < n_splits; ++i) {
       ts += __ldcg(&part[((size_t)i * Nc + col) * 2 + 0]);
       tq += __ldcg(&part[((size_t)i * Nc + col) * 2 + 1]);
     }
@@ -1337,7 +1337,15 @@
     scale[col] = (float)sc;
     shift[col] = (float)((double)beta[col] - sc * mean);
   }
-  if (threadIdx.x == 0) tile_counter[blockIdx.x] = 0u;
+  if (threadIdx.x == 0) tile_counter[tx] = 0u;
+}
+
+__global__ void __launch_bounds__(256) colstats_kernel(const float* __restrict__ Y, int M, int Nc, int rows_per_split,
+                                                       double* __restrict__ part , unsigned int* __restrict__ tile_counter,
+                                                       const float* __restrict__ gamma, const float* __restrict__ beta,
+                                                       float* __restrict__ scale, float* __restrict__ shift) {
+  pdl_wait();
+  colstats_item(Y, M, Nc, rows_per_split, blockIdx.x, blockIdx.y, gridDim.y, part, tile_counter, gamma, beta, scale, shift);
 }
 
 __global__ void __launch_bounds__(1024) colstats_peer_kernel(const double* __restrict__ part, int splits, int Nc, int M_total,
@@ -1403,6 +1411,128 @@
     const size_t o = row_gid ? (size_t)row_gid[i / Nc] * Nc + c : (size_t)c;
     out[i] = fmaxf(fmaf(Y[i], scale[o], shift[o]), 0.f);
   }
+}
+
+constexpr int ENC_TAIL_THREADS = 256;
+constexpr int ENC_TAIL_ROWS = ENC_TAIL_THREADS / 32;
+constexpr int ENC_TAIL_UNROLL = 8;
+constexpr int ENC_TAIL_MAX = MPN_MAX_NODE_LAYERS - 1;
+constexpr int ENC_TAIL_RING_BYTES = TcCfg<128>::STAGES * TcCfg<128>::STAGE_BYTES;
+
+struct EncTailLayer {
+  const float* in;
+  float* out;
+  const float *w, *bias, *gamma, *beta;
+  uint2 *a_hi, *a_lo;
+  float amax, b_scale;
+  int K, Nc, tc;
+};
+struct EncTailArgs {
+  EncTailLayer layer[ENC_TAIL_MAX];
+  int n_layers, M, splits, rows_per_split;
+  float *scale, *shift;
+  double* part;
+  unsigned int* col_counter;
+  unsigned int* barrier;
+  float* h;
+};
+struct EncTailMaps {
+  CUtensorMap m[4 * ENC_TAIL_MAX];
+};
+
+__device__ __forceinline__ void enc_grid_sync(unsigned int* ticket, unsigned int& target) {
+  asm volatile("fence.proxy.async;" ::: "memory");
+  __syncthreads();
+  target += gridDim.x;
+  if (threadIdx.x == 0) {
+    __threadfence();
+    atomicAdd(ticket, 1u);
+    unsigned int v;
+    asm volatile("ld.acquire.gpu.global.u32 %0, [%1];" : "=r"(v) : "l"(ticket) : "memory");
+    if (v < target) {
+      unsigned long long t0, t1;
+      asm volatile("mov.u64 %0, %%globaltimer;" : "=l"(t0));
+      do {
+        asm volatile("mov.u64 %0, %%globaltimer;" : "=l"(t1));
+        if (t1 - t0 > 4000000000ull) __trap();
+        asm volatile("ld.acquire.gpu.global.u32 %0, [%1];" : "=r"(v) : "l"(ticket) : "memory");
+      } while (v < target);
+    }
+  }
+  __syncthreads();
+  asm volatile("fence.proxy.async;" ::: "memory");
+}
+
+__global__ void __launch_bounds__(ENC_TAIL_THREADS, 1) node_encoder_tail_kernel(const __grid_constant__ EncTailMaps maps, const EncTailArgs A) {
+  pdl_wait();
+  extern __shared__ uint8_t smem_raw[];
+  TcPipe<128> P = tc_setup<128>(smem_raw);
+  const int warp = threadIdx.x >> 5, lane = threadIdx.x & 31;
+  const int M = A.M;
+  const long long gtid = (long long)blockIdx.x * blockDim.x + threadIdx.x, gstride = (long long)gridDim.x * blockDim.x;
+  unsigned int target = 0;
+  for (int l = 0; l < A.n_layers; ++l) {
+    const EncTailLayer& L = A.layer[l];
+    const int K = L.K, Nc = L.Nc;
+    const float* in = L.in;
+    if (L.tc) {
+      const float s = f16_scale_of(L.amax);
+      const long long n4 = (long long)M * K / 4;
+      for (long long i0 = gtid; i0 < n4; i0 += ENC_TAIL_UNROLL * gstride) {
+        float4 v[ENC_TAIL_UNROLL];
+#pragma unroll
+        for (int j = 0; j < ENC_TAIL_UNROLL; ++j)
+          if (i0 + j * gstride < n4) v[j] = __ldcg((const float4*)in + i0 + j * gstride);
+#pragma unroll
+        for (int j = 0; j < ENC_TAIL_UNROLL; ++j)
+          if (i0 + j * gstride < n4) split_f16_bn4(v[j], i0 + j * gstride, K, A.scale, A.shift, nullptr, s, L.a_hi, L.a_lo);
+      }
+      enc_grid_sync(A.barrier, target);
+      const float oscale = (1.f / s) * (1.f / L.b_scale);
+      const int tn = (Nc + 127) / 128, n_tiles = tn * ((M + TC_BM - 1) / TC_BM);
+      for (int t = blockIdx.x; t < n_tiles; t += gridDim.x) {
+        const int m0 = (t / tn) * TC_BM, n0 = (t % tn) * 128;
+        tc_tile<128, false, true>(P, &maps.m[4 * l], &maps.m[4 * l + 1], &maps.m[4 * l + 2], &maps.m[4 * l + 3], L.bias, L.out, M, Nc,
+                                  K, m0, n0, m0, n0, oscale);
+      }
+    } else {
+      const int Kp = K | 1;
+      float* ws = (float*)P.smem;
+      float* as = ws + (size_t)Nc * Kp;
+      for (int i = threadIdx.x; i < Nc * K; i += blockDim.x) ws[(i / K) * Kp + i % K] = L.w[i];
+      for (int r0 = blockIdx.x * ENC_TAIL_ROWS; r0 < M; r0 += gridDim.x * ENC_TAIL_ROWS) {
+        __syncthreads();
+        for (int i = threadIdx.x; i < ENC_TAIL_ROWS * K; i += blockDim.x) {
+          const int r = r0 + i / K, k = i % K;
+          as[i] = r < M ? fmaxf(fmaf(in[(size_t)r * K + k], A.scale[k], A.shift[k]), 0.f) : 0.f;
+        }
+        __syncthreads();
+        const int r = r0 + warp;
+        if (r < M)
+          for (int n = lane; n < Nc; n += 32) {
+            const float *a = as + warp * K, *b = ws + (size_t)n * Kp;
+            float acc = 0.f;
+            for (int k = 0; k < K; ++k) acc = fmaf(a[k], b[k], acc);
+            L.out[(size_t)r * Nc + n] = acc + L.bias[n];
+          }
+      }
+      __syncthreads();
+    }
+    enc_grid_sync(A.barrier, target);
+    const int ctiles = (Nc + 31) / 32;
+    for (int it = blockIdx.x; it < ctiles * A.splits; it += gridDim.x) {
+      colstats_item(L.out, M, Nc, A.rows_per_split, it % ctiles, it / ctiles, A.splits, A.part, A.col_counter, L.gamma, L.beta,
+                    A.scale, A.shift);
+      __syncthreads();
+    }
+    enc_grid_sync(A.barrier, target);
+  }
+  const float* y = A.layer[A.n_layers - 1].out;
+  for (long long i = gtid; i < (long long)M * MPN_DH; i += gstride) {
+    const int c = (int)(i % MPN_DH);
+    A.h[i] = fmaxf(fmaf(y[i], A.scale[c], A.shift[c]), 0.f);
+  }
+  tc_teardown<128>(P);
 }
 
 constexpr int NT_NODES = 64, NT_THREADS = 256, NT_OUT = 40;
@@ -1534,6 +1664,8 @@
   PeerArgs* peers_dev;
   unsigned long long seq_m;
   unsigned int* col_counter;
+  int enc_tail_grid;
+  int enc_tail_auto;
   int fuse_fin;
   int n_graphs;
   double* n_total_dev;
@@ -1558,6 +1690,8 @@
   f.consts = p->consts;
   return f;
 }
+
+static size_t col_counter_words(const mpn_fwd_plan& p) { return (size_t)(p.max_dim > 0 ? p.max_dim : 1) / 32 + 2; }
 
 static int plan_layout(mpn_fwd_plan& p, void* ws, size_t ws_bytes, size_t* need) {
   Arena a(ws, ws_bytes);
@@ -1588,7 +1722,7 @@
   p.fix_sums = a.take<unsigned long long>(8);
   p.peers_dev = a.take<PeerArgs>(1);
   p.n_total_dev = a.take<double>(1);
-  p.col_counter = a.take<unsigned int>((size_t)(max_dim > 0 ? max_dim : 1) / 32 + 1);
+  p.col_counter = a.take<unsigned int>(col_counter_words(p));
   p.ybuf = stores_y(p) ? a.take<float>((size_t)g.n_edges * 4) : nullptr;
   size_t gw = 0;
   if (p.use_tc) {
@@ -1701,15 +1835,87 @@
   return b > 0.f ? b * 1.0001f : 1.f;
 }
 
+static bool encoder_tail_covers(const mpn_fwd_plan* p, int l0) {
+  if (p->enc_tail_grid < 0 || p->n_graphs > 1 || !p->use_tc || l0 < 1 || p->w.n_node_layers - l0 > ENC_TAIL_MAX) return false;
+  const int M = p->g.n_cols;
+  for (int l = l0; l < p->w.n_node_layers; ++l) {
+    const int K = p->w.node_dims[l], Nc = p->w.node_dims[l + 1];
+    if (gemm_tc_supported(M, Nc, K)) {
+      if (!encoder_f16(p, l, K)) return false;
+    } else if ((size_t)Nc * (K | 1) * 4 + (size_t)ENC_TAIL_ROWS * K * 4 > (size_t)ENC_TAIL_RING_BYTES) {
+      return false;
+    }
+  }
+  return true;
+}
+
+static int node_encoder_tail(mpn_fwd_plan* p, int l0, cudaStream_t st) {
+  const int M = p->g.n_cols;
+  EncTailMaps maps;
+  EncTailArgs A;
+  memset(&maps, 0, sizeof(maps));
+  memset(&A, 0, sizeof(A));
+  float* bufs[2] = {p->act0, p->act1};
+  char* w = (char*)(((uintptr_t)p->gemm_ws + 255) & ~(uintptr_t)255);
+  A.n_layers = p->w.n_node_layers - l0;
+  A.M = M;
+  for (int i = 0; i < A.n_layers; ++i) {
+    const int l = l0 + i;
+    EncTailLayer& L = A.layer[i];
+    L.K = p->w.node_dims[l];
+    L.Nc = p->w.node_dims[l + 1];
+    L.in = bufs[(l - 1) & 1];
+    L.out = bufs[l & 1];
+    L.w = p->w.node_w[l];
+    L.bias = p->w.node_b[l];
+    L.gamma = p->w.node_gamma[l];
+    L.beta = p->w.node_beta[l];
+    L.tc = gemm_tc_supported(M, L.Nc, L.K) ? 1 : 0;
+    if (L.tc) {
+      const size_t plane = (((size_t)M * L.K * sizeof(__half)) + 255) & ~(size_t)255;
+      MPN_REQUIRE(p->gemm_ws_bytes >= gemm_tc_workspace_bytes(M, L.Nc, L.K), "node encoder tail: GEMM workspace too small");
+      L.a_hi = (uint2*)w;
+      L.a_lo = (uint2*)(w + plane);
+      L.amax = encoder_input_bound(p, l, M);
+      L.b_scale = p->w.node_w_scale16[l];
+      MPN_TRY(make_tma_map_2d(&maps.m[4 * i], L.a_hi, M, L.K, TC_BM, true));
+      MPN_TRY(make_tma_map_2d(&maps.m[4 * i + 1], L.a_lo, M, L.K, TC_BM, true));
+      MPN_TRY(make_tma_map_2d(&maps.m[4 * i + 2], p->w.node_w_hi16[l], L.Nc, L.K, 128, true));
+      MPN_TRY(make_tma_map_2d(&maps.m[4 * i + 3], p->w.node_w_lo16[l], L.Nc, L.K, 128, true));
+    }
+  }
+  int splits = div_up(M, 256);
+  A.splits = splits > CS_ROWSPLIT_MAX ? CS_ROWSPLIT_MAX : splits;
+  A.rows_per_split = div_up(M, A.splits);
+  A.scale = p->colscale;
+  A.shift = p->colshift;
+  A.part = p->colpart;
+  A.col_counter = p->col_counter;
+  A.barrier = p->col_counter + col_counter_words(*p) - 1;
+  A.h = p->h_full;
+  const int want = p->enc_tail_grid > 0 ? p->enc_tail_grid : (p->enc_tail_auto > 0 ? p->enc_tail_auto : kNumSMs);
+  const int grid = want < kNumSMs ? want : kNumSMs;
+  constexpr int smem = TcCfg<128>::SMEM_BYTES;
+  static bool configured = false;
+  if (!configured) {
+    MPN_CUDA_OK(cudaFuncSetAttribute(node_encoder_tail_kernel, cudaFuncAttributeMaxDynamicSharedMemorySize, smem));
+    configured = true;
+  }
+  mpn::launch(node_encoder_tail_kernel, grid, ENC_TAIL_THREADS, smem, st, maps, A);
+  MPN_LAUNCH_OK();
+  return MPN_OK;
+}
+
 static int node_encoder_layers(mpn_fwd_plan* p, const float* x, int l_begin, int l_end, cudaStream_t st) {
   MPN_REQUIRE(p && x, "node_encoder: NULL argument");
   const int M = p->g.n_cols;
   const bool batched = p->n_graphs > 1;
-  if (l_begin == 0) MPN_CUDA_OK(cudaMemsetAsync(p->col_counter, 0, sizeof(unsigned int) * ((size_t)p->max_dim / 32 + 1), st));
+  if (l_begin == 0) MPN_CUDA_OK(cudaMemsetAsync(p->col_counter, 0, sizeof(unsigned int) * col_counter_words(*p), st));
   float* bufs[2] = {p->act0, p->act1};
   const float* in = l_begin == 0 ? x : bufs[(l_begin - 1) & 1];
   const float *sc = l_begin == 0 ? nullptr : p->colscale, *sh = l_begin == 0 ? nullptr : p->colshift;
   for (int l = l_begin; l < l_end; ++l) {
+    if (l > 0 && l_end == p->w.n_node_layers && encoder_tail_covers(p, l)) return node_encoder_tail(p, l, st);
     const int K = p->w.node_dims[l], Nc = p->w.node_dims[l + 1];
     float* out = bufs[l & 1];
     bool done = false;
@@ -1742,6 +1948,12 @@
   if (l_end < p->w.n_node_layers) return MPN_OK;
   mpn::launch(bn_relu_apply_kernel, min(kNumSMs * 4, div_up((long long)M * MPN_DH, 256)), 256, 0, st, in, (long long)M * MPN_DH, MPN_DH, sc, sh, batched ? p->g.node_gid : nullptr, p->h_full);
   MPN_LAUNCH_OK();
+  return MPN_OK;
+}
+
+int mpn_plan_set_encoder_tail(mpn_fwd_plan* p, int32_t grid) {
+  MPN_REQUIRE(p, "set_encoder_tail: NULL plan");
+  p->enc_tail_grid = grid;
   return MPN_OK;
 }
 
@@ -2014,6 +2226,10 @@
       STEP_TRY(node_encoder_layers(p, x, enc_done_layers, p->w.n_node_layers, fork ? ss->stream : st)); \
       tl_mark("node_encoder_end(side stream)", fork ? ss->stream : st); \
       if (fork && cudaEventRecord(ss->join, ss->stream) != cudaSuccess) { set_error("event record failed"); rc = MPN_ERR_CUDA; goto done; } } } while (0)
+    if (fork && ef_ws != nullptr && p->n_graphs <= 1) {
+      const int free_sms = kNumSMs - gram_ef_busy_blocks(g->n_nodes, g->n_cols, 1);
+      p->enc_tail_auto = free_sms > 0 ? free_sms : 0;
+    }
     if (!fork || ef_ws == nullptr) ENQUEUE_ENCODER();
     else if (p->w.n_node_layers > 1) {
       STEP_TRY(node_encoder_layers(p, x, 0, 1, ss->stream));
diff --git a/include/mpn_b200.h b/include/mpn_b200.h
--- a/include/mpn_b200.h
+++ b/include/mpn_b200.h
@@ -148,6 +148,7 @@
                     void* workspace_dev, size_t workspace_bytes);
 void mpn_plan_destroy(mpn_fwd_plan* plan);
 int mpn_plan_node_encoder(mpn_fwd_plan* plan, const float* x_dev, void* stream);
+int mpn_plan_set_encoder_tail(mpn_fwd_plan* plan, int32_t grid);
 int mpn_plan_node_tables(mpn_fwd_plan* plan, int32_t step, void* stream);
 int mpn_plan_sweep(mpn_fwd_plan* plan, int32_t step, int32_t stage, const float* edge_attr_dev,
                    float* logits_out_dev, uint8_t* pred_out_dev, float* prob1_out_dev, void* stream);
```
